# relgukxilef/GAN-Class-Transfer2

Measured on AMD Instinct MI355X. Metric: images/sec (train step) 3x128x128 bs=64/GPU, higher is better.
Workload: dtype bf16; 1 GPU; BASELINE config 3: Trainer step, 3x128x128, bs 64/GPU, octaves 6, pixel_size 128, max_size 512, bf16 operands / fp32 accumulate, Keras Adam + WarmUp; global_batch=64, parallelism=dp1

## Files before the change

gan-class-transfer2_amd/_lib.py:

```python
from __future__ import annotations

import ctypes as C
import os
import struct

F32, BF16, F16 = 0, 1, 2
F32_MATH_DIRECT, F32_MATH_MFMA = 0, 1
DTYPE_NAMES = {F32: "f32", BF16: "bf16", F16: "f16"}
ABI_VERSION = 17
DENSE2_FAST_PIXELS = 64
DENSE2_PLAIN_MAX = 256
SAMPLE_X, SAMPLE_EPS, SAMPLE_SCALED_EPS, SAMPLE_ODE = 0, 1, 2, 3
BUILD_STAMP = 1
CLIP_NONE, CLIP_VALUE, CLIP_NORM, CLIP_GLOBAL_NORM = 0, 1, 2, 3
SUMSQ_CHUNK, SUMSQ_MAX_SEGMENTS = 32768, 1024
OPT_ADAM, OPT_SGD, OPT_RMSPROP = 0, 1, 2
SCHEDULE_WARMUP, SCHEDULE_INVERSE_TIME_DECAY = 0, 1
GRAD_NONE, GRAD_SIGN = 0, 1
LOSS_MSE, LOSS_L1, LOSS_MSE_POOLED, LOSS_DCT = 0, 1, 2, 3

_HERE = os.path.dirname(os.path.abspath(__file__))
LIB_PATH = os.path.join(_HERE, "csrc", "libgct2.so")


class Gct2Error(RuntimeError):
    """non-zero status from libgct2 (mirrors TensorFlow raising on bad shapes, SURVEY.md §8b)."""


class LossScaleState(C.Structure):
    _fields_ = [("scale", C.c_float), ("inv_scale", C.c_float), ("good_steps", C.c_int32), ("found_inf", C.c_int32),
                ("applied_steps", C.c_int32), ("alpha", C.c_float), ("reserved", C.c_int32 * 2)]


class AdamArgs(C.Structure):
    _fields_ = [("p", C.c_void_p), ("m", C.c_void_p), ("v", C.c_void_p), ("shadow", C.c_void_p), ("shadow_dtype", C.c_int),
                ("n", C.c_size_t), ("alpha", C.c_float), ("beta1", C.c_float), ("beta2", C.c_float), ("eps", C.c_float),
                ("grad_mul", C.c_float), ("defer", C.c_int), ("slab_base", C.c_void_p), ("nslab", C.c_int), ("slab_stride", C.c_size_t)]


_vp, _i, _f, _d, _u64, _sz = C.c_void_p, C.c_int, C.c_float, C.c_double, C.c_uint64, C.c_size_t

SIGNATURES = {
    "gct2_abi_version": [],
    "gct2_build_flags": [],
    "gct2_device_check": [],
    "gct2_stream_occupy": [_vp, _i, _d],
    "gct2_ctx_create": [C.POINTER(C.c_void_p)],
    "gct2_ctx_destroy": [_vp],
    "gct2_ctx_set_workspace": [_vp, _vp, _sz],
    "gct2_ctx_set_wgrad_workspace": [_vp, _vp, _sz],
    "gct2_ctx_set_bias_queue": [_vp, _vp, _sz],
    "gct2_bias_queue_flush": [_vp, _vp],
    "gct2_ctx_set_tuning": [_vp, _i],
    "gct2_ctx_force_direct": [_vp, _i],
    "gct2_ctx_set_f32_math": [_vp, _i],
    "gct2_ctx_set_stamp_buffer": [_vp, _vp, _sz],
    "gct2_ctx_set_relu_bits": [_vp, _vp, _i],
    "gct2_ctx_log_launches": [_vp, _i],
    "gct2_ctx_read_launch_log": [_vp, _vp, _sz, C.POINTER(C.c_size_t)],
    "gct2_diffusion_mix": [_i, _vp, _vp, _f, _vp, _vp, _i, _vp, _i, _sz, _i, _vp],
    "gct2_diffusion_update": [_i, _vp, _vp, _d, _d, _vp, _vp, _sz, _vp],
    "gct2_noise_edits": [_vp, _vp, _i, _vp, _i, _i, _i, _vp],
    "gct2_image_prepare": [_vp, _vp, _vp, _vp, _i, _i, _vp],
    "gct2_conv4s2_fwd": [_vp, _i, _vp, _i, _vp, _vp, _vp, _i, _i, _i, _i, _i, _i, _i, _vp],
    "gct2_conv4s2_dgrad": [_vp, _i, _vp, _i, _vp, _vp, _i, _vp, _i, _i, _i, _i, _i, _i, _i, _vp, _i, _vp, _i, _vp],
    "gct2_conv4s2_wgrad": [_vp, _i, _vp, _i, _vp, _i, _vp, _vp, _i, _i, _i, _i, _i, _i, _vp, _vp],
    "gct2_adam_apply": [_vp, _vp, _sz, _vp],
    "gct2_convT4s2_fwd": [_vp, _i, _vp, _i, _vp, _vp, _vp, _i, _i, _i, _i, _i, _i, _i, _vp],
    "gct2_convT4s2_fwd_head_train": [_vp, _i, _vp, _i, _vp, _vp, _vp, _vp, _vp, _vp, _vp, _i, _vp, _vp, _vp, _i, _i, _i, _i, _i, _i, _i,
                                     _vp, _vp, _vp, _i, _i, _vp],
    "gct2_convT4s2_dgrad": [_vp, _i, _vp, _i, _vp, _vp, _i, _vp, _i, _i, _i, _i, _i, _i, _i, _vp, _i, _vp, _i, _vp],
    "gct2_convT4s2_wgrad": [_vp, _i, _vp, _i, _vp, _i, _vp, _vp, _i, _i, _i, _i, _i, _i, _vp, _vp],
    "gct2_conv2d_s1_fwd": [_vp, _i, _vp, _i, _vp, _vp, _vp, _i, _i, _i, _i, _i, _i, _i, _i, _vp],
    "gct2_conv2d_s1_dgrad": [_vp, _i, _vp, _i, _vp, _vp, _i, _vp, _i, _i, _i, _i, _i, _i, _i, _i, _vp],
    "gct2_conv2d_s1_wgrad": [_vp, _i, _vp, _i, _vp, _i, _vp, _vp, _i, _i, _i, _i, _i, _i, _i, _vp],
    "gct2_relu_mask": [_i, _vp, _i, _vp, _i, _sz, _i, _vp],
    "gct2_add": [_i, _vp, _i, _vp, _i, _sz, _i, _vp],
    "gct2_mix_per_image": [_vp, _vp, _vp, _vp, _vp, _i, _sz, _vp],
    "gct2_dense_fwd": [_i, _vp, _i, _vp, _vp, _vp, _i, _i, _i, _vp],
    "gct2_dense_bwd": [_i, _vp, _i, _vp, _vp, _vp, _i, _vp, _vp, _i, _i, _i, _i, _i, _vp],
    "gct2_dense_head_train": [_vp, _i, _vp, _i, _vp, _vp, _vp, _vp, _vp, _i, _vp, _vp, _vp, _vp, _i, _i, _i, _i, _vp, _vp, _vp, _i, _i, _vp],
    "gct2_dense_steps_fwd": [_vp, _i, _vp, _i, _vp, _vp, _vp, _vp, _i, _i, _i, _i, _i, _vp],
    "gct2_dense_steps_scratch": [_i, _i, _i, _i, C.POINTER(C.c_size_t)],
    "gct2_dense_steps_bwd": [_vp, _i, _vp, _i, _vp, _vp, _vp, _vp, _i, _vp, _vp, _vp, _sz, _i, _i, _i, _i, _i, _i, _i, _vp],
    "gct2_dense2_fwd": [_vp, _i, _vp, _i, _vp, _vp, _vp, _vp, _vp, _i, _i, _i, _i, _vp],
    "gct2_dense2_scratch": [_i, _i, _i, _i, C.POINTER(C.c_size_t)],
    "gct2_dense2_bwd": [_vp, _i, _vp, _i, _vp, _vp, _vp, _vp, _vp, _i, _vp, _vp, _vp, _vp, _vp, _sz, _i, _i, _i, _i, _i, _i, _vp],
    "gct2_rng_uniform_int": [_u64, _u64, _u64, _vp, _sz, _i, _i, _vp],
    "gct2_rng_normal": [_u64, _u64, _u64, _vp, _sz, _vp],
    "gct2_noise_image": [_i, _vp, _vp, _vp, _vp, _i, _vp, _i, _i, _i, _i, _i, _vp],
    "gct2_noise_image_rng": [_i, _vp, _vp, _u64, _u64, _u64, _vp, _vp, _i, _vp, _i, _i, _i, _i, _i, _vp],
    "gct2_mse_fwd_bwd": [_vp, _vp, _vp, _vp, _vp, _sz, _vp, _vp],
    "gct2_loss_scratch": [_i, _i, _i, _i, _i, C.POINTER(C.c_size_t)],
    "gct2_loss_fwd_bwd": [_i, _vp, _vp, _vp, _vp, _vp, _sz, _i, _i, _i, _i, _vp, _vp, _vp],
    "gct2_adam_keras_multi": [_vp, _vp, _vp, _vp, _vp, _i, _sz, _f, _f, _f, _f, _f, _vp, _i, _vp],
    "gct2_ema_update": [_vp, _vp, _vp, _i, _sz, _f, _f, _vp, _vp],
    "gct2_sumsq_layout": [_vp, _vp, _i, _vp, C.POINTER(C.c_size_t)],
    "gct2_grad_sumsq": [_vp, _vp, _i, _sz, _f, _vp, _vp, _vp, _vp],
    "gct2_adam_keras_clipped": [_vp, _vp, _vp, _vp, _vp, _i, _sz, _f, _f, _f, _f, _f, _vp, _i, _f, _vp, _vp],
    "gct2_optimizer_apply": [_i, _vp, _vp, _vp, _vp, _vp, _i, _sz, _f, _f, _i, _f, _f, _f, _vp, _i, _f, _vp, _vp],
    "gct2_optimizer_apply_reg": [_i, _vp, _vp, _vp, _vp, _vp, _i, _sz, _f, _f, _i, _f, _f, _f, _vp, _i, _f, _vp, _f, _i, _vp],
    "gct2_grad_sumsq_l2": [_vp, _vp, _vp, _vp, _i, _sz, _f, _vp, _vp, _vp, _vp],
    "gct2_l2_penalty": [_vp, _vp, _f, _vp, _vp, _vp],
    "gct2_cast_from_f32": [_i, _vp, _vp, _sz, _vp],
    "gct2_loss_scale_init": [_vp, _f, _vp],
    "gct2_loss_scale_begin": [_vp, _f, _i, _f, _f, _vp],
    "gct2_loss_scale_begin_schedule": [_vp, _i, _f, _f, _f, _i, _i, _f, _f, _vp],
    "gct2_scale_check_finite": [_vp, _sz, _vp, _vp],
    "gct2_loss_scale_update": [_vp, _i, _vp],
    "gct2_plan_create": [C.POINTER(C.c_void_p)],
    "gct2_plan_destroy": [_vp],
    "gct2_plan_add_call": [_vp, C.c_char_p, C.POINTER(C.c_uint64), _i, C.POINTER(C.c_int)],
    "gct2_plan_add_record": [_vp, _vp, C.POINTER(C.c_int)],
    "gct2_plan_add_wait": [_vp, _vp, _i],
    "gct2_plan_add_record_kind": [_vp, _vp, _i, C.POINTER(C.c_int)],
    "gct2_plan_elapsed": [_vp, _i, _i, C.POINTER(C.c_float)],
    "gct2_plan_size": [_vp, C.POINTER(C.c_int)],
    "gct2_plan_set_arg": [_vp, _i, _i, _u64],
    "gct2_plan_run": [_vp, _i, _i, C.POINTER(C.c_int)],
}

_lib = None


def load() -> C.CDLL:
    global _lib
    if _lib is not None:
        return _lib
    path = LIB_PATH
    if os.environ.get("GCT2_ALLOW_DIAGNOSTIC_BUILD") == "1" and os.environ.get("GCT2_USE_STAMP_LIB") in ("1", "phases"):
        path = os.path.join(_HERE, "csrc", "libgct2_phases.so" if os.environ["GCT2_USE_STAMP_LIB"] == "phases" else "libgct2_stamp.so")
    if not os.path.exists(path):
        raise Gct2Error(
            f"{path} not found: build it with `python -c 'import __graft_entry__ as g; g.build()'` "
            "(or `make -C gan-class-transfer2_amd/csrc`). There is no CPU fallback.")
    lib = C.CDLL(path)
    for name, argtypes in SIGNATURES.items():
        fn = getattr(lib, name)
        fn.argtypes = argtypes
        fn.restype = _i
    lib.gct2_last_error.argtypes = []
    lib.gct2_last_error.restype = C.c_char_p
    if lib.gct2_abi_version() != ABI_VERSION:
        raise Gct2Error(f"{LIB_PATH} has ABI version {lib.gct2_abi_version()}, this binding is written for {ABI_VERSION}: rebuild it "
                        "(`make -C gan-class-transfer2_amd/csrc`)")
    flags = lib.gct2_build_flags()
    if flags != 0 and os.environ.get("GCT2_ALLOW_DIAGNOSTIC_BUILD") != "1":
        raise Gct2Error(f"{LIB_PATH} is a DIAGNOSTIC build (gct2_build_flags() = {flags}: in-kernel stamps): results and timings of "
                        "such a library are never product numbers.  Rebuild with `make -C gan-class-transfer2_amd/csrc clean all`, or "
                        "set GCT2_ALLOW_DIAGNOSTIC_BUILD=1 for the scripts/stamp_*.py diagnostics")
    _lib = lib
    return lib


def build_flags() -> int:
    return int(load().gct2_build_flags())


def check(rc: int, what: str = "") -> None:
    if rc != 0:
        msg = load().gct2_last_error().decode("utf-8", "replace")
        raise Gct2Error(f"{what or 'gct2'} failed (status {rc}): {msg}")


class Slot:
    __slots__ = ("key", "value")

    def __init__(self, key: str, value):
        self.key, self.value = key, value


def call(name: str, *args) -> None:
    if _recording is not None:
        _recording.add_call(name, args)
        if not _recording.execute or name not in PLANNABLE:
            return
    check(getattr(load(), name)(*[a.value if type(a) is Slot else a for a in args]), name)


PLANNABLE = frozenset(n for n, sig in SIGNATURES.items() if n == "gct2_ctx_set_relu_bits" or (
    not n.startswith(("gct2_ctx_", "gct2_plan_", "gct2_loss_scale_init")) and n not in ("gct2_abi_version", "gct2_build_flags", "gct2_device_check", "gct2_stream_occupy", "gct2_sumsq_layout", "gct2_loss_scratch", "gct2_dense_steps_scratch", "gct2_dense2_scratch")))
_recording = None
_FLOAT_STRUCT = struct.Struct("<f")
_DOUBLE_STRUCT = struct.Struct("<d")


def _slot_bits(ctype, v) -> int:
    if ctype is _f:
        return int.from_bytes(_FLOAT_STRUCT.pack(float(v)), "little")
    if ctype is _d:
        return int.from_bytes(_DOUBLE_STRUCT.pack(float(v)), "little")
    if v is None:
        return 0
    return int(v) & 0xFFFFFFFFFFFFFFFF


EVENT_DEVICE, EVENT_SYSTEM, EVENT_TIMED = 0, 1, 2


class Plan:

    def __init__(self):
        h = C.c_void_p()
        check(load().gct2_plan_create(C.byref(h)), "gct2_plan_create")
        self.handle = h.value
        self.execute = True
        self.slots = {}
        self.values = {}
        self.cuts = []
        self.keep = []
        self.n = 0

    def begin(self, execute: bool = True) -> None:
        global _recording
        if _recording is not None:
            raise Gct2Error("a plan is already recording")
        self.execute = execute
        _recording = self

    def end(self) -> None:
        global _recording
        _recording = None
        self.cuts.append((self.n, None))

    def add_call(self, name: str, args) -> None:
        if name not in PLANNABLE:
            check(getattr(load(), name)(*[a.value if type(a) is Slot else a for a in args]), name)
            return
        types = SIGNATURES[name]
        if len(types) != len(args):
            raise Gct2Error(f"{name}: {len(args)} arguments for {len(types)} parameters")
        arr = (C.c_uint64 * len(args))()
        for i, (t, a) in enumerate(zip(types, args)):
            if type(a) is Slot:
                self.slots.setdefault(a.key, []).append((self.n, i, t))
                self.values[a.key] = a.value
                a = a.value
            arr[i] = _slot_bits(t, a)
        idx = C.c_int(-1)
        check(load().gct2_plan_add_call(self.handle, name.encode(), arr, len(args), C.byref(idx)), "gct2_plan_add_call")
        self.n = idx.value + 1

    def record(self, stream: int, kind: int = EVENT_DEVICE) -> int:
        ev = C.c_int(-1)
        check(load().gct2_plan_add_record_kind(self.handle, stream, kind, C.byref(ev)), "gct2_plan_add_record_kind")
        self.n += 1
        return ev.value

    def elapsed_ms(self, start: int, end: int) -> float:
        ms = C.c_float(0.0)
        check(load().gct2_plan_elapsed(self.handle, start, end, C.byref(ms)), "gct2_plan_elapsed")
        return ms.value

    def wait(self, stream: int, event: int) -> None:
        check(load().gct2_plan_add_wait(self.handle, stream, event), "gct2_plan_add_wait")
        self.n += 1

    def cut(self, payload) -> None:
        self.cuts.append((self.n, payload))

    def set(self, key: str, value) -> None:
        if self.values.get(key) == value:
            return
        self.values[key] = value
        L = load()
        for rec, arg, t in self.slots.get(key, ()):
            check(L.gct2_plan_set_arg(self.handle, rec, arg, _slot_bits(t, value)), "gct2_plan_set_arg")

    def segments(self) -> int:
        return len(self.cuts)

    def run_segment(self, k: int):
        first = self.cuts[k - 1][0] if k else 0
        last, payload = self.cuts[k]
        if last > first:
            failed = C.c_int(-1)
            rc = load().gct2_plan_run(self.handle, first, last - first, C.byref(failed))
            if rc != 0:
                check(rc, f"gct2_plan_run (record {failed.value})")
        return payload

    def __del__(self):
        try:
            if getattr(self, "handle", None) and _lib is not None:
                _lib.gct2_plan_destroy(self.handle)
                self.handle = None
        except Exception:
            pass


class Context:

    def __init__(self):
        h = C.c_void_p()
        call("gct2_ctx_create", C.byref(h))
        self.handle = h.value
        self._keep = [None, None, None]
        self.version = 0
        self.tuning = 0
        self.direct = False
        self.f32_math = F32_MATH_DIRECT
        self.logging = False

    def set_relu_bits(self, ptr, ld_bytes: int) -> None:
        call("gct2_ctx_set_relu_bits", self.handle, ptr, int(ld_bytes) if ptr is not None else 0)

    def set_stamp_buffer(self, tensor) -> None:
        self._keep[2] = tensor
        self.version += 1
        call("gct2_ctx_set_stamp_buffer", self.handle, tensor.data_ptr() if tensor is not None else None,
             tensor.numel() * tensor.element_size() if tensor is not None else 0)

    def log_launches(self, on: bool = True) -> None:
        self.logging = bool(on)
        call("gct2_ctx_log_launches", self.handle, int(bool(on)))

    def read_launch_log(self) -> list:
        need = C.c_size_t(0)
        buf = C.create_string_buffer(1 << 12)
        rc = load().gct2_ctx_read_launch_log(self.handle, C.cast(buf, C.c_void_p), len(buf), C.byref(need))
        if rc != 0 and need.value > len(buf):
            buf = C.create_string_buffer(need.value)
            rc = load().gct2_ctx_read_launch_log(self.handle, C.cast(buf, C.c_void_p), len(buf), C.byref(need))
        check(rc, "gct2_ctx_read_launch_log")
        return [t for t in buf.value.decode().split(";") if t]

    def mirror(self, other: "Context") -> None:
        if self.tuning != other.tuning:
            self.set_tuning(other.tuning)
        if self.direct != other.direct:
            self.force_direct(other.direct)
        if self.f32_math != other.f32_math:
            self.set_f32_math(other.f32_math)
        if self.logging != other.logging:
            self.log_launches(other.logging)
        if self._keep[2] is not other._keep[2]:
            self.set_stamp_buffer(other._keep[2])

    def set_workspace(self, tensor) -> None:
        self._keep[0] = tensor
        self.version += 1
        call("gct2_ctx_set_workspace", self.handle, tensor.data_ptr() if tensor is not None else None,
             tensor.numel() * tensor.element_size() if tensor is not None else 0)

    def set_wgrad_workspace(self, tensor) -> None:
        self._keep[1] = tensor
        self.version += 1
        call("gct2_ctx_set_wgrad_workspace", self.handle, tensor.data_ptr() if tensor is not None else None,
             tensor.numel() * tensor.element_size() if tensor is not None else 0)

    def set_bias_queue(self, tensor) -> None:
        self._keep.append(tensor)
        self.version += 1
        call("gct2_ctx_set_bias_queue", self.handle, tensor.data_ptr() if tensor is not None else None,
             tensor.numel() * tensor.element_size() if tensor is not None else 0)

    def set_tuning(self, v: int) -> None:
        self.version += 1
        self.tuning = int(v)
        call("gct2_ctx_set_tuning", self.handle, int(v))

    def force_direct(self, on: bool) -> None:
        self.version += 1
        self.direct = bool(on)
        call("gct2_ctx_force_direct", self.handle, int(bool(on)))

    def set_f32_math(self, mode: int) -> None:
        call("gct2_ctx_set_f32_math", self.handle, int(mode))
        self.version += 1
        self.f32_math = int(mode)

    def __del__(self):
        try:
            if getattr(self, "handle", None) and _lib is not None:
                _lib.gct2_ctx_destroy(self.handle)
                self.handle = None
        except Exception:
            pass
```

gan-class-transfer2_amd/csrc/capi.hip:

```cpp
#include "gct2_common.h"
#include <cstdarg>
#include <cstdio>
#include <cstring>

static thread_local char g_err[512] = "";
static thread_local gct2_ctx g_null_ctx{};

int gct2_fail(int code, const char* fmt, ...) {
  va_list ap;
  va_start(ap, fmt);
  vsnprintf(g_err, sizeof(g_err), fmt, ap);
  va_end(ap);
  return code;
}
void gct2_log(gct2_ctx& c, const char* fmt, ...) {
  if (!c.log_on) return;
  char buf[160];
  va_list ap;
  va_start(ap, fmt);
  vsnprintf(buf, sizeof(buf), fmt, ap);
  va_end(ap);
  constexpr size_t LOG_CAP = (size_t)1 << 20;
  if (c.log.size() + sizeof(buf) + 16 > LOG_CAP) {
    if (!c.log_full) { c.log += "log:truncated;"; c.log_full = true; }
    return;
  }
  c.log += buf;
  c.log += ';';
}
int gct2_check_launch(const char* what) {
  const hipError_t e = hipGetLastError();
  if (e != hipSuccess) return gct2_fail(GCT2_ELAUNCH, "%s: %s", what, hipGetErrorString(e));
  return GCT2_OK;
}

namespace {
inline hipStream_t S(void* s) { return reinterpret_cast<hipStream_t>(s); }
inline bool dtype_ok(int d) { return d == GCT2_F32 || d == GCT2_BF16 || d == GCT2_F16; }
inline size_t esize(int d) { return d == GCT2_F32 ? 4 : 2; }

int check_conv_args(const char* fn, int dtype, const void* a, const void* b, const void* c, int B, int H, int W, int Cin, int Cout) {
  if (!dtype_ok(dtype)) return gct2_fail(GCT2_EINVAL, "%s: unknown dtype %d", fn, dtype);
  if (!a || !b || !c) return gct2_fail(GCT2_EINVAL, "%s: null pointer", fn);
  if (B <= 0 || H <= 0 || W <= 0 || Cin <= 0 || Cout <= 0) return gct2_fail(GCT2_EINVAL, "%s: non-positive dimension", fn);
  if ((size_t)B * H * W * 4 >= ((size_t)1 << 31)) return gct2_fail(GCT2_EINVAL, "%s: B*H*W too large for 32-bit pixel indices", fn);
  return GCT2_OK;
}
inline gct2_ctx& C(gct2_ctx* c) {
  if (c) return *c;
  g_null_ctx = gct2_ctx{};
  return g_null_ctx;
}
struct PlaneTaken {
  unsigned char* bits; int ld;
  explicit PlaneTaken(gct2_ctx& c) : bits(c.relu_bits), ld(c.relu_ldbits) { c.relu_bits = nullptr; c.relu_ldbits = 0; c.relu_bits_done = 0; }
  int none(const char* fn) const {
    return bits ? gct2_fail(GCT2_EINVAL, "%s: a ReLU bit plane was registered (gct2_ctx_set_relu_bits), but this call neither writes nor reads one", fn) : GCT2_OK;
  }
  int into(const char* fn, int channels, TapGemmParams& p) const {
    if (!bits) return GCT2_OK;
    if (channels % 8 || ld < channels / 8) return gct2_fail(GCT2_EINVAL, "%s: ReLU bit plane needs channels %% 8 == 0 and ld_bytes >= channels / 8 (got %d, %d)", fn, channels, ld);
    p.bits = bits; p.ldbits = ld;
    return GCT2_OK;
  }
};
int finish_relu_bits(gct2_ctx& c, int dtype, const TapGemmParams& p, size_t pixels, void* stream) {
  if (!p.bits || c.relu_bits_done) return GCT2_OK;
  gct2_log(c, "relu_bits:derived");
  return pw_relu_bits(dtype, p.y, p.ldy, pixels, p.N, p.bits, p.ldbits, S(stream));
}
inline bool f32_on_mfma(const gct2_ctx& c, int dtype) { return dtype == GCT2_F32 && c.f32_math == GCT2_F32_MATH_MFMA && !c.force_direct; }
int run_tapgemm(gct2_ctx& c, int dtype, int form, int epi, const TapGemmParams& p, void* stream) {
  const bool s1 = form == FORM_S1 || form == FORM_S1T;
  if (f32_on_mfma(c, dtype)) return f32_tapgemm(c, form, epi, p, S(stream));
  if (!c.force_direct && (!s1 || p.ks <= 5) && tapgemm_mfma_supported(dtype, p)) return tapgemm_mfma(c, dtype, form, epi, p, S(stream));
  if (s1)
    return conv_s1_direct(dtype, form == FORM_S1T, p.x, p.ldx, p.w, p.bias, p.act, p.ldact, p.y, p.ldy, p.B, p.Hs, p.Ws, p.K, p.N, p.ks, p.relu,
                          p.accumulate, S(stream));
  gct2_log(c, "direct:tap");
  return tapgemm_direct(dtype, form, epi, p, S(stream));
}
int run_dgrad(gct2_ctx& c, int dtype, int form, TapGemmParams p, size_t out_pixels, float* db, int split, float* db2, int db_acc,
              void* stream) {
  if (split < 0 || split > p.N) return gct2_fail(GCT2_EINVAL, "dgrad: db_split out of range");
  p.db = db; p.db_split = split; p.db2 = db2; p.db_acc = db_acc;
  if (!c.force_direct && tapgemm_mfma_supported(dtype, p)) return tapgemm_mfma(c, dtype, form, EPI_MASK, p, S(stream));
  const bool f32m = f32_on_mfma(c, dtype);
  if (!f32m) gct2_log(c, "direct:tap");
  if (int e = tapgemm_dbq_flush_for(c, db, split, db2, p.N - split, S(stream))) return e;
  zero_overwritten_db(p, S(stream));
  const size_t es = esize(dtype);
  auto sums = [&](float sign) -> int {
    if (db && split > 0) if (int e = pw_colsum(dtype, p.y, p.ldy, db, out_pixels, split, sign, S(stream))) return e;
    if (db2 && split < p.N)
      if (int e = pw_colsum(dtype, (const char*)p.y + (size_t)split * es, p.ldy, db2, out_pixels, p.N - split, sign, S(stream))) return e;
    return GCT2_OK;
  };
  if ((db || db2) && p.accumulate) if (int e = sums(-1.f)) return e;
  if (int e = f32m ? f32_tapgemm(c, form, EPI_MASK, p, S(stream)) : tapgemm_direct(dtype, form, EPI_MASK, p, S(stream))) return e;
  return (db || db2) ? sums(1.f) : GCT2_OK;
}
int run_wgrad(gct2_ctx& c, int dtype, const WgradParams& p, void* stream, WgradSlabs* defer) {
  if (f32_on_mfma(c, dtype)) return f32_wgrad(c, p, S(stream), defer);
  if (!c.force_direct && wgrad_mfma_supported(dtype, p)) return wgrad_mfma(c, dtype, p, S(stream), defer);
  if (defer) *defer = WgradSlabs{nullptr, 0, 0};
  if (p.ks)
    return conv_s1_wgrad_direct(dtype, p.big, p.ldbig, p.small, p.ldsmall, p.dw, p.B, p.Hs, p.Ws, p.Cb, p.Cs, p.ks, p.accumulate, S(stream));
  gct2_log(c, "direct:wgrad");
  return wgrad_direct(dtype, p, S(stream));
}
int wgrad_db(gct2_ctx& c, int dtype, const void* dz, int lddz, float* db, size_t pixels, int Cout, int accumulate, void* stream) {
  if (int e = tapgemm_dbq_flush_for(c, db, Cout, nullptr, 0, S(stream))) return e;
  if (!accumulate) (void)hipMemsetAsync(db, 0, (size_t)Cout * sizeof(float), S(stream));
  return pw_colsum(dtype, dz, lddz, db, pixels, Cout, 1.f, S(stream));
}
int check_adam_args(const gct2_adam_args* a, const float* dw, size_t nw) {
  if (!a->p || !a->m || !a->v) return gct2_fail(GCT2_EINVAL, "wgrad + adam: null arena pointers");
  if (a->n < nw || ((uintptr_t)a->p | (uintptr_t)a->m | (uintptr_t)a->v | (uintptr_t)dw) % 16)
    return gct2_fail(GCT2_EINVAL, "wgrad + adam: range shorter than the weight tensor or misaligned");
  return GCT2_OK;
}
int run_adam(const gct2_adam_args* a, float* dw, size_t nw, const WgradSlabs& sl, void* stream) {
  return pw_adam(a->p, a->m, a->v, dw, a->shadow, a->shadow_dtype, a->n, a->alpha, a->beta1, a->beta2, a->eps, a->grad_mul, nullptr, 0,
                 S(stream), sl.base, sl.nslab, sl.stride, sl.nslab ? nw : 0);
}
int adam_after_wgrad(gct2_adam_args* a, float* dw, size_t nw, const WgradSlabs& sl, void* stream) {
  if (a->defer) {
    a->slab_base = sl.base; a->nslab = sl.nslab; a->slab_stride = sl.stride;
    return GCT2_OK;
  }
  return run_adam(a, dw, nw, sl, stream);
}
int check_s1(const char* fn, int KS) {
  if (KS < 1 || KS > 7 || !(KS & 1)) return gct2_fail(GCT2_EINVAL, "%s: kernel size %d (odd, 1..7: 'same' padding is symmetric then)", fn, KS);
  return GCT2_OK;
}
enum WgradKind { WG_CONV, WG_CONVT, WG_S1 };
int wgrad_entry(gct2_ctx* ctx, const char* fn, WgradKind kind, int dtype, const void* x, int ldx, const void* dz, int lddz, float* dw, float* db,
                int B, int H, int W, int Cin, int Cout, int KS, int accumulate, gct2_adam_args* adam, void* stream) {
  gct2_ctx& c = C(ctx);
  if (int e = PlaneTaken(c).none(fn)) return e;
  const int up = kind == WG_CONVT ? 2 : 1;
  if (int e = check_conv_args(fn, dtype, x, dz, dw, B, up * H, up * W, Cin, Cout)) return e;
  if (kind == WG_S1) if (int e = check_s1(fn, KS)) return e;
  if (kind == WG_CONV && ((H & 1) || (W & 1))) return gct2_fail(GCT2_EINVAL, "%s: H=%d W=%d must be even", fn, H, W);
  if (ldx < Cin || lddz < Cout) return gct2_fail(GCT2_EINVAL, "%s: ld smaller than channel count", fn);
  if (adam && accumulate) return gct2_fail(GCT2_EINVAL, "%s: the fused optimizer step needs accumulate = 0", fn);
  WgradParams p = kind == WG_CONV    ? WgradParams{x, ldx, dz, lddz, dw, B, H / 2, W / 2, Cin, Cout, 1}
                  : kind == WG_CONVT ? WgradParams{dz, lddz, x, ldx, dw, B, H, W, Cout, Cin, 1}
                                     : WgradParams{x, ldx, dz, lddz, dw, B, H, W, Cin, Cout, 1};
  p.accumulate = accumulate ? 1 : 0;
  p.ks = kind == WG_S1 ? KS : 0;
  const size_t nw = (size_t)16 * Cin * Cout, dz_pixels = (size_t)B * p.Hs * p.Ws * (kind == WG_CONVT ? 4 : 1);
  WgradSlabs sl{nullptr, 0, 0};
  WgradSlabs* defer = adam ? &sl : nullptr;
  if (adam) if (int e = check_adam_args(adam, dw, nw)) return e;
  if (kind == WG_CONV && !c.force_direct && rgb_wgrad_supported(dtype, p)) {
    gct2_log(c, "rgb:wgrad");
    if (int e = rgb_wgrad(c, dtype, p, S(stream), defer)) return e;
  } else if (int e = run_wgrad(c, dtype, p, stream, defer)) return e;
  if (db) if (int e = wgrad_db(c, dtype, dz, lddz, db, dz_pixels, Cout, accumulate, stream)) return e;
  return adam ? adam_after_wgrad(adam, dw, nw, sl, stream) : GCT2_OK;
}
int check_scratch(const char* fn, const gct2_ctx* ctx, const void* buf) {
  if (!ctx) return gct2_fail(GCT2_EINVAL, "%s: null ctx", fn);
  if (buf && ((uintptr_t)buf % 16)) return gct2_fail(GCT2_EINVAL, "%s: pointer must be 16-byte aligned", fn);
  return GCT2_OK;
}
}

extern "C" {

int gct2_abi_version(void) { return 17; }
int gct2_build_flags(void) {
#ifdef GCT2_STAMP
  return GCT2_BUILD_STAMP;
#else
  return 0;
#endif
}
const char* gct2_last_error(void) { return g_err; }

int gct2_ctx_create(gct2_ctx** ctx) {
  if (!ctx) return gct2_fail(GCT2_EINVAL, "ctx_create: null output pointer");
  *ctx = new (std::nothrow) gct2_ctx();
  return *ctx ? GCT2_OK : gct2_fail(GCT2_EINVAL, "ctx_create: out of host memory");
}
int gct2_ctx_destroy(gct2_ctx* ctx) {
  delete ctx;
  return GCT2_OK;
}
int gct2_ctx_set_workspace(gct2_ctx* ctx, void* ws, size_t bytes) {
  if (int e = check_scratch("ctx_set_workspace", ctx, ws)) return e;
  ctx->ws = ws ? reinterpret_cast<float*>(ws) : nullptr;
  ctx->ws_bytes = ws ? bytes : 0;
  return GCT2_OK;
}
int gct2_ctx_set_wgrad_workspace(gct2_ctx* ctx, void* ws, size_t bytes) {
  if (int e = check_scratch("ctx_set_wgrad_workspace", ctx, ws)) return e;
  ctx->wws = ws ? reinterpret_cast<float*>(ws) : nullptr;
  ctx->wws_bytes = ws ? bytes : 0;
  return GCT2_OK;
}
int gct2_ctx_set_bias_queue(gct2_ctx* ctx, void* buf, size_t bytes) {
  if (int e = check_scratch("ctx_set_bias_queue", ctx, buf)) return e;
  ctx->dbq_jobs.clear();
  ctx->dbq_used = 0;
  ctx->dbq = buf ? reinterpret_cast<float*>(buf) : nullptr;
  ctx->dbq_floats = buf ? bytes / sizeof(float) : 0;
  return GCT2_OK;
}
int gct2_bias_queue_flush(gct2_ctx* ctx, void* stream) {
  if (!ctx) return gct2_fail(GCT2_EINVAL, "bias_queue_flush: null ctx");
  return tapgemm_dbq_flush(*ctx, S(stream));
}
int gct2_ctx_set_tuning(gct2_ctx* ctx, int v) {
  if (!ctx) return gct2_fail(GCT2_EINVAL, "ctx_set_tuning: null ctx");
  const int tap = v & 0xff, wg = (v >> 16) & 0xff, known = 0x1ff | (0xff << 16) | (0x7f << 24);
  if ((v & ~known) || (tap != 0 && tap != 2 && tap != 5) || (wg != 0 && wg != 2 && wg != 3 && wg != 4 && wg != 5 && wg != 6 && wg != 7) || ((v >> 24) & 3) == 3 || ((v >> 26) & 3) == 3)
    return gct2_fail(GCT2_EINVAL, "ctx_set_tuning: unknown tuning word 0x%x (include/gct2.h)", v);
  ctx->tap_variant = tap;
  ctx->wgrad_variant = wg;
  ctx->no_splitk = (v >> 8) & 1;
  ctx->halo_mode = (v >> 24) & 3;
  ctx->xcd_order = (v >> 26) & 3;
  ctx->wgrad_split = (v >> 28) & 7;
  return GCT2_OK;
}
int gct2_ctx_set_relu_bits(gct2_ctx* ctx, void* bits, int ld_bytes) {
  if (!ctx) return gct2_fail(GCT2_EINVAL, "ctx_set_relu_bits: null ctx");
  if (bits && ld_bytes <= 0) return gct2_fail(GCT2_EINVAL, "ctx_set_relu_bits: ld_bytes must be positive");
  ctx->relu_bits = reinterpret_cast<unsigned char*>(bits);
  ctx->relu_ldbits = bits ? ld_bytes : 0;
  return GCT2_OK;
}
int gct2_ctx_set_stamp_buffer(gct2_ctx* ctx, void* stamps, size_t bytes) {
  if (!ctx) return gct2_fail(GCT2_EINVAL, "ctx_set_stamp_buffer: null ctx");
#ifdef GCT2_STAMP
  if (stamps && ((uintptr_t)stamps % 8)) return gct2_fail(GCT2_EINVAL, "ctx_set_stamp_buffer: pointer must be 8-byte aligned");
  ctx->stamps = reinterpret_cast<unsigned long long*>(stamps);
  ctx->stamps_bytes = stamps ? bytes : 0;
  return GCT2_OK;
#else
  (void)stamps; (void)bytes;
  return gct2_fail(GCT2_EINVAL, "ctx_set_stamp_buffer: this is the product build (rebuild with make EXTRA=-DGCT2_STAMP for in-kernel stamps)");
#endif
}
int gct2_ctx_log_launches(gct2_ctx* ctx, int on) {
  if (!ctx) return gct2_fail(GCT2_EINVAL, "ctx_log_launches: null ctx");
  ctx->log_on = on != 0;
  ctx->log.clear();
  ctx->log_full = false;
  return GCT2_OK;
}
int gct2_ctx_read_launch_log(gct2_ctx* ctx, char* buf, size_t bytes, size_t* needed) {
  if (!ctx) return gct2_fail(GCT2_EINVAL, "ctx_read_launch_log: null ctx");
  const size_t need = ctx->log.size() + 1;
  if (needed) *needed = need;
  if (!buf || bytes < need)
    return gct2_fail(GCT2_EINVAL, "ctx_read_launch_log: the log holds %zu bytes, the buffer %zu", need, buf ? bytes : (size_t)0);
  memcpy(buf, ctx->log.data(), need - 1);
  buf[need - 1] = 0;
  ctx->log.clear();
  ctx->log_full = false;
  return GCT2_OK;
}
int gct2_ctx_force_direct(gct2_ctx* ctx, int on) {
  if (!ctx) return gct2_fail(GCT2_EINVAL, "ctx_force_direct: null ctx");
  ctx->force_direct = on ? 1 : 0;
  return GCT2_OK;
}
int gct2_ctx_set_f32_math(gct2_ctx* ctx, int mode) {
  if (!ctx) return gct2_fail(GCT2_EINVAL, "ctx_set_f32_math: null ctx");
  if (mode != GCT2_F32_MATH_DIRECT && mode != GCT2_F32_MATH_MFMA) return gct2_fail(GCT2_EINVAL, "ctx_set_f32_math: unknown mode %d", mode);
  ctx->f32_math = mode;
  return GCT2_OK;
}

int gct2_device_check(void) {
  int dev = 0;
  if (hipGetDevice(&dev) != hipSuccess) return gct2_fail(GCT2_ENODEV, "no HIP device");
  hipDeviceProp_t prop;
  if (hipGetDeviceProperties(&prop, dev) != hipSuccess) return gct2_fail(GCT2_ENODEV, "hipGetDeviceProperties failed");
  if (strncmp(prop.gcnArchName, "gfx950", 6) != 0) return gct2_fail(GCT2_ENODEV, "device is %s, this library is built for gfx950", prop.gcnArchName);
  return GCT2_OK;
}

int gct2_stream_occupy(void* stream, int workgroups, double microseconds) {
  if (workgroups < 1 || workgroups > 1024 || !(microseconds >= 0.0) || microseconds > 20000.0)
    return gct2_fail(GCT2_EINVAL, "stream_occupy: 1..1024 work-groups for 0..20000 us (got %d, %g)", workgroups, microseconds);
  return pw_occupy(workgroups, (unsigned long long)(microseconds * 100.0), S(stream));
}

int gct2_conv4s2_fwd(gct2_ctx* ctx, int dtype, const void* x, int ldx, const void* w, const float* bias, void* y, int ldy, int B, int H, int W,
                     int Cin, int Cout, int relu, void* stream) {
  gct2_ctx& c = C(ctx);
  const PlaneTaken plane(c);
  if (int e = check_conv_args("conv4s2_fwd", dtype, x, w, y, B, H, W, Cin, Cout)) return e;
  if ((H & 1) || (W & 1)) return gct2_fail(GCT2_EINVAL, "conv4s2_fwd: H=%d W=%d must be even (skip concat, train.py:114-119)", H, W);
  if (ldx < Cin || ldy < Cout) return gct2_fail(GCT2_EINVAL, "conv4s2_fwd: ld smaller than channel count");
  TapGemmParams p{x, ldx, w, bias, nullptr, 0, y, ldy, B, H / 2, W / 2, Cin, Cout, relu, 0};
  if (int e = plane.into("conv4s2_fwd", Cout, p)) return e;
  const size_t out_pixels = (size_t)B * (H / 2) * (W / 2);
  if (!c.force_direct && rgb_fwd_supported(dtype, p)) {
    gct2_log(c, "rgb:fwd");
    if (int e = rgb_fwd(dtype, p, S(stream))) return e;
    if (p.bits && rgb_fwd_writes_bits(p)) c.relu_bits_done = 1;
    return finish_relu_bits(c, dtype, p, out_pixels, stream);
  }
  if (int e = run_tapgemm(c, dtype, FORM_CONV, EPI_BIAS_ACT, p, stream)) return e;
  return finish_relu_bits(c, dtype, p, out_pixels, stream);
}

int gct2_conv4s2_dgrad(gct2_ctx* ctx, int dtype, const void* dz, int lddz, const void* w, const void* act, int ldact, void* dx, int lddx, int B,
                       int H, int W, int Cin, int Cout, int accumulate, float* db, int db_split, float* db2, int db_accumulate, void* stream) {
  gct2_ctx& c = C(ctx);
  const PlaneTaken plane(c);
  if (int e = check_conv_args("conv4s2_dgrad", dtype, dz, w, dx, B, H, W, Cin, Cout)) return e;
  if ((H & 1) || (W & 1)) return gct2_fail(GCT2_EINVAL, "conv4s2_dgrad: H=%d W=%d must be even", H, W);
  if (lddz < Cout || lddx < Cin || (act && ldact < Cin)) return gct2_fail(GCT2_EINVAL, "conv4s2_dgrad: ld smaller than channel count");
  TapGemmParams p{dz, lddz, w, nullptr, act, ldact, dx, lddx, B, H / 2, W / 2, Cout, Cin, 0, accumulate};
  if (int e = plane.into("conv4s2_dgrad", Cin, p)) return e;
  if (!act) p.bits = nullptr;
  return run_dgrad(c, dtype, FORM_CONVT, p, (size_t)B * H * W, db, db_split, db2, db_accumulate, stream);
}

int gct2_conv4s2_wgrad(gct2_ctx* ctx, int dtype, const void* x, int ldx, const void* dz, int lddz, float* dw, float* db, int B, int H, int W,
                       int Cin, int Cout, int accumulate, gct2_adam_args* adam, void* stream) {
  return wgrad_entry(ctx, "conv4s2_wgrad", WG_CONV, dtype, x, ldx, dz, lddz, dw, db, B, H, W, Cin, Cout, 0, accumulate, adam, stream);
}

int gct2_convT4s2_fwd(gct2_ctx* ctx, int dtype, const void* x, int ldx, const void* w, const float* bias, void* y, int ldy, int B, int H, int W,
                      int Cin, int Cout, int relu, void* stream) {
  gct2_ctx& c = C(ctx);
  const PlaneTaken plane(c);
  if (int e = check_conv_args("convT4s2_fwd", dtype, x, w, y, B, 2 * H, 2 * W, Cin, Cout)) return e;
  if (ldx < Cin || ldy < Cout) return gct2_fail(GCT2_EINVAL, "convT4s2_fwd: ld smaller than channel count");
  TapGemmParams p{x, ldx, w, bias, nullptr, 0, y, ldy, B, H, W, Cin, Cout, relu, 0};
  if (int e = plane.into("convT4s2_fwd", Cout, p)) return e;
  if (int e = run_tapgemm(c, dtype, FORM_CONVT, EPI_BIAS_ACT, p, stream)) return e;
  return finish_relu_bits(c, dtype, p, (size_t)B * 4 * H * W, stream);
}

int gct2_convT4s2_fwd_head_train(gct2_ctx* ctx, int dtype, const void* x, int ldx, const void* w, const float* bias, const float* head_w,
                                 const float* head_b, const float* target, float* pred, void* dy, int lddy, float* head_dw, float* head_db,
                                 float* loss, int B, int H, int W, int Cin, int Cout, int head_Cin, int head_Cout,
                                 const float* loss_scale_ptr, float* db, const void* x2, int ldx2, int accumulate, void* stream) {
  gct2_ctx& c = C(ctx);
  if (int e = PlaneTaken(c).none("convT4s2_fwd_head_train")) return e;
  if (int e = check_conv_args("convT4s2_fwd_head_train", dtype, x, w, dy, B, 2 * H, 2 * W, Cin, Cout)) return e;
  if (!head_w || !target || !head_dw || !loss) return gct2_fail(GCT2_EINVAL, "convT4s2_fwd_head_train: null pointer");
  if (ldx < Cin || lddy < Cout) return gct2_fail(GCT2_EINVAL, "convT4s2_fwd_head_train: ld smaller than channel count");
  const int nimg = head_Cin - Cout;
  if (head_Cout < 1 || head_Cout > 3 || nimg < 0 || nimg > 3 || (nimg > 0 && (!x2 || ldx2 < 4 || ldx2 % 4 || (uintptr_t)x2 % 8)))
    return gct2_fail(GCT2_EINVAL, "convT4s2_fwd_head_train: head needs <= 3 outputs and <= 3 image channels in a packed x2 (8-byte rows)");
  TapGemmParams p{x, ldx, w, bias, nullptr, 0, dy, lddy, B, H, W, Cin, Cout, 1, 0};
  p.head = HeadFuse{head_w, head_b, target, pred, x2, ldx2, nullptr, loss_scale_ptr, head_Cin, head_Cout,
                    (float)((double)B * 2 * H * 2 * W * head_Cout)};
  if (c.force_direct || !halo_head_supported(c, dtype, p))
    return gct2_fail(GCT2_EINVAL, "convT4s2_fwd_head_train: needs a 16-bit dtype, Cout = 64, H and W multiples of 16, 16-byte aligned views "
                                  "and a ctx workspace of B*(H/16)*(W/16)*288 floats");
  return halo_head(c, dtype, p, head_dw, head_db, loss, db, accumulate, S(stream));
}

int gct2_convT4s2_dgrad(gct2_ctx* ctx, int dtype, const void* dz, int lddz, const void* w, const void* act, int ldact, void* dx, int lddx, int B,
                        int H, int W, int Cin, int Cout, int accumulate, float* db, int db_split, float* db2, int db_accumulate, void* stream) {
  gct2_ctx& c = C(ctx);
  const PlaneTaken plane(c);
  if (int e = check_conv_args("convT4s2_dgrad", dtype, dz, w, dx, B, 2 * H, 2 * W, Cin, Cout)) return e;
  if (lddz < Cout || lddx < Cin || (act && ldact < Cin)) return gct2_fail(GCT2_EINVAL, "convT4s2_dgrad: ld smaller than channel count");
  TapGemmParams p{dz, lddz, w, nullptr, act, ldact, dx, lddx, B, H, W, Cout, Cin, 0, accumulate};
  if (int e = plane.into("convT4s2_dgrad", Cin, p)) return e;
  if (!act) p.bits = nullptr;
  return run_dgrad(c, dtype, FORM_CONV, p, (size_t)B * H * W, db, db_split, db2, db_accumulate, stream);
}

int gct2_convT4s2_wgrad(gct2_ctx* ctx, int dtype, const void* x, int ldx, const void* dz, int lddz, float* dw, float* db, int B, int H, int W,
                        int Cin, int Cout, int accumulate, gct2_adam_args* adam, void* stream) {
  return wgrad_entry(ctx, "convT4s2_wgrad", WG_CONVT, dtype, x, ldx, dz, lddz, dw, db, B, H, W, Cin, Cout, 0, accumulate, adam, stream);
}

int gct2_conv2d_s1_fwd(gct2_ctx* ctx, int dtype, const void* x, int ldx, const void* w, const float* bias, void* y, int ldy, int B, int H, int W,
                       int Cin, int Cout, int KS, int relu, void* stream) {
  gct2_ctx& c = C(ctx);
  if (int e = PlaneTaken(c).none("conv2d_s1_fwd")) return e;
  if (int e = check_conv_args("conv2d_s1_fwd", dtype, x, w, y, B, H, W, Cin, Cout)) return e;
  if (int e = check_s1("conv2d_s1_fwd", KS)) return e;
  if (ldx < Cin || ldy < Cout) return gct2_fail(GCT2_EINVAL, "conv2d_s1_fwd: ld smaller than channel count");
  TapGemmParams p{x, ldx, w, bias, nullptr, 0, y, ldy, B, H, W, Cin, Cout, relu, 0};
  p.ks = KS;
  return run_tapgemm(c, dtype, FORM_S1, EPI_BIAS_ACT, p, stream);
}
int gct2_conv2d_s1_dgrad(gct2_ctx* ctx, int dtype, const void* dz, int lddz, const void* w, const void* act, int ldact, void* dx, int lddx, int B,
                         int H, int W, int Cin, int Cout, int KS, int accumulate, void* stream) {
  gct2_ctx& c = C(ctx);
  if (int e = PlaneTaken(c).none("conv2d_s1_dgrad")) return e;
  if (int e = check_conv_args("conv2d_s1_dgrad", dtype, dz, w, dx, B, H, W, Cin, Cout)) return e;
  if (int e = check_s1("conv2d_s1_dgrad", KS)) return e;
  if (lddz < Cout || lddx < Cin || (act && ldact < Cin)) return gct2_fail(GCT2_EINVAL, "conv2d_s1_dgrad: ld smaller than channel count");
  TapGemmParams p{dz, lddz, w, nullptr, act, ldact, dx, lddx, B, H, W, Cout, Cin, 0, accumulate};
  p.ks = KS;
  return run_tapgemm(c, dtype, FORM_S1T, EPI_MASK, p, stream);
}
int gct2_conv2d_s1_wgrad(gct2_ctx* ctx, int dtype, const void* x, int ldx, const void* dz, int lddz, float* dw, float* db, int B, int H, int W,
                         int Cin, int Cout, int KS, int accumulate, void* stream) {
  return wgrad_entry(ctx, "conv2d_s1_wgrad", WG_S1, dtype, x, ldx, dz, lddz, dw, db, B, H, W, Cin, Cout, KS, accumulate, nullptr, stream);
}
int gct2_relu_mask(int dtype, const void* act, int ldact, void* d, int ldd, size_t npix, int C, void* stream) {
  if (!dtype_ok(dtype) || !act || !d || C <= 0 || ldact < C || ldd < C) return gct2_fail(GCT2_EINVAL, "relu_mask: bad dtype, null pointer or ld < C");
  if (npix == 0) return GCT2_OK;
  return pw_relu_mask(dtype, act, ldact, d, ldd, npix, C, S(stream));
}
int gct2_add(int dtype, void* dst, int lddst, const void* src, int ldsrc, size_t npix, int C, void* stream) {
  if (!dtype_ok(dtype) || !dst || !src || C <= 0 || lddst < C || ldsrc < C) return gct2_fail(GCT2_EINVAL, "add: bad dtype, null pointer or ld < C");
  if (npix == 0) return GCT2_OK;
  return pw_add(dtype, dst, lddst, src, ldsrc, npix, C, S(stream));
}
int gct2_mix_per_image(const float* x, const float* eps, const float* a, const float* c, float* out, int B, size_t per_image, void* stream) {
  if (!x || !a || !out || (eps && !c) || B <= 0 || per_image == 0) return gct2_fail(GCT2_EINVAL, "mix_per_image: null pointer or empty batch");
  return pw_mix_per_image(x, eps, a, c, out, B, per_image, S(stream));
}

int gct2_dense_fwd(int dtype, const void* x, int ldx, const float* w, const float* b, float* y, int M, int Cin, int Cout, void* stream) {
  if (!dtype_ok(dtype) || !x || !w || !y) return gct2_fail(GCT2_EINVAL, "dense_fwd: bad dtype or null pointer");
  if (M <= 0 || Cin <= 0 || Cout <= 0 || Cout > 4 || ldx < Cin) return gct2_fail(GCT2_EINVAL, "dense_fwd: bad shape (Cout must be 1..4)");
  return pw_dense_fwd(dtype, x, ldx, w, b, y, M, Cin, Cout, S(stream));
}

int gct2_dense_bwd(int dtype, const void* x, int ldx, const float* w, const float* dy, void* dx, int lddx, float* dw, float* db, int M,
                   int Cin, int Cout, int Cmask, int accumulate, void* stream) {
  if (!dtype_ok(dtype) || !x || !w || !dy || !dx || !dw) return gct2_fail(GCT2_EINVAL, "dense_bwd: bad dtype or null pointer");
  if (M <= 0 || Cin <= 0 || Cout <= 0 || Cout > 4 || ldx < Cin || Cmask < 0 || Cmask > Cin || lddx < Cmask)
    return gct2_fail(GCT2_EINVAL, "dense_bwd: bad shape");
  if ((Cin + 1) * Cout > 2048) return gct2_fail(GCT2_EINVAL, "dense_bwd: (Cin+1)*Cout = %d exceeds 2048", (Cin + 1) * Cout);
  if ((size_t)Cin * 16 + 128 * 16 + (size_t)128 * Cin * esize(dtype) > 160 * 1024)
    return gct2_fail(GCT2_EINVAL, "dense_bwd: Cin=%d too large for the LDS tile", Cin);
  return pw_dense_bwd(dtype, x, ldx, w, dy, dx, lddx, dw, db, M, Cin, Cout, Cmask, accumulate, S(stream));
}

static int check_steps_shape(const char* fn, int B, int HW, int Cin, int Cout, int steps) {
  if (B <= 0 || HW <= 0 || Cin <= 0 || steps <= 0) return gct2_fail(GCT2_EINVAL, "%s: non-positive dimension (B=%d HW=%d Cin=%d steps=%d)", fn, B, HW, Cin, steps);
  if (Cout < 1 || Cout > 4) return gct2_fail(GCT2_EINVAL, "%s: Cout=%d outside 1..4", fn, Cout);
  if (B > 65535 || steps > 65535) return gct2_fail(GCT2_EINVAL, "%s: B=%d / steps=%d beyond 65535 (one grid row per image / per slice)", fn, B, steps);
  if ((size_t)B * HW >= ((size_t)1 << 31)) return gct2_fail(GCT2_EINVAL, "%s: B*HW too large for 32-bit pixel indices", fn);
  if ((size_t)Cin * steps * Cout >= ((size_t)1 << 31)) return gct2_fail(GCT2_EINVAL, "%s: Cin*steps*Cout too large for 32-bit weight indices", fn);
  return GCT2_OK;
}
int gct2_dense_steps_fwd(gct2_ctx* ctx, int dtype, const void* x, int ldx, const float* w, const float* b, const int32_t* t_int, float* y,
                         int B, int HW, int Cin, int Cout, int steps, void* stream) {
  if (!dtype_ok(dtype)) return gct2_fail(GCT2_EINVAL, "dense_steps_fwd: unknown dtype %d", dtype);
  if (!x || !w || !t_int || !y) return gct2_fail(GCT2_EINVAL, "dense_steps_fwd: null pointer (x, w, t_int, y)");
  if (int e = check_steps_shape("dense_steps_fwd", B, HW, Cin, Cout, steps)) return e;
  if (ldx < Cin) return gct2_fail(GCT2_EINVAL, "dense_steps_fwd: ldx=%d smaller than Cin=%d", ldx, Cin);
  if ((size_t)Cin * 16 > 64 * 1024) return gct2_fail(GCT2_EINVAL, "dense_steps_fwd: Cin=%d too large for the LDS weight image", Cin);
  if (ctx) gct2_log(*ctx, "dense_steps:fwd");
  return pw_dense_steps_fwd(dtype, x, ldx, w, b, t_int, y, B, HW, Cin, Cout, steps, S(stream));
}
int gct2_dense_steps_scratch(int B, int HW, int Cin, int Cout, size_t* floats) {
  if (!floats) return gct2_fail(GCT2_EINVAL, "dense_steps_scratch: null output pointer");
  if (int e = check_steps_shape("dense_steps_scratch", B, HW, Cin, Cout, 1)) return e;
  if ((Cin + 1) * Cout > 2048) return gct2_fail(GCT2_EINVAL, "dense_steps_scratch: (Cin+1)*Cout = %d exceeds 2048", (Cin + 1) * Cout);
  *floats = dense_steps_scratch_floats(B, HW, Cin, Cout);
  return GCT2_OK;
}
int gct2_dense_steps_bwd(gct2_ctx* ctx, int dtype, const void* x, int ldx, const float* w, const int32_t* t_int, const float* dy, void* dx,
                         int lddx, float* dw, float* db, float* scratch, size_t scratch_floats, int B, int HW, int Cin, int Cout, int steps,
                         int Cmask, int accumulate, void* stream) {
  if (!dtype_ok(dtype)) return gct2_fail(GCT2_EINVAL, "dense_steps_bwd: unknown dtype %d", dtype);
  if (!x || !w || !t_int || !dy || !dw || !scratch) return gct2_fail(GCT2_EINVAL, "dense_steps_bwd: null pointer (x, w, t_int, dy, dw, scratch)");
  if (int e = check_steps_shape("dense_steps_bwd", B, HW, Cin, Cout, steps)) return e;
  if (ldx < Cin) return gct2_fail(GCT2_EINVAL, "dense_steps_bwd: ldx=%d smaller than Cin=%d", ldx, Cin);
  if (Cmask < 0 || Cmask > Cin || (dx && lddx < Cmask)) return gct2_fail(GCT2_EINVAL, "dense_steps_bwd: Cmask=%d outside 0..Cin or lddx=%d smaller than it", Cmask, lddx);
  if ((Cin + 1) * Cout > 2048) return gct2_fail(GCT2_EINVAL, "dense_steps_bwd: (Cin+1)*Cout = %d exceeds 2048", (Cin + 1) * Cout);
  if ((size_t)Cin * 16 + 128 * 16 + (size_t)128 * Cin * esize(dtype) > 160 * 1024)
    return gct2_fail(GCT2_EINVAL, "dense_steps_bwd: Cin=%d too large for the LDS tile", Cin);
  if ((uintptr_t)scratch % 16) return gct2_fail(GCT2_EINVAL, "dense_steps_bwd: scratch must be 16-byte aligned");
  const size_t need = dense_steps_scratch_floats(B, HW, Cin, Cout);
  if (scratch_floats < need)
    return gct2_fail(GCT2_EINVAL, "dense_steps_bwd: %zu floats of scratch, this shape needs %zu (gct2_dense_steps_scratch)", scratch_floats, need);
  if (ctx) gct2_log(*ctx, "dense_steps:bwd");
  return pw_dense_steps_bwd(dtype, x, ldx, w, t_int, dy, dx, lddx, dw, db, scratch, B, HW, Cin, Cout, steps, Cmask, accumulate, S(stream));
}
// ... 360 lines not shown
```

gan-class-transfer2_amd/csrc/gct2_common.h:

```cpp
#pragma once
#include <hip/hip_runtime.h>
#include <stdint.h>
#include <stddef.h>
#include <string>
#include <vector>
#include "../../include/gct2.h"

typedef __attribute__((ext_vector_type(8))) __bf16 bf16x8_t;
typedef __attribute__((ext_vector_type(8))) _Float16 f16x8_t;
typedef __attribute__((ext_vector_type(4))) short s16x4_t;
typedef __attribute__((ext_vector_type(4))) float f32x4_t;
typedef __attribute__((ext_vector_type(4))) uint32_t u32x4_t;
typedef __attribute__((ext_vector_type(2))) uint32_t u32x2_t;
typedef __attribute__((address_space(3))) s16x4_t lds_s16x4_t;

struct gct2_ctx {
  float* ws = nullptr; size_t ws_bytes = 0;
  float* wws = nullptr; size_t wws_bytes = 0;
  int tap_variant = 0;
  int wgrad_variant = 0;
  int halo_mode = 0;
  int xcd_order = 0;
  int wgrad_split = 0;
  int no_splitk = 0;
  int force_direct = 0;
  int f32_math = GCT2_F32_MATH_DIRECT;
  unsigned long long* stamps = nullptr; size_t stamps_bytes = 0;
  unsigned char* relu_bits = nullptr; int relu_ldbits = 0; int relu_bits_done = 0;
  bool log_on = false, log_full = false; std::string log;
  struct DbJob { const float* part; int rows, N; float* db; int db_split; float* db2; int db_acc; };
  float* dbq = nullptr; size_t dbq_floats = 0, dbq_used = 0;
  std::vector<DbJob> dbq_jobs;
  float* dbq_alloc(size_t floats) {
    floats = (floats + 3) / 4 * 4;
    if (!dbq || dbq_jobs.size() >= 16 || dbq_used + floats > dbq_floats) return nullptr;
    float* q = dbq + dbq_used;
    dbq_used += floats;
    return q;
  }
  float* wgrad_scratch(size_t* bytes) const {
    if (wws) { *bytes = wws_bytes; return wws; }
    *bytes = ws_bytes; return ws;
  }
};

#ifdef GCT2_STAMP
constexpr size_t GCT2_CLOCK_OFF = (size_t)1 << 19, GCT2_CLOCK_ENTRIES = (size_t)1 << 16, GCT2_CLOCK_BYTES = (GCT2_CLOCK_OFF + 8 * GCT2_CLOCK_ENTRIES) * 8;
struct ClockStamp { unsigned long long t0 = 0, r0 = 0, t1 = 0, r1 = 0, rin = 0; };
__device__ __forceinline__ void clock_now(unsigned long long& t, unsigned long long& r) {
  __builtin_amdgcn_sched_barrier(0);
  asm volatile("s_memtime %0\n\ts_memrealtime %1\n\ts_waitcnt lgkmcnt(0)" : "=s"(t), "=s"(r)::"memory");
  __builtin_amdgcn_sched_barrier(0);
}
__device__ __forceinline__ unsigned long long realtime_now() {
  unsigned long long r;
  __builtin_amdgcn_sched_barrier(0);
  asm volatile("s_memrealtime %0\n\ts_waitcnt lgkmcnt(0)" : "=s"(r)::"memory");
  __builtin_amdgcn_sched_barrier(0);
  return r;
}
__device__ __forceinline__ void clock_store(unsigned long long* stamps, const ClockStamp& c, int waves_per_group, int wave, int lane) {
  const size_t e = (size_t)blockIdx.x * waves_per_group + wave;
  if (stamps && lane == 0 && e < GCT2_CLOCK_ENTRIES) {
    unsigned long long* o = stamps + GCT2_CLOCK_OFF + e * 8;
    o[0] = c.t0; o[1] = c.r0; o[2] = c.t1; o[3] = c.r1; o[4] = c.rin;
  }
}
__device__ __forceinline__ void clock_exit(unsigned long long* stamps, int waves_per_group, int wave, int lane) {
  const size_t e = (size_t)blockIdx.x * waves_per_group + wave;
  asm volatile("s_waitcnt vmcnt(0)" ::: "memory");
  const unsigned long long r = realtime_now();
  if (stamps && lane == 0 && e < GCT2_CLOCK_ENTRIES) stamps[GCT2_CLOCK_OFF + e * 8 + 5] = r;
}
#define GCT2_CLOCK_DECL ClockStamp clk_; clk_.rin = realtime_now()
#define GCT2_CLOCK_BEGIN clock_now(clk_.t0, clk_.r0)
#define GCT2_CLOCK_END(stamps, nwaves, wave, lane) do { clock_now(clk_.t1, clk_.r1); clock_store(stamps, clk_, nwaves, wave, lane); } while (0)
#define GCT2_CLOCK_EXIT(stamps, nwaves, wave, lane) clock_exit(stamps, nwaves, wave, lane)
#else
#define GCT2_CLOCK_DECL
#define GCT2_CLOCK_BEGIN
#define GCT2_CLOCK_END(stamps, nwaves, wave, lane)
#define GCT2_CLOCK_EXIT(stamps, nwaves, wave, lane)
#endif

template <typename T> struct is16 { static constexpr bool value = sizeof(T) == 2; };

template <typename T> __device__ __forceinline__ float to_f32(T v) { return (float)v; }
template <typename T> __device__ __forceinline__ T from_f32(float v) { return (T)v; }

template <typename T> __device__ __forceinline__ f32x4_t mfma16(u32x4_t a, u32x4_t b, f32x4_t c);
template <> __device__ __forceinline__ f32x4_t mfma16<__bf16>(u32x4_t a, u32x4_t b, f32x4_t c) {
  return __builtin_amdgcn_mfma_f32_16x16x32_bf16(__builtin_bit_cast(bf16x8_t, a),
                                                 __builtin_bit_cast(bf16x8_t, b), c, 0, 0, 0);
}
template <> __device__ __forceinline__ f32x4_t mfma16<_Float16>(u32x4_t a, u32x4_t b, f32x4_t c) {
  return __builtin_amdgcn_mfma_f32_16x16x32_f16(__builtin_bit_cast(f16x8_t, a),
                                                __builtin_bit_cast(f16x8_t, b), c, 0, 0, 0);
}

__device__ __forceinline__ int nimg_off(int row, int chunk) {
  return row * 128 + ((chunk ^ ((row >> 1) & 7)) << 4);
}
__device__ __forceinline__ int timg_swz(int k) { return (k & 3) | (((k >> 3) & 1) << 2); }
__device__ __forceinline__ int timg_off(int k, int chunk16) {
  return k * 256 + ((((chunk16 >> 1) ^ timg_swz(k))) << 5) + ((chunk16 & 1) << 4);
}

__device__ __forceinline__ u32x4_t lds_read128(const char* lds, int off) {
  return *reinterpret_cast<const u32x4_t*>(lds + off);
}
__device__ __forceinline__ void lds_write128(char* lds, int off, u32x4_t v) {
  *reinterpret_cast<u32x4_t*>(lds + off) = v;
}
__device__ __forceinline__ u32x4_t nimg_frag(const char* img, int rowbase, int kk, int lane) {
  return lds_read128(img, nimg_off(rowbase + (lane & 15), 4 * kk + (lane >> 4)));
}
__device__ __forceinline__ u32x4_t timg_frag(const char* img, int colbase, int kk, int lane) {
  const int g = lane >> 4, q = (lane >> 2) & 3, p = lane & 3;
  const int k0 = kk * 32 + 8 * g + q;
  const int c32 = colbase >> 4;
  const int o0 = k0 * 256 + ((c32 ^ timg_swz(k0)) << 5) + p * 8;
  const int o1 = (k0 + 4) * 256 + ((c32 ^ timg_swz(k0 + 4)) << 5) + p * 8;
  s16x4_t lo = __builtin_amdgcn_ds_read_tr16_b64_v4i16((lds_s16x4_t*)(img + o0));
  s16x4_t hi = __builtin_amdgcn_ds_read_tr16_b64_v4i16((lds_s16x4_t*)(img + o1));
  u32x2_t l2 = __builtin_bit_cast(u32x2_t, lo), h2 = __builtin_bit_cast(u32x2_t, hi);
  u32x4_t r = {l2[0], l2[1], h2[0], h2[1]};
  return r;
}

template <int CTRL> __device__ __forceinline__ float dpp_f32(float v) {
  return __builtin_bit_cast(float, __builtin_amdgcn_update_dpp(0, __builtin_bit_cast(int, v), CTRL, 0xf, 0xf, true));
}
__device__ __forceinline__ float row16_sum(float t) {
  t += dpp_f32<0xB1>(t);
  t += dpp_f32<0x4E>(t);
  t += dpp_f32<0x141>(t);
  t += dpp_f32<0x140>(t);
  return t;
}
__device__ __forceinline__ float rows4_sum(float t) {
  float a = t, b = t;
  asm volatile("" : "+v"(b));
  asm volatile("v_permlane16_swap_b32 %0, %1" : "+v"(a), "+v"(b));
  t = a + b;
  a = t; b = t;
  asm volatile("" : "+v"(b));
  asm volatile("v_permlane32_swap_b32 %0, %1" : "+v"(a), "+v"(b));
  return a + b;
}

__device__ __forceinline__ unsigned rows4_or(unsigned t) {
  unsigned a = t, b = t;
  asm volatile("" : "+v"(b));
  asm volatile("v_permlane16_swap_b32 %0, %1" : "+v"(a), "+v"(b));
  t = a | b;
  a = t; b = t;
  asm volatile("" : "+v"(b));
  asm volatile("v_permlane32_swap_b32 %0, %1" : "+v"(a), "+v"(b));
  return a | b;
}

__device__ __forceinline__ u32x4_t gload128(const void* p) {
  return *reinterpret_cast<const u32x4_t*>(p);
}

typedef __attribute__((ext_vector_type(2))) float f32x2_t;
template <typename T> __device__ __forceinline__ uint32_t pack2(float a, float b) {
  typedef __attribute__((ext_vector_type(2))) T t2_t;
  static_assert(sizeof(T) == 2, "pack2 packs 16-bit storage types");
  const f32x2_t v = {a, b};
  return __builtin_bit_cast(uint32_t, __builtin_convertvector(v, t2_t));
}
template <typename T> __device__ __forceinline__ float unpack_lo(uint32_t u) {
  return to_f32<T>(__builtin_bit_cast(T, (uint16_t)(u & 0xffffu)));
}
template <typename T> __device__ __forceinline__ float unpack_hi(uint32_t u) {
  return to_f32<T>(__builtin_bit_cast(T, (uint16_t)(u >> 16)));
}

template <typename T> __device__ __forceinline__ unsigned relu_bits8(u32x4_t o) {
  unsigned m = 0;
#pragma unroll
  for (int k = 0; k < 4; k++) {
    m |= (unpack_lo<T>(o[k]) > 0.f ? 1u : 0u) << (2 * k);
    m |= (unpack_hi<T>(o[k]) > 0.f ? 1u : 0u) << (2 * k + 1);
  }
  return m;
}
__device__ __forceinline__ void apply_relu_bits8(unsigned m, f32x4_t& a, f32x4_t& c) {
#pragma unroll
  for (int r = 0; r < 4; r++) {
    if (!((m >> r) & 1u)) a[r] = 0.f;
    if (!((m >> (4 + r)) & 1u)) c[r] = 0.f;
  }
}

enum { FORM_CONV = 0, FORM_CONVT = 1, FORM_S1 = 2, FORM_S1T = 3 };
enum { EPI_BIAS_ACT = 0, EPI_MASK = 1, EPI_HEAD = 2 };

template <typename T> __device__ __forceinline__ float keras_f16_point(float v) {
  if constexpr (sizeof(T) == 2 && !__is_same(T, __bf16)) return (float)(_Float16)v;
  else return v;
}

constexpr int HEAD_ROW = 288;
struct HeadFuse {
  const float* w; const float* b;
  const float* target;
  float* pred;
  const void* x2; int ldx2;
  float* part;
  const float* loss_scale;
  int Cin, Cout;
  float count;
};

struct TapGemmParams {
  const void* x; int ldx;
  const void* w;
  const float* bias;
  const void* act; int ldact;
  void* y; int ldy;
  int B, Hs, Ws;
  int K, N;
  int relu, accumulate;
  float* ws; int ksplit;
  int m_tiles, n_tiles, xcd_chunk;
  int wstat;
  int wide;
  float* db; int db_split; float* db2;
  int db_acc;
  float* dbws;
  HeadFuse head;
  int ks = 0;
  int bits_words = 0;
  unsigned char* bits = nullptr; int ldbits = 0;
  int ws_shift = -1, hs_shift = -1;
#ifdef GCT2_STAMP
  unsigned long long* stamps = nullptr;
  int clock = 0;
#endif
};
inline int pow2_shift(int v) { return (v > 0 && !(v & (v - 1))) ? __builtin_ctz((unsigned)v) : -1; }
__device__ __forceinline__ void decode_pixel(int m, int Hs, int Ws, int hs_shift, int ws_shift, int& sw, int& sh, int& b) {
  if (ws_shift >= 0 && hs_shift >= 0) {
    sw = m & (Ws - 1);
    const int t = m >> ws_shift;
    sh = t & (Hs - 1);
    b = t >> hs_shift;
  } else {
    sw = m % Ws;
    const int t = m / Ws;
    sh = t % Hs;
    b = t / Hs;
  }
}

__device__ __forceinline__ bool xcd_tile(int id, int m_tiles, int inner, int chunk, int& m_tile, int& in) {
  const int xcd = id & 7, j = id >> 3;
  in = j % inner;
  m_tile = xcd * chunk + j / inner;
  return (j / inner) < chunk && m_tile < m_tiles;
}

inline void zero_overwritten_db(const TapGemmParams& p, hipStream_t s) {
  if (p.db && !(p.db_acc & 1) && p.db_split > 0) (void)hipMemsetAsync(p.db, 0, (size_t)p.db_split * sizeof(float), s);
  if (p.db2 && !(p.db_acc & 2) && p.N > p.db_split) (void)hipMemsetAsync(p.db2, 0, (size_t)(p.N - p.db_split) * sizeof(float), s);
}

__device__ __forceinline__ void adam_keras_update(float& p, float& m, float& v, float g, float alpha, float b1, float ob1, float b2,
                                                  float ob2, float eps) {
#pragma clang fp contract(off)
  const float m1 = b1 * m, m2 = ob1 * g;
  m = m1 + m2;
  const float v1 = b2 * v, v2 = (ob2 * g) * g;
  v = v1 + v2;
  const float num = alpha * m, den = sqrtf(v) + eps;
  p = p - num / den;
}
struct WgradParams {
  const void* big; int ldbig;
  const void* small; int ldsmall;
  float* dw;
  int B, Hs, Ws, Cb, Cs;
  int rsplit;
  float* ws;
  int accumulate;
  int ks = 0;
#ifdef GCT2_STAMP
  unsigned long long* stamps = nullptr;
  int clock = 0;
#endif
};
struct WgradSlabs { const float* base; int nslab; size_t stride; };

template <typename T> struct DTypeTag { using type = T; };
template <typename F> inline auto with_dtype16(int dtype, F&& f) {
  if (dtype == GCT2_BF16) return f(DTypeTag<__bf16>{});
  return f(DTypeTag<_Float16>{});
}
template <typename F> inline auto with_dtype(int dtype, F&& f) {
  if (dtype == GCT2_F32) return f(DTypeTag<float>{});
  return with_dtype16(dtype, f);
}

int gct2_fail(int code, const char* fmt, ...);
void gct2_log(gct2_ctx& c, const char* fmt, ...);
int gct2_check_launch(const char* what);

bool tapgemm_mfma_supported(int dtype, const TapGemmParams& p);
int tapgemm_mfma(gct2_ctx& c, int dtype, int form, int epi, const TapGemmParams& p, hipStream_t s);
int tapgemm_dbpart_reduce(const float* part, int rows, const TapGemmParams& p, hipStream_t s);
int tapgemm_dbq_push(gct2_ctx& c, const float* part, int rows, const TapGemmParams& p, hipStream_t s);
int tapgemm_dbq_flush(gct2_ctx& c, hipStream_t s);
int tapgemm_dbq_flush_for(gct2_ctx& c, const float* db, int n0, const float* db2, int n1, hipStream_t s);

bool halo_convT_wanted(const gct2_ctx& c, int epi, const TapGemmParams& p);
int halo_convT(gct2_ctx& c, int dtype, int epi, TapGemmParams p, hipStream_t s);
bool halo_head_supported(const gct2_ctx& c, int dtype, const TapGemmParams& p);
int halo_head(gct2_ctx& c, int dtype, TapGemmParams p, float* dw, float* db, float* loss, float* db_up, int accumulate, hipStream_t s);

bool wgrad_mfma_supported(int dtype, const WgradParams& p);
int wgrad_mfma(gct2_ctx& c, int dtype, WgradParams p, hipStream_t s, WgradSlabs* defer);
int wgrad_reduce(const float* ws, float* dw, size_t n, int nsplit, int accumulate, hipStream_t s);

bool rgb_fwd_supported(int dtype, const TapGemmParams& p);
bool rgb_fwd_writes_bits(const TapGemmParams& p);
int rgb_fwd(int dtype, const TapGemmParams& p, hipStream_t s);
bool rgb_wgrad_supported(int dtype, const WgradParams& p);
int rgb_wgrad(const gct2_ctx& c, int dtype, WgradParams p, hipStream_t s, WgradSlabs* defer);

int f32_tapgemm(gct2_ctx& c, int form, int epi, TapGemmParams p, hipStream_t s);
int f32_wgrad(gct2_ctx& c, WgradParams p, hipStream_t s, WgradSlabs* defer);

int loss_scratch_floats(int kind, int B, int H, int W, int C, size_t* partial_floats, size_t* floats);
int loss_l1(const float* pred, const float* target, float* dpred, float* loss, float* scratch, size_t n, const float* ls, hipStream_t s);
int loss_pooled(const float* pred, const float* target, float* dpred, float* loss, float* scratch, int B, int H, int W, int C, const float* ls,
                hipStream_t s);
int loss_dct(const float* pred, const float* target, float* dpred, float* loss, float* scratch, int B, int S, int C, const float* basis,
             const float* ls, hipStream_t s);

int tapgemm_direct(int dtype, int form, int epi, const TapGemmParams& p, hipStream_t s);
int wgrad_direct(int dtype, WgradParams p, hipStream_t s);
int conv_s1_direct(int dtype, bool dgrad, const void* x, int ldx, const void* w, const float* bias, const void* act, int ldact, void* y, int ldy,
                   int B, int H, int W, int K, int N, int KS, int relu, int accumulate, hipStream_t s);
int conv_s1_wgrad_direct(int dtype, const void* x, int ldx, const void* dz, int lddz, float* dw, int B, int H, int W, int Cin, int Cout, int KS,
                         int accumulate, hipStream_t s);

int pw_occupy(int workgroups, unsigned long long ticks, hipStream_t s);
int pw_rng_uniform_int(uint64_t seed, uint64_t stream_id, uint64_t offset, int32_t* out, size_t n, int lo, int hi, hipStream_t s);
int pw_rng_normal(uint64_t seed, uint64_t stream_id, uint64_t offset, float* out, size_t n, hipStream_t s);
int pw_noise(int dtype, const float* x, const int32_t* t, const float* eps, void* out, int ldout, void* out2, int ldout2, int B, int HW,
             int C, int steps, hipStream_t s);
int pw_noise_rng(int dtype, const float* x, const int32_t* t, uint64_t seed, uint64_t stream_id, uint64_t offset, float* eps_out, void* out,
                 int ldout, void* out2, int ldout2, int B, int HW, int C, int steps, hipStream_t s);
int pw_dense_fwd(int dtype, const void* x, int ldx, const float* w, const float* b, float* y, int M, int Cin, int Cout, hipStream_t s);
int pw_dense_bwd(int dtype, const void* x, int ldx, const float* w, const float* dy, void* dx, int lddx, float* dw, float* db, int M,
                 int Cin, int Cout, int Cmask, int accumulate, hipStream_t s);
size_t dense_steps_scratch_floats(int B, int HW, int Cin, int Cout);
int pw_dense_steps_fwd(int dtype, const void* x, int ldx, const float* w, const float* b, const int32_t* t_int, float* y, int B, int HW,
                       int Cin, int Cout, int steps, hipStream_t s);
int pw_dense_steps_bwd(int dtype, const void* x, int ldx, const float* w, const int32_t* t_int, const float* dy, void* dx, int lddx,
                       float* dw, float* db, float* scratch, int B, int HW, int Cin, int Cout, int steps, int Cmask, int accumulate,
                       hipStream_t s);
size_t dense2_scratch_floats(int M, int Cin, int Chid, int Cout);
int dense2_fwd(gct2_ctx& c, int dtype, const void* x, int ldx, const void* w1, const float* b1, const float* w2, const float* b2, float* y,
               int M, int Cin, int Chid, int Cout, hipStream_t s);
int dense2_bwd(gct2_ctx& c, int dtype, const void* x, int ldx, const void* w1, const float* b1, const float* w2, const float* dy, void* dx,
               int lddx, float* dw1, float* db1, float* dw2, float* db2, float* scratch, int M, int Cin, int Chid, int Cout, int Cmask,
               int accumulate, hipStream_t s);
int pw_head_finish(const float* part, int rows, float* dw, float* db, float* loss, float* db_dx, int ndw, int Cout, float inv_n,
                   int accumulate, hipStream_t s);
int pw_dense_head_train(const gct2_ctx& c, int dtype, const void* x, int ld, const float* w, const float* b, const float* target, float* pred,
                        void* dx, int lddx, float* dw, float* db, float* loss, float* partials, int M, int Cin, int Cout, int Cmask,
                        const float* ls, float* db_dx, const void* x2, int ldx2, int accumulate, hipStream_t s);
int pw_diffusion_mix(int dtype, const float* x, const float* e, float a, float* fake, void* out, int ldout, void* out2, int ldout2,
                     size_t npix, int C, hipStream_t s);
int pw_diffusion_update(int mode, const float* pred, const float* fake, double a, double a1, float* x, float* e, size_t n, hipStream_t s);
int pw_noise_edits(const float* eps, const float* dict, int K, float* out, int H, int W, int C, hipStream_t s);
int pw_image_prepare(const uint8_t* src, const int64_t* offsets, const int32_t* dims, float* dst, int B, int size, hipStream_t s);
int pw_mse(const float* pred, const float* target, float* dpred, float* loss, float* partials, size_t n, const float* ls, hipStream_t s);
int pw_relu_mask(int dtype, const void* act, int ldact, void* d, int ldd, size_t npix, int C, hipStream_t s);
int pw_add(int dtype, void* dst, int lddst, const void* src, int ldsrc, size_t npix, int C, hipStream_t s);
int pw_mix_per_image(const float* x, const float* eps, const float* a, const float* c, float* out, int B, size_t per_image, hipStream_t s);
int pw_colsum(int dtype, const void* dz, int ld, float* db, size_t M, int C, float sign, hipStream_t s);
int pw_adam(float* p, float* m, float* v, float* g, void* shadow, int shadow_dtype, size_t n, float alpha, float b1, float b2, float eps,
            float grad_mul, const gct2_loss_scale_state* ls, int zero_grad, hipStream_t s, const float* slabs = nullptr, int nslab = 0,
            size_t slab_stride = 0, size_t n_slab = 0);
int pw_ema(float* ema, const float* p, void* shadow, int shadow_dtype, size_t n, float momentum, float one_minus,
           const gct2_loss_scale_state* ls, hipStream_t s);
int pw_grad_sumsq(const float* g, const gct2_sumsq_seg* segs, int nseg, size_t npartials, float grad_mul, gct2_loss_scale_state* ls,
                  double* partials, double* sumsq, hipStream_t s);
int pw_adam_clipped(float* p, float* m, float* v, const float* g, void* shadow, int shadow_dtype, size_t n, float alpha, float b1, float b2,
                    float eps, float grad_mul, const gct2_loss_scale_state* ls, int mode, float clip, const double* sumsq, hipStream_t s);
int pw_optimizer(int kind, float* p, float* m, float* v, const float* g, void* shadow, int shadow_dtype, size_t n, float lr, float momentum,
                 int nesterov, float rho, float eps, float grad_mul, const gct2_loss_scale_state* ls, int mode, float clip, const double* sumsq,
                 hipStream_t s);
int pw_optimizer_reg(int kind, float* p, float* m, float* v, const float* g, void* shadow, int shadow_dtype, size_t n, float lr, float momentum,
                     int nesterov, float rho, float eps, float grad_mul, const gct2_loss_scale_state* ls, int mode, float clip, const double* sumsq,
                     float l2c, int transform, hipStream_t s);
int pw_grad_sumsq_l2(const float* g, const float* p, const gct2_sumsq_seg* segs, const float* seg_coeff, int nseg, size_t npartials,
                     float grad_mul, gct2_loss_scale_state* ls, double* partials, double* sumsq, hipStream_t s);
int pw_l2_penalty(const float* loss, const double* S, float l2, float* penalty, float* total, hipStream_t s);
int pw_cast(int dtype, const float* src, void* dst, size_t n, hipStream_t s);
int pw_ls_init(gct2_loss_scale_state* st, float scale, hipStream_t s);
int pw_ls_begin(gct2_loss_scale_state* st, float base_lr, int warmup_steps, float b1, float b2, hipStream_t s);
int pw_ls_begin_schedule(gct2_loss_scale_state* st, int schedule, float initial, float steps, float decay_rate, int staircase, int bias_correction,
                         float b1, float b2, hipStream_t s);
int pw_ls_check(const float* g, size_t n, gct2_loss_scale_state* st, hipStream_t s);
int pw_ls_update(gct2_loss_scale_state* st, int growth_interval, hipStream_t s);
int pw_relu_bits(int dtype, const void* y, int ldy, size_t pixels, int channels, unsigned char* bits, int ldbits, hipStream_t s);
```

gan-class-transfer2_amd/csrc/plan.hip:

```cpp
#include "gct2_common.h"
#include <cstdlib>
#include <cstring>
#include <type_traits>
#include <utility>
#include <vector>

namespace {

constexpr int MAX_ARGS = 28;

template <class T> T slot_as(uint64_t v) {
  if constexpr (std::is_pointer<T>::value) return reinterpret_cast<T>(static_cast<uintptr_t>(v));
  else if constexpr (std::is_same<T, float>::value) { const uint32_t u = (uint32_t)v; float f; memcpy(&f, &u, 4); return f; }
  else if constexpr (std::is_same<T, double>::value) { double d; memcpy(&d, &v, 8); return d; }
  else return static_cast<T>(v);
}
template <class... A, size_t... I> int invoke(int (*fn)(A...), const uint64_t* a, std::index_sequence<I...>) { return fn(slot_as<A>(a[I])...); }
template <class... A> int thunk(int (*fn)(A...), const uint64_t* a) { return invoke(fn, a, std::index_sequence_for<A...>{}); }
template <class... A> constexpr int arity(int (*)(A...)) { return (int)sizeof...(A); }

struct Entry { const char* name; int (*call)(const uint64_t*); int nargs; };
#define GCT2_ENTRY(f) {#f, [](const uint64_t* a) -> int { return thunk(&f, a); }, arity(&f)}
const Entry ENTRIES[] = {
    GCT2_ENTRY(gct2_ctx_set_relu_bits), GCT2_ENTRY(gct2_bias_queue_flush),
    GCT2_ENTRY(gct2_conv4s2_fwd), GCT2_ENTRY(gct2_conv4s2_dgrad), GCT2_ENTRY(gct2_conv4s2_wgrad),
    GCT2_ENTRY(gct2_convT4s2_fwd), GCT2_ENTRY(gct2_convT4s2_fwd_head_train), GCT2_ENTRY(gct2_convT4s2_dgrad), GCT2_ENTRY(gct2_convT4s2_wgrad),
    GCT2_ENTRY(gct2_adam_apply), GCT2_ENTRY(gct2_adam_keras_multi), GCT2_ENTRY(gct2_ema_update),
    GCT2_ENTRY(gct2_grad_sumsq), GCT2_ENTRY(gct2_adam_keras_clipped), GCT2_ENTRY(gct2_optimizer_apply), GCT2_ENTRY(gct2_loss_scale_begin_schedule),
    GCT2_ENTRY(gct2_optimizer_apply_reg), GCT2_ENTRY(gct2_grad_sumsq_l2), GCT2_ENTRY(gct2_l2_penalty),
    GCT2_ENTRY(gct2_conv2d_s1_fwd), GCT2_ENTRY(gct2_conv2d_s1_dgrad), GCT2_ENTRY(gct2_conv2d_s1_wgrad),
    GCT2_ENTRY(gct2_relu_mask), GCT2_ENTRY(gct2_add), GCT2_ENTRY(gct2_mix_per_image),
    GCT2_ENTRY(gct2_dense_fwd), GCT2_ENTRY(gct2_dense_bwd), GCT2_ENTRY(gct2_dense_head_train),
    GCT2_ENTRY(gct2_dense_steps_fwd), GCT2_ENTRY(gct2_dense_steps_bwd), GCT2_ENTRY(gct2_dense2_fwd), GCT2_ENTRY(gct2_dense2_bwd),
    GCT2_ENTRY(gct2_rng_uniform_int), GCT2_ENTRY(gct2_rng_normal), GCT2_ENTRY(gct2_noise_image), GCT2_ENTRY(gct2_noise_image_rng),
    GCT2_ENTRY(gct2_mse_fwd_bwd), GCT2_ENTRY(gct2_loss_fwd_bwd), GCT2_ENTRY(gct2_cast_from_f32),
    GCT2_ENTRY(gct2_loss_scale_begin), GCT2_ENTRY(gct2_scale_check_finite), GCT2_ENTRY(gct2_loss_scale_update),
    GCT2_ENTRY(gct2_diffusion_mix), GCT2_ENTRY(gct2_diffusion_update), GCT2_ENTRY(gct2_noise_edits), GCT2_ENTRY(gct2_image_prepare),
};
#undef GCT2_ENTRY

enum { OP_CALL = 0, OP_RECORD = 1, OP_WAIT = 2 };
struct Op {
  int kind, entry, nargs, event;
  hipStream_t stream;
  uint64_t a[MAX_ARGS];
};

}

struct gct2_plan {
  std::vector<Op> ops;
  std::vector<hipEvent_t> events;
  std::vector<char> timed;
};

extern "C" {

int gct2_plan_create(gct2_plan** plan) {
  if (!plan) return gct2_fail(GCT2_EINVAL, "plan_create: null output pointer");
  *plan = new (std::nothrow) gct2_plan();
  return *plan ? GCT2_OK : gct2_fail(GCT2_EINVAL, "plan_create: out of host memory");
}

int gct2_plan_destroy(gct2_plan* plan) {
  if (!plan) return GCT2_OK;
  for (hipEvent_t e : plan->events) (void)hipEventDestroy(e);
  delete plan;
  return GCT2_OK;
}

int gct2_plan_add_call(gct2_plan* plan, const char* name, const uint64_t* args, int nargs, int* index) {
  if (!plan || !name || (nargs > 0 && !args)) return gct2_fail(GCT2_EINVAL, "plan_add_call: null pointer");
  for (int e = 0; e < (int)(sizeof(ENTRIES) / sizeof(ENTRIES[0])); e++) {
    if (strcmp(ENTRIES[e].name, name)) continue;
    if (nargs != ENTRIES[e].nargs) return gct2_fail(GCT2_EINVAL, "plan_add_call: %s takes %d arguments, got %d", name, ENTRIES[e].nargs, nargs);
    static_assert(MAX_ARGS >= 28, "gct2_convT4s2_fwd_head_train has 28 arguments");
    if (nargs > MAX_ARGS) return gct2_fail(GCT2_EINVAL, "plan_add_call: too many arguments");
    Op op{};
    op.kind = OP_CALL; op.entry = e; op.nargs = nargs; op.event = -1; op.stream = nullptr;
    for (int i = 0; i < nargs; i++) op.a[i] = args[i];
    plan->ops.push_back(op);
    if (index) *index = (int)plan->ops.size() - 1;
    return GCT2_OK;
  }
  return gct2_fail(GCT2_EINVAL, "plan_add_call: %s is not an entry point a plan can hold", name);
}

int gct2_plan_add_record_kind(gct2_plan* plan, void* stream, int kind, int* event) {
  if (!plan || !event) return gct2_fail(GCT2_EINVAL, "plan_add_record: null pointer");
  if (kind < GCT2_EVENT_DEVICE || kind > GCT2_EVENT_TIMED) return gct2_fail(GCT2_EINVAL, "plan_add_record: unknown event kind %d", kind);
  hipEvent_t ev;
  unsigned flags = kind == GCT2_EVENT_DEVICE ? (hipEventDisableTiming | hipEventReleaseToDevice) : kind == GCT2_EVENT_SYSTEM ? hipEventDisableTiming : hipEventDefault;
  if (kind == GCT2_EVENT_DEVICE)
    if (const char* e = getenv("GCT2_PLAN_EVENT_FLAGS")) flags = (unsigned)strtoul(e, nullptr, 0);
  if (hipEventCreateWithFlags(&ev, flags) != hipSuccess) {
    (void)hipGetLastError();
    return gct2_fail(GCT2_ELAUNCH, "plan_add_record: hipEventCreateWithFlags failed");
  }
  plan->events.push_back(ev);
  plan->timed.push_back(kind == GCT2_EVENT_TIMED);
  Op op{};
  op.kind = OP_RECORD; op.entry = -1; op.nargs = 0; op.event = (int)plan->events.size() - 1; op.stream = reinterpret_cast<hipStream_t>(stream);
  plan->ops.push_back(op);
  *event = op.event;
  return GCT2_OK;
}

int gct2_plan_add_record(gct2_plan* plan, void* stream, int* event) { return gct2_plan_add_record_kind(plan, stream, GCT2_EVENT_DEVICE, event); }

int gct2_plan_elapsed(gct2_plan* plan, int start, int end, float* ms) {
  if (!plan || !ms) return gct2_fail(GCT2_EINVAL, "plan_elapsed: null pointer");
  const int n = (int)plan->events.size();
  if (start < 0 || start >= n || end < 0 || end >= n || !plan->timed[start] || !plan->timed[end])
    return gct2_fail(GCT2_EINVAL, "plan_elapsed: events %d / %d are not timed records of this plan", start, end);
  if (hipEventElapsedTime(ms, plan->events[start], plan->events[end]) != hipSuccess) {
    (void)hipGetLastError();
    return gct2_fail(GCT2_ELAUNCH, "plan_elapsed: hipEventElapsedTime failed (events not recorded yet, or still pending)");
  }
  return GCT2_OK;
}

int gct2_plan_add_wait(gct2_plan* plan, void* stream, int event) {
  if (!plan || event < 0 || event >= (int)plan->events.size()) return gct2_fail(GCT2_EINVAL, "plan_add_wait: null plan or unknown event %d", event);
  Op op{};
  op.kind = OP_WAIT; op.entry = -1; op.nargs = 0; op.event = event; op.stream = reinterpret_cast<hipStream_t>(stream);
  plan->ops.push_back(op);
  return GCT2_OK;
}

int gct2_plan_size(const gct2_plan* plan, int* ops) {
  if (!plan || !ops) return gct2_fail(GCT2_EINVAL, "plan_size: null pointer");
  *ops = (int)plan->ops.size();
  return GCT2_OK;
}

int gct2_plan_set_arg(gct2_plan* plan, int index, int arg, uint64_t value) {
  if (!plan || index < 0 || index >= (int)plan->ops.size()) return gct2_fail(GCT2_EINVAL, "plan_set_arg: no record %d", index);
  Op& op = plan->ops[index];
  if (op.kind != OP_CALL || arg < 0 || arg >= op.nargs) return gct2_fail(GCT2_EINVAL, "plan_set_arg: record %d has no argument %d", index, arg);
  op.a[arg] = value;
  return GCT2_OK;
}

int gct2_plan_run(gct2_plan* plan, int first, int count, int* failed) {
  if (failed) *failed = -1;
  if (!plan || first < 0 || count < 0 || (size_t)first + (size_t)count > plan->ops.size())
    return gct2_fail(GCT2_EINVAL, "plan_run: records [%d, %d) outside the plan", first, first + count);
  for (int k = first; k < first + count; k++) {
    const Op& op = plan->ops[k];
    int rc = GCT2_OK;
    if (op.kind == OP_CALL) rc = ENTRIES[op.entry].call(op.a);
    else if (op.kind == OP_RECORD) {
      if (hipEventRecord(plan->events[op.event], op.stream) != hipSuccess) { (void)hipGetLastError(); rc = gct2_fail(GCT2_ELAUNCH, "plan_run: hipEventRecord failed"); }
    } else {
      if (hipStreamWaitEvent(op.stream, plan->events[op.event], 0) != hipSuccess) { (void)hipGetLastError(); rc = gct2_fail(GCT2_ELAUNCH, "plan_run: hipStreamWaitEvent failed"); }
    }
    if (rc != GCT2_OK) {
      if (failed) *failed = k;
      return rc;
    }
  }
  return GCT2_OK;
}

}
```

gan-class-transfer2_amd/csrc/wgrad_mfma.hip:

```cpp
#include "gct2_common.h"
#include <type_traits>
#include <algorithm>

namespace {

constexpr unsigned OOB = 0x80000000u;
typedef __attribute__((address_space(3))) void lds_void_t;

__device__ __forceinline__ __amdgpu_buffer_rsrc_t make_rsrc(const void* base) {
  return __builtin_amdgcn_make_buffer_rsrc(const_cast<void*>(base), 0, (int)OOB, 0x00020000);
}
__device__ __forceinline__ void dma16(__amdgpu_buffer_rsrc_t rsrc, char* lds_piece, unsigned voff) {
  __builtin_amdgcn_raw_ptr_buffer_load_lds(rsrc, (lds_void_t*)lds_piece, 16, (int)voff, 0, 0, 0);
}

template <typename T, bool S1 = false, bool IMGAL = false>
__global__ __launch_bounds__(256, 2) void wgrad_kernel(WgradParams p) {
  static_assert(!(S1 && IMGAL), "the image-aligned form exists for the 4x4 / stride-2 layers");
  constexpr int IMG = 64 * 256;
  const int KS = S1 ? p.ks : 4, STRIDE = S1 ? 1 : 2, PAD = S1 ? (p.ks - 1) / 2 : 1;
  __shared__ __attribute__((aligned(16))) char lds0[2 * IMG];
  __shared__ __attribute__((aligned(16))) char lds1[2 * IMG];

  GCT2_CLOCK_DECL;
// ... 38 lines not shown
  int rb[4], rh[4], rw[4];
#pragma unroll
  for (int i = 0; i < 4; i++) {
    const int r = step_lo * 64 + row0 + 16 * i;
    rw[i] = r % Ws; const int t = r / Ws; rh[i] = t % Hs; rb[i] = t / Hs;
  }

  unsigned cB[4], cS[4];
  bool vB[4];
  int rr4[4];
  const unsigned stepB = IMGAL ? (unsigned)((64 / (Hs * Ws)) * Hb * Wb * ldb2) : 0u, stepS = (unsigned)(64 * lds2);
  if constexpr (IMGAL) {
    const int hw = Hs * Ws;
#pragma unroll
    for (int i = 0; i < 4; i++) {
      const int rr = row0 + 16 * i, img = rr / hw, pos = rr - img * hw, sh = pos / Ws, sw = pos - sh * Ws;
      const int h = 2 * sh + kh - 1, w = 2 * sw + kw - 1;
      rr4[i] = rr;
      vB[i] = gc_ok && (unsigned)h < (unsigned)Hb && (unsigned)w < (unsigned)Wb;
      cB[i] = (unsigned)(((img * Hb + h) * Wb + w) * ldb2 + cb * 2) + (unsigned)step_lo * stepB;
      cS[i] = (unsigned)(rr * lds2 + (cs0 + lc * 8) * 2) + (unsigned)step_lo * stepS;
    }
  }
  auto issue_al = [&](int step, char* base) {
    const int rem = R - step * 64;
#pragma unroll
    for (int i = 0; i < 4; i++) {
      const bool in = rr4[i] < rem;
      dma16(rs_b, base + (wave + 4 * i) * 1024, (vB[i] && in) ? cB[i] : OOB);
      dma16(rs_s, base + IMG + (wave + 4 * i) * 1024, (cs_ok && in) ? cS[i] : OOB);
      cB[i] += stepB; cS[i] += stepS;
    }
  };
  auto issue_gen = [&](int step, char* base) {
#pragma unroll
    for (int i = 0; i < 4; i++) {
      const int r = step * 64 + row0 + 16 * i;
      const int h = STRIDE * rh[i] + kh - PAD, w = STRIDE * rw[i] + kw - PAD;
      const bool okb = gc_ok && r < R && (unsigned)h < (unsigned)Hb && (unsigned)w < (unsigned)Wb;
      const unsigned offb = (unsigned)(((rb[i] * Hb + h) * Wb + w) * ldb2 + cb * 2);
      dma16(rs_b, base + (wave + 4 * i) * 1024, okb ? offb : OOB);
      const unsigned offs = (unsigned)(r * lds2 + (cs0 + lc * 8) * 2);
      dma16(rs_s, base + IMG + (wave + 4 * i) * 1024, (cs_ok && r < R) ? offs : OOB);
      rw[i] += adv_w; rh[i] += adv_h; rb[i] += adv_b;
      if (rw[i] >= Ws) { rw[i] -= Ws; rh[i]++; }
      if (rh[i] >= Hs) { rh[i] -= Hs; rb[i]++; }
    }
  };
  auto issue = [&](int step, char* base) {
    if constexpr (IMGAL) issue_al(step, base);
    else issue_gen(step, base);
  };

  f32x4_t acc[4][4];
#pragma unroll
  for (int i = 0; i < 4; i++)
#pragma unroll
    for (int j = 0; j < 4; j++) acc[i][j] = f32x4_t{0.f, 0.f, 0.f, 0.f};

  int bfo[2][4], sfo[2][4];
  if constexpr (IMGAL) {
    const int g4 = lane >> 4, q = (lane >> 2) & 3, pq = lane & 3;
#pragma unroll
    for (int kk = 0; kk < 2; kk++) {
      const int k0 = kk * 32 + 8 * g4 + q, swz = timg_swz(k0);
#pragma unroll
      for (int i = 0; i < 4; i++) {
        bfo[kk][i] = k0 * 256 + ((((wm * 64 + i * 16) >> 4) ^ swz) << 5) + pq * 8;
        sfo[kk][i] = IMG + k0 * 256 + ((((wn * 64 + i * 16) >> 4) ^ swz) << 5) + pq * 8;
      }
    }
  }
  auto frag_at = [&](const char* base, int off) -> u32x4_t {
    const s16x4_t lo = __builtin_amdgcn_ds_read_tr16_b64_v4i16((lds_s16x4_t*)(base + off));
    const s16x4_t hi = __builtin_amdgcn_ds_read_tr16_b64_v4i16((lds_s16x4_t*)(base + off + 4 * 256));
    const u32x2_t l2 = __builtin_bit_cast(u32x2_t, lo), h2 = __builtin_bit_cast(u32x2_t, hi);
    return u32x4_t{l2[0], l2[1], h2[0], h2[1]};
  };
  auto compute = [&](const char* base) {
#pragma unroll
    for (int kk = 0; kk < 2; kk++) {
      u32x4_t bf[4], sf[4];
#pragma unroll
      for (int i = 0; i < 4; i++) {
        if constexpr (IMGAL) {
          bf[i] = frag_at(base, bfo[kk][i]);
          sf[i] = frag_at(base, sfo[kk][i]);
        } else {
          bf[i] = timg_frag(base, wm * 64 + i * 16, kk, lane);
          sf[i] = timg_frag(base + IMG, wn * 64 + i * 16, kk, lane);
        }
      }
#pragma unroll
      for (int i = 0; i < 4; i++)
#pragma unroll
        for (int j = 0; j < 4; j++) acc[i][j] = mfma16<T>(sf[j], bf[i], acc[i][j]);
    }
  };

  GCT2_CLOCK_BEGIN;
  {
    issue(step_lo, lds0);
    asm volatile("s_waitcnt vmcnt(0)" ::: "memory");
    __syncthreads();
    for (int step = step_lo; step < step_hi; step += 2) {
      if (step + 1 < step_hi) issue(step + 1, lds1);
      compute(lds0);
      asm volatile("s_waitcnt vmcnt(0)" ::: "memory");
      __syncthreads();
      if (step + 1 >= step_hi) break;
      if (step + 2 < step_hi) issue(step + 2, lds0);
      compute(lds1);
      asm volatile("s_waitcnt vmcnt(0)" ::: "memory");
      __syncthreads();
    }
  }

#ifdef GCT2_STAMP
  GCT2_CLOCK_END(p.clock ? p.stamps : nullptr, 4, wave, lane);
#endif
  float* __restrict__ out = p.ws ? p.ws + (size_t)split * GC * Cs : p.dw;
  const int mode = p.ws ? 2 : (p.rsplit == 1 ? 1 : 0);
  int elane = lane;
  asm volatile("" : "+v"(elane));
#pragma unroll
  for (int i = 0; i < 4; i++) {
    const int row = gc0 + wm * 64 + i * 16 + (elane & 15);
    if (row >= GC) continue;
#pragma unroll
    for (int j = 0; j < 4; j++) {
      const int col = cs0 + wn * 64 + j * 16 + 4 * (elane >> 4);
      if (col >= Cs) continue;
      float* q = out + (size_t)row * Cs + col;
      if (mode == 2) *reinterpret_cast<f32x4_t*>(q) = acc[i][j];
      else if (mode == 1) { if (p.accumulate) *reinterpret_cast<f32x4_t*>(q) += acc[i][j]; else *reinterpret_cast<f32x4_t*>(q) = acc[i][j]; }
      else {
#pragma unroll
        for (int r = 0; r < 4; r++) atomicAdd(q + r, acc[i][j][r]);
      }
    }
  }
#ifdef GCT2_STAMP
  GCT2_CLOCK_EXIT(p.clock ? p.stamps : nullptr, 4, wave, lane);
#endif
}

#define GCT2_VMCNT_ONLY(n) ((((n) & 0xF) | 0x70 | 0xF00 | ((((n) >> 4) & 3) << 14)))
__device__ __forceinline__ void dma16_hidden(__amdgpu_buffer_rsrc_t rsrc, char* lds_piece, unsigned voff) {
  const unsigned lds_addr = (unsigned)(uintptr_t)(lds_void_t*)lds_piece;
  asm volatile("s_mov_b32 m0, %0\n\ts_nop 0\n\tbuffer_load_dwordx4 %1, %2, 0 offen lds" ::"s"(lds_addr), "v"(voff), "s"(rsrc)
               : "memory", "m0");
}

template <typename T, bool TURNS, bool ALIGNED, bool PIPE = false>
__global__ __launch_bounds__(512, 2) void wgrad256q_kernel(WgradParams p) {
  static_assert(!PIPE || (TURNS && ALIGNED), "the pipelined order exists for the aligned, turn-taking stage only");
  constexpr int NST = 5;
  constexpr int IMG = 32 * 256;
  constexpr int STAGE = 4 * IMG;
  constexpr int NDMA = 4;
  __shared__ __attribute__((aligned(16))) char lds[NST * STAGE];

  GCT2_CLOCK_DECL;
  const int tid = threadIdx.x, lane = tid & 63;
  const int wave = __builtin_amdgcn_readfirstlane(tid >> 6);
  const int wn = wave & 3, wm = wave >> 2;
  const int Hs = p.Hs, Ws = p.Ws, Cb = p.Cb, Cs = p.Cs;
  const int Hb = 2 * Hs, Wb = 2 * Ws;
  const int R = p.B * Hs * Ws;
  const int GC = 16 * Cb;
  const int tiles_n = (Cs + 255) / 256;
  const int tiles = ((GC + 255) / 256) * tiles_n;
  int tile, split;
  if (p.rsplit >= 8) {
    const int xcd = blockIdx.x & 7, j = blockIdx.x >> 3;
    tile = j % tiles;
    split = (j / tiles) * 8 + xcd;
    if (split >= p.rsplit) return;
  } else {
    tile = blockIdx.x % tiles;
    split = blockIdx.x / tiles;
  }
  const int gc0 = (tile / tiles_n) * 256, cs0 = (tile % tiles_n) * 256;
  const int steps_total = (R + 63) / 64;
  const int steps_per = (steps_total + p.rsplit - 1) / p.rsplit;
  const int step_lo = split * steps_per;
  const int step_hi = min(steps_total, step_lo + steps_per);
  if (step_lo >= step_hi) return;
  const int st_lo = 2 * step_lo, st_hi = 2 * step_hi;

  const __amdgpu_buffer_rsrc_t rs_b = make_rsrc(p.big), rs_s = make_rsrc(p.small);
  const int row0 = 4 * wave + (lane >> 4);
  const int lc = ((((lane & 15) >> 1) ^ timg_swz(row0)) << 1) | (lane & 1);
  const int ldb2 = p.ldbig * 2, lds2b = p.ldsmall * 2;
  int dg[2];
  unsigned edge[2];
  unsigned s_bad[2];
#pragma unroll
  for (int g = 0; g < 2; g++) {
    const int gc = gc0 + 128 * g + lc * 8;
    const bool ok = gc < GC;
    const int tap = ok ? gc / Cb : 0;
    const int cb = ok ? gc - tap * Cb : 0;
    const int kh = tap >> 2, kw = tap & 3;
    dg[g] = ((kh - 1) * Wb + (kw - 1)) * ldb2 + cb * 2;
    edge[g] = (kh == 0 ? 1u : 0u) | (kh == 3 ? 2u : 0u) | (kw == 0 ? 4u : 0u) | (kw == 3 ? 8u : 0u) | (ok ? 0u : 16u);
    s_bad[g] = (cs0 + 128 * g + lc * 8) < Cs ? 0u : 16u;
  }
  const int adv_w = 32 % Ws, q1 = 32 / Ws, adv_h = q1 % Hs, adv_b = q1 / Hs;
  const int pixA = adv_w * 2 * ldb2, pixB = Wb * ldb2, pixCD = (adv_h * 2 * Wb + adv_b * Hb * Wb) * ldb2;
  int r = st_lo * 32 + row0;
  int rw = r % Ws, rh, rb;
  { const int t = r / Ws; rh = t % Hs; rb = t / Hs; }
  unsigned pix = (unsigned)(((rb * Hb + 2 * rh) * Wb + 2 * rw) * ldb2);
  unsigned soff = (unsigned)(r * lds2b + (cs0 + lc * 8) * 2);
  auto issue = [&](char* base) {
    const unsigned pos = (rh == 0 ? 1u : 0u) | (rh == Hs - 1 ? 2u : 0u) | (rw == 0 ? 4u : 0u) | (rw == Ws - 1 ? 8u : 0u) | (r < R ? 0u : 16u);
    char* piece = base + wave * 1024;
#pragma unroll
    for (int g = 0; g < 2; g++) {
      const unsigned badb = (edge[g] & pos & 15u) | ((edge[g] | pos) & 16u);
      const unsigned bads = (s_bad[g] | pos) & 16u;
      dma16_hidden(rs_b, piece + g * IMG, badb ? OOB : pix + (unsigned)dg[g]);
      dma16_hidden(rs_s, piece + (2 + g) * IMG, bads ? OOB : soff + (unsigned)(g * 256));
    }
    r += 32; soff += (unsigned)(32 * lds2b);
    rw += adv_w; pix += (unsigned)pixA;
    const bool cw = rw >= Ws;
    rw -= cw ? Ws : 0; rh += cw ? 1 : 0; pix += cw ? (unsigned)pixB : 0u;
    rh += adv_h; rb += adv_b; pix += (unsigned)pixCD;
    const bool ch = rh >= Hs;
    rh -= ch ? Hs : 0; rb += ch ? 1 : 0;
  };

  const int span_w = min(32, Ws), span_h = max(1, 32 / Ws);
  const int l_rw = row0 % span_w, l_dh = row0 / span_w;
  unsigned cbig[2], csml[2], eflag[2];
  unsigned long long ms_never[2];
#pragma unroll
  for (int g = 0; g < 2; g++) {
    cbig[g] = (unsigned)((2 * l_dh * Wb + 2 * l_rw) * ldb2 + dg[g]);
    csml[g] = (unsigned)(row0 * lds2b + (cs0 + lc * 8) * 2 + g * 256);
    eflag[g] = ((edge[g] & 1u) && l_dh == 0 ? 1u : 0u) | ((edge[g] & 2u) && l_dh == span_h - 1 ? 2u : 0u) | ((edge[g] & 4u) && l_rw == 0 ? 4u : 0u) |
               ((edge[g] & 8u) && l_rw == span_w - 1 ? 8u : 0u) | (edge[g] & 16u) | 32u;
    ms_never[g] = __builtin_amdgcn_ballot_w64(s_bad[g] != 0);
  }
  int u_rs = st_lo * 32;
  int u_w = u_rs % Ws, u_h, u_b;
  { const int t = u_rs / Ws; u_h = t % Hs; u_b = t / Hs; }
  unsigned u_pix = (unsigned)(((u_b * Hb + 2 * u_h) * Wb + 2 * u_w) * ldb2), u_soff = (unsigned)(u_rs * lds2b);
  auto issue_aligned = [&](char* base) {
    const bool beyond = u_rs >= R;
    const unsigned s_pos = (u_h == 0 ? 1u : 0u) | (u_h + span_h == Hs ? 2u : 0u) | (u_w == 0 ? 4u : 0u) | (u_w + span_w == Ws ? 8u : 0u) | 16u | (beyond ? 32u : 0u);
    const unsigned long long all = beyond ? ~0ull : 0ull;
    char* piece = base + wave * 1024;
#pragma unroll
    for (int g = 0; g < 2; g++) {
      const bool badb = (eflag[g] & s_pos) != 0u;
      const bool bads = __builtin_amdgcn_inverse_ballot_w64(all | ms_never[g]);
      dma16_hidden(rs_b, piece + g * IMG, badb ? OOB : u_pix + cbig[g]);
      dma16_hidden(rs_s, piece + (2 + g) * IMG, bads ? OOB : u_soff + csml[g]);
    }
    u_rs += 32; u_soff += (unsigned)(32 * lds2b);
    u_w += adv_w; u_pix += (unsigned)pixA;
    if (u_w >= Ws) { u_w -= Ws; u_h++; u_pix += (unsigned)pixB; }
    u_h += adv_h; u_b += adv_b; u_pix += (unsigned)pixCD;
    if (u_h >= Hs) { u_h -= Hs; u_b++; }
  };
  auto issue_x = [&](char* base) {
    if constexpr (ALIGNED) issue_aligned(base);
    else issue(base);
  };

  f32x4_t acc[8][4];
#pragma unroll
  for (int i = 0; i < 8; i++)
#pragma unroll
    for (int j = 0; j < 4; j++) acc[i][j] = f32x4_t{0.f, 0.f, 0.f, 0.f};

  int sf_off[4], bf_off[8];
  {
    const int g4 = lane >> 4, q = (lane >> 2) & 3, pq = lane & 3;
    const int k0 = 8 * g4 + q;
    const int swz = timg_swz(k0);
#pragma unroll
    for (int j = 0; j < 4; j++) sf_off[j] = (2 + (wn >> 1)) * IMG + k0 * 256 + (((((wn & 1) * 64 + j * 16) >> 4) ^ swz) << 5) + pq * 8;
#pragma unroll
    for (int i = 0; i < 8; i++) bf_off[i] = wm * IMG + k0 * 256 + ((i ^ swz) << 5) + pq * 8;
  }
  auto frag = [&](const char* base, int off) -> u32x4_t {
    const s16x4_t lo = __builtin_amdgcn_ds_read_tr16_b64_v4i16((lds_s16x4_t*)(base + off));
    const s16x4_t hi = __builtin_amdgcn_ds_read_tr16_b64_v4i16((lds_s16x4_t*)(base + off + 4 * 256));
    const u32x2_t l2 = __builtin_bit_cast(u32x2_t, lo), h2 = __builtin_bit_cast(u32x2_t, hi);
    return u32x4_t{l2[0], l2[1], h2[0], h2[1]};
  };
  auto compute = [&](const char* base) {
    u32x4_t sf[4];
#pragma unroll
    for (int j = 0; j < 4; j++) sf[j] = frag(base, sf_off[j]);
#pragma unroll
    for (int i = 0; i < 8; i++) {
      const u32x4_t bf = frag(base, bf_off[i]);
#pragma unroll
      for (int j = 0; j < 4; j++) acc[i][j] = mfma16<T>(sf[j], bf, acc[i][j]);
    }
  };

  const bool live = p.rsplit > 0;
  auto wait_tail = [&](int ahead) {
    if (ahead >= 3) __builtin_amdgcn_s_waitcnt(GCT2_VMCNT_ONLY(3 * NDMA));
    else if (ahead == 2) __builtin_amdgcn_s_waitcnt(GCT2_VMCNT_ONLY(2 * NDMA));
    else if (ahead == 1) __builtin_amdgcn_s_waitcnt(GCT2_VMCNT_ONLY(NDMA));
    else __builtin_amdgcn_s_waitcnt(GCT2_VMCNT_ONLY(0));
  };
  auto stage = [&](int st, const char* cur, char* tgt) {
    const bool more = st + NST - 1 < st_hi;
    if (more) issue_x(tgt);
    if (live) compute(cur);
    if (more) __builtin_amdgcn_s_waitcnt(GCT2_VMCNT_ONLY(3 * NDMA));
    else wait_tail(st_hi - 1 - (st + 1));
    __builtin_amdgcn_s_barrier();
  };
#if defined(GCT2_STAMP) && defined(GCT2_PHASES)
  unsigned long long ph[6] = {0, 0, 0, 0, 0, 0}, nstages = 0;
  auto now = [&]() -> unsigned long long {
    unsigned long long t;
    __builtin_amdgcn_sched_barrier(0);
// ... 29 lines not shown
        for (int j = 0; j < 4; j++) acc[i][j] = mfma16<T>(sf[j], bf[i], acc[i][j]);
        __builtin_amdgcn_sched_barrier(0);
        if (has_next) {
          bf[i] = frag(nxt, bf_off[i]);
          if (i < 4) sn[i] = frag(nxt, sf_off[i]);
        }
        __builtin_amdgcn_sched_barrier(0);
      }
      if (has_next) {
#pragma unroll
        for (int j = 0; j < 4; j++) sf[j] = sn[j];
      }
    };
    auto pstage_fast = [&](const char* nxt, char* tgt) {
      GCT2_PH(const unsigned long long t0 = now();)
      if (front) issue_aligned(tgt);
      GCT2_PH(const unsigned long long t1 = now();)
      __builtin_amdgcn_sched_barrier(0);
      if (live) rows(nxt, true);
      __builtin_amdgcn_sched_barrier(0);
      GCT2_PH(const unsigned long long t3 = now();)
      if (!front) issue_aligned(tgt);
      GCT2_PH(const unsigned long long t4 = now();)
      __builtin_amdgcn_s_waitcnt(GCT2_VMCNT_ONLY(2 * NDMA));
      GCT2_PH(const unsigned long long t5 = now();)
      __builtin_amdgcn_s_barrier();
      GCT2_PH(const unsigned long long t6 = now();
              ph[0] += t1 - t0; ph[2] += t3 - t1; ph[3] += t4 - t3; ph[4] += t5 - t4; ph[5] += t6 - t5; nstages++;)
    };
    auto pstage = [&](int s, const char* nxt, char* tgt) {
      const bool more = s + NST - 1 < st_hi, has_next = s + 1 < st_hi;
      if (more && front) issue_aligned(tgt);
      __builtin_amdgcn_sched_barrier(0);
      if (live) rows(nxt, has_next);
      __builtin_amdgcn_sched_barrier(0);
      if (more && !front) issue_aligned(tgt);
      const int ahead = st_hi - 1 - (s + 2);
      if (ahead >= 2) __builtin_amdgcn_s_waitcnt(GCT2_VMCNT_ONLY(2 * NDMA));
      else if (ahead == 1) __builtin_amdgcn_s_waitcnt(GCT2_VMCNT_ONLY(NDMA));
      else __builtin_amdgcn_s_waitcnt(GCT2_VMCNT_ONLY(0));
      __builtin_amdgcn_s_barrier();
    };
    int s = st_lo;
    for (; s + 8 < st_hi; s += 5) {
      pstage_fast(lds + STAGE, lds + 4 * STAGE);
      pstage_fast(lds + 2 * STAGE, lds);
      pstage_fast(lds + 3 * STAGE, lds + STAGE);
      pstage_fast(lds + 4 * STAGE, lds + 2 * STAGE);
      pstage_fast(lds, lds + 3 * STAGE);
    }
    for (; s < st_hi; s += 5) {
      pstage(s, lds + STAGE, lds + 4 * STAGE);
      if (s + 1 >= st_hi) break;
      pstage(s + 1, lds + 2 * STAGE, lds);
      if (s + 2 >= st_hi) break;
      pstage(s + 2, lds + 3 * STAGE, lds + STAGE);
      if (s + 3 >= st_hi) break;
      pstage(s + 3, lds + 4 * STAGE, lds + 2 * STAGE);
      if (s + 4 >= st_hi) break;
      pstage(s + 4, lds, lds + 3 * STAGE);
    }
  } else {
  wait_tail(min(st_lo + 3, st_hi - 1) - st_lo);
  __builtin_amdgcn_s_barrier();
  auto stage_fast = [&](const char* cur, char* tgt) {
    const bool front = TURNS ? wm != 0 : true;
    GCT2_PH(const unsigned long long t0 = now(); unsigned long long t2 = 0;)
    if (front) issue_x(tgt);
    GCT2_PH(const unsigned long long t1 = now();)
    __builtin_amdgcn_sched_barrier(0);
    if (live) {
      if constexpr (TURNS) {
        u32x4_t sf[4], bf[8];
#pragma unroll
        for (int j = 0; j < 4; j++) sf[j] = frag(cur, sf_off[j]);
#pragma unroll
        for (int i = 0; i < 8; i++) bf[i] = frag(cur, bf_off[i]);
        __builtin_amdgcn_sched_barrier(0);
        GCT2_PH(t2 = now();)
#pragma unroll
        for (int i = 0; i < 8; i++)
#pragma unroll
          for (int j = 0; j < 4; j++) acc[i][j] = mfma16<T>(sf[j], bf[i], acc[i][j]);
      } else {
        GCT2_PH(t2 = t1;)
        compute(cur);
      }
    }
    __builtin_amdgcn_sched_barrier(0);
    GCT2_PH(const unsigned long long t3 = now();)
    if (!front) issue_x(tgt);
    GCT2_PH(const unsigned long long t4 = now();)
    __builtin_amdgcn_s_waitcnt(GCT2_VMCNT_ONLY(3 * NDMA));
    GCT2_PH(const unsigned long long t5 = now();)
    __builtin_amdgcn_s_barrier();
    GCT2_PH(const unsigned long long t6 = now();
            ph[0] += t1 - t0; ph[1] += t2 - t1; ph[2] += t3 - t2; ph[3] += t4 - t3; ph[4] += t5 - t4; ph[5] += t6 - t5; nstages++;)
  };
  int st = st_lo;
  for (; st + 8 < st_hi; st += 5) {
    stage_fast(lds, lds + 4 * STAGE);
    stage_fast(lds + STAGE, lds);
    stage_fast(lds + 2 * STAGE, lds + STAGE);
    stage_fast(lds + 3 * STAGE, lds + 2 * STAGE);
    stage_fast(lds + 4 * STAGE, lds + 3 * STAGE);
  }
  for (; st < st_hi; st += 5) {
    stage(st, lds, lds + 4 * STAGE);
    if (st + 1 >= st_hi) break;
    stage(st + 1, lds + STAGE, lds);
    if (st + 2 >= st_hi) break;
    stage(st + 2, lds + 2 * STAGE, lds + STAGE);
    if (st + 3 >= st_hi) break;
    stage(st + 3, lds + 3 * STAGE, lds + 2 * STAGE);
    if (st + 4 >= st_hi) break;
    stage(st + 4, lds + 4 * STAGE, lds + 3 * STAGE);
  }
  }
#ifdef GCT2_STAMP
  GCT2_CLOCK_END(p.clock ? p.stamps : nullptr, 8, wave, lane);
#ifdef GCT2_PHASES
  if (p.clock && lane == 0 && (size_t)blockIdx.x * 8 + wave < ((size_t)1 << 15)) {
    unsigned long long* o = p.stamps + ((size_t)1 << 18) + ((size_t)blockIdx.x * 8 + wave) * 8;
    for (int k = 0; k < 6; k++) o[k] = ph[k];
    o[6] = 0; o[7] = nstages;
  }
#endif
#endif
  float* __restrict__ out = p.ws ? p.ws + (size_t)split * GC * Cs : p.dw;
  const int mode = p.ws ? 2 : (p.rsplit == 1 ? 1 : 0);
  int elane = lane;
  asm volatile("" : "+v"(elane));
#pragma unroll
  for (int i = 0; i < 8; i++) {
    const int row = gc0 + wm * 128 + i * 16 + (elane & 15);
    if (row >= GC) continue;
#pragma unroll
    for (int j = 0; j < 4; j++) {
      const int col = cs0 + wn * 64 + j * 16 + 4 * (elane >> 4);
      if (col >= Cs) continue;
      float* q = out + (size_t)row * Cs + col;
      if (mode == 2) *reinterpret_cast<f32x4_t*>(q) = acc[i][j];
      else if (mode == 1) { if (p.accumulate) *reinterpret_cast<f32x4_t*>(q) += acc[i][j]; else *reinterpret_cast<f32x4_t*>(q) = acc[i][j]; }
      else {
#pragma unroll
        for (int rr = 0; rr < 4; rr++) atomicAdd(q + rr, acc[i][j][rr]);
      }
    }
  }
#ifdef GCT2_STAMP
  GCT2_CLOCK_EXIT(p.clock ? p.stamps : nullptr, 8, wave, lane);
#endif
}

__global__ __launch_bounds__(256) void wgrad_reduce_kernel(const float* __restrict__ ws, float* __restrict__ dw, size_t n4, int nsplit,
                                                            int accumulate) {
  const size_t i = (size_t)blockIdx.x * blockDim.x + threadIdx.x;
  if (i >= n4) return;
  const f32x4_t* src = reinterpret_cast<const f32x4_t*>(ws) + i;
  f32x4_t a = src[0];
  int s = 1;
  for (; s + 8 <= nsplit; s += 8) {
    f32x4_t t[8];
#pragma unroll
    for (int u = 0; u < 8; u++) t[u] = src[(size_t)(s + u) * n4];
#pragma unroll
    for (int u = 0; u < 8; u++) a += t[u];
  }
  for (; s < nsplit; s++) a += src[(size_t)s * n4];
  if (accumulate) a += reinterpret_cast<const f32x4_t*>(dw)[i];
  reinterpret_cast<f32x4_t*>(dw)[i] = a;
}

__global__ __launch_bounds__(256) void wgrad_reduce_wide_kernel(const float* __restrict__ ws, float* __restrict__ dw, size_t n4, int nsplit,
                                                                 int accumulate) {
  const int col = threadIdx.x & 15, grp = threadIdx.x >> 4;
  const size_t i = (size_t)blockIdx.x * 16 + col;
  const int per = (nsplit + 15) / 16;
  const int s_lo = grp * per, s_hi = min(nsplit, s_lo + per);
  f32x4_t a = {0.f, 0.f, 0.f, 0.f};
  if (i < n4) {
    const f32x4_t* src = reinterpret_cast<const f32x4_t*>(ws) + i;
    int s = s_lo;
    for (; s + 8 <= s_hi; s += 8) {
      f32x4_t t[8];
#pragma unroll
      for (int u = 0; u < 8; u++) t[u] = __builtin_nontemporal_load(src + (size_t)(s + u) * n4);
#pragma unroll
      for (int u = 0; u < 8; u++) a += t[u];
    }
    for (; s < s_hi; s++) a += __builtin_nontemporal_load(src + (size_t)s * n4);
  }
  __shared__ f32x4_t red[16][16];
  red[grp][col] = a;
  __syncthreads();
  if (grp == 0 && i < n4) {
    f32x4_t t = red[0][col];
#pragma unroll
    for (int g = 1; g < 16; g++) t += red[g][col];
    if (accumulate) t += reinterpret_cast<const f32x4_t*>(dw)[i];
    reinterpret_cast<f32x4_t*>(dw)[i] = t;
  }
}

}

bool wgrad_mfma_supported(int dtype, const WgradParams& p) {
  if (dtype != GCT2_BF16 && dtype != GCT2_F16) return false;
  if (p.Cb % 8 || p.Cs % 8 || p.ldbig % 8 || p.ldsmall % 8) return false;
  if ((uintptr_t)p.big % 16 || (uintptr_t)p.small % 16 || (uintptr_t)p.dw % 16) return false;
  if (p.ks && (p.ks < 1 || p.ks > 7 || !(p.ks & 1))) return false;
  const size_t big_bytes = (size_t)p.B * p.Hs * p.Ws * (p.ks ? 1 : 4) * p.ldbig * 2, small_bytes = (size_t)p.B * p.Hs * p.Ws * p.ldsmall * 2;
  if (big_bytes >= 0x7ff00000u || small_bytes >= 0x7ff00000u) return false;
  return true;
}

int wgrad_mfma(gct2_ctx& c, int dtype, WgradParams p, hipStream_t s, WgradSlabs* defer) {
  if (defer) *defer = WgradSlabs{nullptr, 0, 0};
  const int variant = c.wgrad_variant;
  const int R = p.B * p.Hs * p.Ws;
  const int taps = p.ks ? p.ks * p.ks : 16;
  const int steps_total = (R + 63) / 64;
  const int tiles128 = ((taps * p.Cb + 127) / 128) * ((p.Cs + 127) / 128);
  const int tiles256 = ((taps * p.Cb + 255) / 256) * ((p.Cs + 255) / 256);
  const int minsteps = tiles128 < 256 ? 4 : 8;
  const int blocks256 = tiles256 * std::max(1, std::min((256 + tiles256 - 1) / tiles256, steps_total / minsteps));
  const bool big_tile = !p.ks && (variant == 2 || variant == 4 || variant == 5 || (variant == 0 && tiles128 < 512 && blocks256 >= 192));
  const int tiles = big_tile ? tiles256 : tiles128;
  int rsplit = big_tile ? (256 + tiles - 1) / tiles : (tiles >= 512 ? 1 : (768 + tiles - 1) / tiles);
  if (!big_tile && tiles >= 256 && tiles < 512) rsplit = steps_total >= 32 ? 2 : 1;
  if (!big_tile && c.wgrad_split) rsplit = 1 << (c.wgrad_split - 1);
  rsplit = max(1, min(rsplit, steps_total / 4));
  const int per = (steps_total + rsplit - 1) / rsplit;
  rsplit = (steps_total + per - 1) / per;
  p.rsplit = rsplit;
  p.ws = nullptr;
#ifdef GCT2_STAMP
  p.stamps = c.stamps;
  p.clock = c.stamps_bytes >= GCT2_CLOCK_BYTES ? 1 : 0;
#endif
  const size_t n = (size_t)taps * p.Cb * p.Cs;
  size_t ws_bytes = 0;
  float* ws = c.wgrad_scratch(&ws_bytes);
  if (rsplit > 1 && rsplit <= 128 && ws && n % 4 == 0 && (uintptr_t)p.dw % 16 == 0 && n * sizeof(float) * rsplit <= ws_bytes && variant != 7)
    p.ws = ws;
  dim3 grid(rsplit >= 8 ? tiles * 8 * ((rsplit + 7) / 8) : tiles * rsplit);
  if (!p.ws && rsplit > 1 && !p.accumulate) {
    (void)hipMemsetAsync(p.dw, 0, n * sizeof(float), s);
  }
  gct2_log(c, "wgrad:%s:rsplit=%d:%s", p.ks ? "s1" : (big_tile ? (variant == 4 ? "256q-r03" : (variant == 5 ? "256q-r04" : "256q")) : "128"), rsplit, p.ws ? "slabs" : (rsplit == 1 ? "owner" : "atomics"));
  const bool aligned = (p.Ws % 32 == 0 || (32 % p.Ws == 0 && p.Hs % (32 / p.Ws) == 0)) && variant != 4;
  const bool pipe = aligned && variant != 5;
  const bool imgal = 64 % (p.Hs * p.Ws) == 0 && variant != 6;
  with_dtype16(dtype, [&](auto tag) {
    using T = typename decltype(tag)::type;
    if (p.ks) hipLaunchKernelGGL((wgrad_kernel<T, true>), grid, dim3(256), 0, s, p);
    else if (big_tile && pipe) hipLaunchKernelGGL((wgrad256q_kernel<T, true, true, true>), grid, dim3(512), 0, s, p);
    else if (big_tile && aligned) hipLaunchKernelGGL((wgrad256q_kernel<T, true, true>), grid, dim3(512), 0, s, p);
    else if (big_tile) hipLaunchKernelGGL((wgrad256q_kernel<T, false, false>), grid, dim3(512), 0, s, p);
    else if (imgal) hipLaunchKernelGGL((wgrad_kernel<T, false, true>), grid, dim3(256), 0, s, p);
    else hipLaunchKernelGGL((wgrad_kernel<T>), grid, dim3(256), 0, s, p);
  });
  if (p.ws && defer && !p.accumulate) *defer = WgradSlabs{p.ws, rsplit, n};
  else if (p.ws) hipLaunchKernelGGL(wgrad_reduce_kernel, dim3((unsigned)((n / 4 + 255) / 256)), dim3(256), 0, s, p.ws, p.dw, n / 4, rsplit, p.accumulate);
  return gct2_check_launch("wgrad_mfma");
}

int wgrad_reduce(const float* ws, float* dw, size_t n, int nsplit, int accumulate, hipStream_t s) {
  if (n / 4 <= 16384 && nsplit >= 64) {
    hipLaunchKernelGGL(wgrad_reduce_wide_kernel, dim3((unsigned)((n / 4 + 15) / 16)), dim3(256), 0, s, ws, dw, n / 4, nsplit, accumulate);
    return gct2_check_launch("wgrad_reduce");
  }
  hipLaunchKernelGGL(wgrad_reduce_kernel, dim3((unsigned)((n / 4 + 255) / 256)), dim3(256), 0, s, ws, dw, n / 4, nsplit, accumulate);
  return gct2_check_launch("wgrad_reduce");
}
```

gan-class-transfer2_amd/engine.py:

```python
from __future__ import annotations

import ctypes
import os
import threading
from collections import OrderedDict
from dataclasses import dataclass
from typing import Callable, Dict, List, Optional, Tuple

import numpy as np
import torch

from . import _lib
from ._lib import BF16, F16, F32, Slot, call
from .trainer_math import TrainerState, glorot_limit
from .trainer_math import ema_coefficients as TM_ema_coefficients
from .trainer_math import check_timesteps as TM_check_timesteps
from .trainer_math import check_head_options as TM_check_head_options
from .trainer_math import check_hidden_marker as TM_check_hidden_marker
from .trainer_math import OPTIMIZER_KINDS as _OPTIMIZER_CODES

TORCH_DTYPE = {F32: torch.float32, BF16: torch.bfloat16, F16: torch.float16}


def _round_up(a: int, b: int) -> int:
# ... 115 lines not shown
            for suffix in (".w", ".b"):
                offs[layer + suffix] = off
                off = _round_up(off + int(np.prod(shapes[layer + suffix])), ParamArena.ALIGN)
        return offs, _round_up(off, 64 * ParamArena.ALIGN)

    def ready_order(self) -> List[str]:
        return [l for l in self.topo.layer_order() if l != "dense"] + ["fp32"]

    def numel(self, name: str) -> int:
        return int(np.prod(self.shapes[name]))

    def _view(self, arena: torch.Tensor, name: str) -> torch.Tensor:
        o = self.offsets[name]
        return arena[o:o + self.numel(name)].view(self.shapes[name])

    def param(self, name): return self._view(self.p, name)
    def grad(self, name): return self._view(self.g, name)
    def slot_m(self, name): return self._view(self.m, name)
    def slot_v(self, name): return self._view(self.v, name)

    def wptr(self, name: str) -> int:
        o = self.offsets[name]
        p, shadow = (self._ema, self._ema_shadow) if self._read_ema else (self._p, self._shadow)
        if shadow is None:
            return p.data_ptr() + 4 * o
        return shadow.data_ptr() + 2 * o

    def pptr(self, name: str) -> int:
        return (self._ema if self._read_ema else self._p).data_ptr() + 4 * self.offsets[name]

    def gptr(self, name: str) -> int:
        return self.g.data_ptr() + 4 * self.offsets[name]

    def refresh_shadow(self, stream: int) -> None:
        if self.shadow is not None:
            call("gct2_cast_from_f32", self.dtype, self._p.data_ptr(), self._shadow.data_ptr(), self.total, stream)

    def glorot_init(self, seed: int = 1234, head_initializer: str = "glorot_uniform") -> None:
        gen = torch.Generator(device="cpu").manual_seed(seed)
        for name in sorted(self.shapes):
            shp = self.shapes[name]
            if name.endswith(".b"):
                self.param(name).zero_()
                continue
            w = (torch.rand(shp, generator=gen, dtype=torch.float32) * 2 - 1) * glorot_limit(shp)
            if name == "dense.w" and head_initializer == "zeros":
                w.zero_()
            self.param(name).copy_(w.to(self.device))


class _Buffers:
    pass


class _StepPlan:

    def __init__(self, b: _Buffers):
        self.plan = _lib.Plan()
        self.b = b
        self.loss = None
        self.after: dict = {}
        self.d_off_t = self.d_off_eps = self.d_its = 0
        self.adam_inputs: dict = {}
        self.x_ref = None


_STREAMS: Dict[tuple, "torch.cuda.Stream"] = {}
_STREAMS_LOCK = threading.Lock()
_STREAM_LOG: list = []


def _marker_delay_us(busy: "torch.cuda.Stream", cand: "torch.cuda.Stream", device: torch.device, occupy_us: float = 300.0) -> float:
    e0, e1 = torch.cuda.Event(enable_timing=True), torch.cuda.Event(enable_timing=True)
    torch.cuda.synchronize(device)
    e0.record(busy)
    call("gct2_stream_occupy", busy.cuda_stream, 1, float(occupy_us))
    call("gct2_stream_occupy", cand.cuda_stream, 1, 1.0)
    e1.record(cand)
    cand.synchronize()
    busy.synchronize()
    return e0.elapsed_time(e1) * 1e3


def distinct_stream(device: torch.device, role: str, caller: "torch.cuda.Stream", priority: int = 0, tries: int = 8) -> "torch.cuda.Stream":
    key = (device.index, caller.cuda_stream, role)
    st = _STREAMS.get(key)
    if st is not None:
        return st
    with _STREAMS_LOCK:
        return _pick_stream(key, device, role, caller, priority, tries)


def _pick_stream(key: tuple, device: torch.device, role: str, caller: "torch.cuda.Stream", priority: int, tries: int) -> "torch.cuda.Stream":
    st = _STREAMS.get(key)
    if st is not None:
        return st
    avoid = [caller] + [v for (d, c, _), v in _STREAMS.items() if d == device.index and c == caller.cuda_stream]
    probe = os.environ.get("GCT2_STREAM_PROBE", "1") != "0"
    best, best_wait = None, None
    for k in range(tries if probe else 1):
        cand = torch.cuda.Stream(device=device, priority=priority)
        if any(cand.cuda_stream == a.cuda_stream for a in avoid):
            continue
        waits = [_marker_delay_us(a, cand, device) for a in avoid] if probe else []
        _STREAM_LOG.append((role, k, [round(w, 1) for w in waits]))
        worst = max(waits) if waits else 0.0
        if best is None or worst < best_wait:
            best, best_wait = cand, worst
        if worst < 150.0:
            break
    if best is None:
        best = torch.cuda.Stream(device=device, priority=priority)
    _STREAMS[key] = best
    return best


_ADAM_INPUT_FIELDS = ("p", "m", "v", "shadow", "shadow_dtype", "n", "beta1", "beta2", "eps", "grad_mul", "defer")


class UNetEngine(TrainerState):

    def __init__(self, topo: Topology, dtype: int = BF16, device: Optional[torch.device] = None, steps: int = 200,
                 base_lr: float = 2e-5, warm_up: int = 2000, beta_1: float = 0.9, beta_2: float = 0.999,
                 epsilon: float = 1e-7, loss_scaling: bool = False, seed: int = 1234, rng_seed: int = 0,
                 workspace_mb: int = 64, predict_x: bool = True, predict_scaled_epsilon: bool = False,
                 prediction_weighting: bool = False, ordinary_differential_equation: bool = False, f32_matrix: bool = False,
                 use_ema: bool = False, ema_momentum: float = 0.99, timestep_heads: bool = False,
                 hidden_dense: bool = False, head_initializer: str = "glorot_uniform"):
        TM_check_head_options(type(self).__name__, hidden_dense, timestep_heads, head_initializer)
        super().__init__(dtype, device, steps, base_lr, warm_up, beta_1, beta_2, epsilon, loss_scaling, rng_seed, predict_x,
                         predict_scaled_epsilon, prediction_weighting, ordinary_differential_equation, f32_matrix)
        self.topo = topo
        self.hidden_dense = bool(hidden_dense)
        self.head_initializer = head_initializer
        self.timestep_heads = bool(timestep_heads)
        self.use_fused_head = True
        self.fuse_u0_head = True
        self.keep_pred = False
        self.relu_bits = True
        self.relu_bits_min_bytes = 32 << 20
        self.arena = ParamArena(topo, dtype, self.device, self.head_shapes(topo.fu(0) + 3)[1][0], self.hidden_dense)
        self.arena.glorot_init(seed, head_initializer)
        self.arena.refresh_shadow(self._stream())
        self._bufs: "OrderedDict[Tuple[int, int, int], _Buffers]" = OrderedDict()
        self.max_buffer_sets = 4
        self.ctx = self._new_ctx()
        self.workspace = torch.empty(workspace_mb << 18, dtype=torch.float32, device=self.device) if workspace_mb else None
        self.overlap = True
        self.fuse_adam = True
        self._caller0 = torch.cuda.current_stream(self.device)
        self._side = distinct_stream(self.device, "side", self._caller0)
        self.chain_priority = False
        self._chain_stream = None
        self.wgrad_workspace = torch.empty(workspace_mb << 18, dtype=torch.float32, device=self.device) if workspace_mb else None
        self.ctx.set_workspace(self.workspace)
        self.ctx.set_wgrad_workspace(self.wgrad_workspace)
        self.tail_on_chain = True
        self.ctx_tail = self._new_ctx()
        self.ctx_tail.set_workspace(self.workspace)
        self.defer_adam = True
        self.defer_layers = ("U0", "U1", "U2")
        self.defer_window_at = 3
        self.defer_rowsums = True
        self._bias_queue = None
        self._bias_queue_on = False
        self._pending: list = []
        self._pending_event = None
        self._flush_event = None
        self._pending_names: set = set()
        self._pending_ema: Optional[tuple] = None
        self._defer_ctxs: Dict[str, "_lib.Context"] = {}
        self._defer_ws: Dict[str, torch.Tensor] = {}
        self.arena.before_read = self.flush_deferred
        self._adam_args: Dict[str, "_lib.AdamArgs"] = {}
        self.use_plan = True
        self._plans: Dict[tuple, "_StepPlan"] = {}
        self._plan_seen: Dict[tuple, int] = {}
        self.plan_after = 2
        self.grad_ready_hook: Optional[Callable[[str], None]] = None
        self.hook_plan_aware = False
        self.post_backward: Optional[Callable[[], None]] = None
        self.post_backward_ran = False
        self.post_replay: Optional[Callable[[], None]] = None
        self._grads_in_arena = True
        if use_ema:
            self.enable_ema(ema_momentum)

    def stream_for(self, role: str) -> "torch.cuda.Stream":
        return distinct_stream(self.device, role, self._caller0)

    def _mark(self, stream: "torch.cuda.Stream", system_scope: bool = False):
        P = _lib._recording
        if P is not None:
            return P.record(stream.cuda_stream, _lib.EVENT_SYSTEM if system_scope else _lib.EVENT_DEVICE)
        ev = torch.cuda.Event()
        ev.record(stream)
        return ev

    def _wait(self, stream: "torch.cuda.Stream", token) -> None:
        P = _lib._recording
        if P is not None:
            P.wait(stream.cuda_stream, token)
        else:
            stream.wait_event(token)

    def _wait_stream(self, waiter: "torch.cuda.Stream", other: "torch.cuda.Stream", system_scope: bool = False) -> None:
        self._wait(waiter, self._mark(other, system_scope))

    def _defer_ctx(self, layer: str) -> "_lib.Context":
        c = self._defer_ctxs.get(layer)
        if c is None:
            c = self._defer_ctxs[layer] = self._new_ctx()
            self._defer_ws[layer] = torch.empty_like(self.wgrad_workspace)
            c.set_wgrad_workspace(self._defer_ws[layer])
        c.mirror(self.ctx)
        return c

    def read_launch_log(self) -> list:
        out = self.ctx.read_launch_log() + self.ctx_tail.read_launch_log()
        for c in self._defer_ctxs.values():
            out += c.read_launch_log()
        return out

    def _launch_pending(self, stream: int) -> None:
        A = self.arena
        for _, layer, args in self._pending:
            call("gct2_adam_apply", ctypes.addressof(args), A.gptr(layer + ".w"), A.numel(layer + ".w"), stream)
        self._pending = []
        if self._pending_ema is not None:
            ranges, m, c = self._pending_ema
            self._pending_ema = None
            if self.use_ema:
                for lo, hi in ranges:
                    self._ema_launch(lo, hi, m, c, None, stream)

    def _ema_source(self) -> Tuple[torch.Tensor, Optional[torch.Tensor]]:
        return self.arena._p, self.arena._shadow

    def _ema_tensors(self) -> Tuple[Optional[torch.Tensor], Optional[torch.Tensor]]:
        return self.arena._ema, self.arena._ema_shadow

    def _ema_attach(self, ema: Optional[torch.Tensor], ema_shadow: Optional[torch.Tensor]) -> None:
        self.arena._ema, self.arena._ema_shadow = ema, ema_shadow
        self._plans.clear()
        self._plan_seen.clear()
        graphs = getattr(self, "_forward_graphs", None)
        if graphs:
            for gk in [k for k in graphs if k[2]]:
                del graphs[gk]

    def _ema_select(self, on: bool) -> None:
        self.arena._read_ema = bool(on)

    def _ema_selected(self) -> bool:
        return self.arena._read_ema

    def _ema_partition(self) -> Tuple[List[Tuple[int, int]], List[Tuple[int, int]]]:
        A = self.arena
        held: List[Tuple[int, int]] = []
        for lo, hi in sorted(A.layer_ranges[layer] for _, layer, _ in self._pending):
            if held and held[-1][1] == lo:
                held[-1] = (held[-1][0], hi)
            else:
                held.append((lo, hi))
        now, at = [], 0
        for lo, hi in held:
            if lo > at:
                now.append((at, lo))
            at = hi
        if at < A.total:
            now.append((at, A.total))
        return now, held

    def _ema_step_update(self) -> None:
        m, c = TM_ema_coefficients(self.ema_momentum)
        now, held = self._ema_partition()
        self._pending_ema = (tuple(held), m, c) if held else None
        for lo, hi in now:
            self._ema_launch(lo, hi, m, c, self._ls_ptr(), self._stream())

    def flush_deferred(self) -> None:
        cur = torch.cuda.current_stream(self.device)
        if self._pending:
            self._launch_pending(cur.cuda_stream)
            if _lib._recording is None:
                self._flush_event = torch.cuda.Event()
                self._flush_event.record(cur)
        if self._pending_event is not None:
            self._wait(cur, self._pending_event)
            self._pending_event = None
        self._pending_names = set()

    def _after_flush(self, stream: "torch.cuda.Stream") -> None:
        if self._flush_event is not None and _lib._recording is None:
            stream.wait_event(self._flush_event)

    def check_input_shape(self, H: int, W: int) -> None:
        n = self.topo.octaves
        if H % (2 ** n) or W % (2 ** n):
            raise ValueError(
                f"spatial size {H}x{W} is not divisible by 2**octaves = {2 ** n}: the channel concat of "
                "train.py:114-119 would see mismatched shapes (TensorFlow raises InvalidArgumentError here)")

    def buffers(self, B: int, H: int, W: int) -> _Buffers:
        key = (B, H, W)
        if key in self._bufs:
            self._bufs.move_to_end(key)
            return self._bufs[key]
        self.check_input_shape(H, W)
        while len(self._bufs) >= max(1, self.max_buffer_sets):
            _, old = self._bufs.popitem(last=False)
            graphs = getattr(self, "_forward_graphs", None)
            if graphs:
                for gk in [k for k in graphs if k[0] == id(old)]:
                    del graphs[gk]
        t, n, dt = self.topo, self.topo.octaves, TORCH_DTYPE[self.dtype]
        b = _Buffers()
        b.B, b.H, b.W = B, H, W
        b.hw = [(H >> i, W >> i) for i in range(n + 1)]
        b.ld = [_round_up(t.fu(i) + t.cx(i), 8) for i in range(n)]
        z = lambda *shape, dtype=dt: torch.zeros(*shape, dtype=dtype, device=self.device)
        b.R = [z(B, b.hw[i][0], b.hw[i][1], b.ld[i]) for i in range(n)]
        b.ldd = [_round_up(t.fu(0), 8) if i == 0 else b.ld[i] for i in range(n)]
        b.dR = [z(B, b.hw[i][0], b.hw[i][1], b.ldd[i]) for i in range(n)]
        b.img = z(B, H, W, 4)
        b.bits = [None] * n
        b.bits_valid = False
        for i in range(1, n):
            px = B * b.hw[i][0] * b.hw[i][1]
            if self.dtype != F32 and px * b.ld[i] * 2 >= self.relu_bits_min_bytes and b.ld[i] % 8 == 0 and t.fu(i) % 8 == 0:
                b.bits[i] = torch.zeros(px, b.ld[i] // 8, dtype=torch.uint8, device=self.device)
        b.Dlast = z(B, b.hw[n][0], b.hw[n][1], t.fd(n - 1))
        b.dDlast = z(B, b.hw[n][0], b.hw[n][1], t.fd(n - 1))
        b.pred = z(B, H, W, 3, dtype=torch.float32)
        b.dpred = z(B, H, W, 3, dtype=torch.float32)
        b.eps = z(B, H, W, 3, dtype=torch.float32)
        b.target = None
        b.t_int = z(B, dtype=torch.int32)
        b.loss = z(1, dtype=torch.float32)
        b.partials = z(1024, dtype=torch.float32)
        b.loss_store = {}
        self._bufs[key] = b
        return b

    def _esize(self) -> int:
        return 4 if self.dtype == F32 else 2

    def _slice_ptr(self, buf: torch.Tensor, ch: int) -> int:
        return buf.data_ptr() + ch * self._esize()

    def set_params(self, params: Dict[str, "np.ndarray | torch.Tensor"]) -> None:
        for name, val in params.items():
            tv = torch.as_tensor(np.asarray(val, dtype=np.float32) if not torch.is_tensor(val) else val)
            self.arena.param(name).copy_(tv.to(self.device, torch.float32))
        self.arena.refresh_shadow(self._stream())

    def get_params(self) -> Dict[str, np.ndarray]:
        return {k: self.arena.param(k).detach().cpu().numpy().copy() for k in self.arena.shapes}

    def get_grads(self) -> Dict[str, np.ndarray]:
        if not self._grads_in_arena:
            raise _lib.Gct2Error("the last step applied its weight gradients straight from the kernels' partial sums: the "
                                 "gradient arena does not hold them (use train_step(..., apply=False) or fuse_adam = False)")
        return {k: self.arena.grad(k).detach().cpu().numpy().copy() for k in self.arena.shapes}

    def sample_noise(self, b: _Buffers) -> None:
# ... 113 lines not shown
        n = b.H * b.W * 3
        call("gct2_mix_per_image", b.pred.data_ptr(), None, w.data_ptr(), None, b.pred.data_ptr(), b.B, n, self._stream())
        loss = self.loss_and_dpred(b, target, grad=grad)
        if not grad and self.training_loss != "mse":
            return loss
        call("gct2_mix_per_image", b.dpred.data_ptr(), None, w.data_ptr(), None, b.dpred.data_ptr(), b.B, n, self._stream())
        return loss

    def fused_head_ok(self) -> bool:
        return (self.use_fused_head and self.dtype != F32 and self.topo.fu(0) == 64 and self.workspace is not None
                and not self.objective_weighted() and self.training_loss == "mse" and not self.timestep_heads and not self.hidden_dense)

    def head_train(self, b: _Buffers, target: torch.Tensor, target_is_x: bool = False) -> torch.Tensor:
        t, A = self.topo, self.arena
        ls_ptr = self._ls_ptr()
        call("gct2_dense_head_train", self.ctx.handle, self.dtype, b.R[0].data_ptr(), b.ld[0], A.pptr("dense.w"), A.pptr("dense.b"),
             Slot("x", target.data_ptr()) if target_is_x else target.data_ptr(), b.pred.data_ptr() if self.keep_pred else None, b.dR[0].data_ptr(), b.ldd[0], A.gptr("dense.w"), A.gptr("dense.b"),
             b.loss.data_ptr(), b.partials.data_ptr(), b.B * b.H * b.W, t.fu(0) + 3, 3, t.fu(0), ls_ptr, A.gptr("U0.b"),
             b.img.data_ptr(), 4, 0, self._stream())
        return b.loss

    def fused_u0_head_ok(self, b: _Buffers) -> bool:
        if not (self.fuse_u0_head and self.fused_head_ok() and self.topo.octaves >= 1):
            return False
        Hs, Ws = b.hw[1]
        return Hs % 16 == 0 and Ws % 16 == 0 and self.workspace.numel() >= b.B * (Hs // 16) * (Ws // 16) * 288

    def u0_head_train(self, b: _Buffers, target: torch.Tensor, target_is_x: bool = False) -> torch.Tensor:
        t, A, n = self.topo, self.arena, self.topo.octaves
        Hi, Wi = b.hw[1]
        x, ldx = (b.R[1].data_ptr(), b.ld[1]) if n > 1 else (b.Dlast.data_ptr(), t.fd(0))
        ls_ptr = self._ls_ptr()
        call("gct2_convT4s2_fwd_head_train", self.ctx.handle, self.dtype, x, ldx, A.wptr("U0.w"), A.pptr("U0.b"),
             A.pptr("dense.w"), A.pptr("dense.b"), Slot("x", target.data_ptr()) if target_is_x else target.data_ptr(),
             b.pred.data_ptr() if self.keep_pred else None, b.dR[0].data_ptr(), b.ldd[0],
             A.gptr("dense.w"), A.gptr("dense.b"), b.loss.data_ptr(), b.B, Hi, Wi, t.up_in(0), t.fu(0), t.fu(0) + 3, 3, ls_ptr,
             A.gptr("U0.b"), b.img.data_ptr(), 4, 0, self._stream())
        return b.loss

    def host_call(self, fn: Callable[[], None]) -> None:
        P = _lib._recording
        if P is not None:
            P.cut(("__call__", fn))
        else:
            fn()

    def _ready(self, layer: str, stream: Optional["torch.cuda.Stream"] = None) -> None:
        if self.grad_ready_hook is None:
            return
        P = _lib._recording
        if P is not None and not self.hook_plan_aware:
            P.cut((layer, stream))
        elif stream is None:
            self.grad_ready_hook(layer)
        else:
            with torch.cuda.stream(stream):
                self.grad_ready_hook(layer)

    def backward(self, b: _Buffers, head_done: bool = False, adam_inline: bool = False) -> None:
        t, n, dt, A, cx = self.topo, self.topo.octaves, self.dtype, self.arena, self.ctx.handle
        want_queue = bool(self.defer_rowsums) and self.workspace is not None
        if want_queue != self._bias_queue_on:
            if want_queue and self._bias_queue is None:
                self._bias_queue = torch.empty(4 << 20, dtype=torch.float32, device=self.device)
            self.ctx.set_bias_queue(self._bias_queue if want_queue else None)
            self._bias_queue_on = want_queue
        caller = torch.cuda.current_stream(self.device)
        if self.overlap and self.chain_priority and self._chain_stream is None:
            self._chain_stream = distinct_stream(self.device, "chain", self._caller0, priority=-1)
        main = self._chain_stream if (self.overlap and self.chain_priority) else caller
        if main is not caller:
            self._wait_stream(main, caller)
        self._after_flush(main)
        side = self._side if self.overlap else main
        s, sw = main.cuda_stream, side.cuda_stream
        M = b.B * b.H * b.W
        if not head_done and self.hidden_dense:
            scratch = self._dense2_scratch(b.loss_store, M, t.fu(0) + 3, t.pixel_size)
            call("gct2_dense2_bwd", cx, dt, b.R[0].data_ptr(), b.ld[0], A.wptr("dense_hidden.w"), A.pptr("dense_hidden.b"), A.pptr("dense.w"),
                 b.dpred.data_ptr(), b.dR[0].data_ptr(), b.ldd[0], A.gptr("dense_hidden.w"), A.gptr("dense_hidden.b"), A.gptr("dense.w"),
                 A.gptr("dense.b"), scratch.data_ptr(), scratch.numel(), M, t.fu(0) + 3, t.pixel_size, 3, t.fu(0), 0, s)
        elif not head_done and self.timestep_heads:
            scratch = self._steps_scratch(b.loss_store, b.B, b.H * b.W, t.fu(0) + 3)
            call("gct2_dense_steps_bwd", cx, dt, b.R[0].data_ptr(), b.ld[0], A.pptr("dense.w"), b.t_int.data_ptr(), b.dpred.data_ptr(),
                 b.dR[0].data_ptr(), b.ldd[0], A.gptr("dense.w"), A.gptr("dense.b"), scratch.data_ptr(), scratch.numel(), b.B, b.H * b.W,
                 t.fu(0) + 3, 3, self.steps, t.fu(0), 0, s)
        elif not head_done:
            call("gct2_dense_bwd", dt, b.R[0].data_ptr(), b.ld[0], A.pptr("dense.w"), b.dpred.data_ptr(), b.dR[0].data_ptr(),
                 b.ldd[0], A.gptr("dense.w"), A.gptr("dense.b"), M, t.fu(0) + 3, 3, t.fu(0), 0, s)
        self._ready("dense", main)

        def side_waits_main() -> None:
            if side is not main:
                self._wait_stream(side, main)

        deferred = set(self.defer_layers) if (adam_inline and self.defer_adam and side is not main and self.wgrad_workspace is not None) else set()
        if self._pending:
            self.flush_deferred()

        alpha = self.adam_alpha() if adam_inline else 0.0

        def fused(layer: str):
            if not adam_inline:
                return None
            lo, hi = A.layer_ranges[layer]
            args = self._adam_args.get(layer)
            if args is None:
                args = self._adam_args[layer] = _lib.AdamArgs()
            args.p, args.m, args.v = A._p.data_ptr() + 4 * lo, A._m.data_ptr() + 4 * lo, A._v.data_ptr() + 4 * lo
            args.shadow = (A._shadow.data_ptr() + 2 * lo) if A._shadow is not None else None
            args.shadow_dtype, args.n = self.dtype, hi - lo
            args.alpha, args.beta1, args.beta2, args.eps, args.grad_mul = alpha, self.beta_1, self.beta_2, self.epsilon, 1.0
            args.defer = 1 if layer in deferred else 0
            if layer in deferred:
                self._pending.append(("layer", layer, args))
                self._pending_names.add(layer)
            used.append(layer)
            return ctypes.addressof(args)

        def wctx(layer: str) -> int:
            if layer not in deferred:
                return cx
            return self._defer_ctx(layer).handle

        used: list = []
        self._fused_layers = used
        for i in range(n):
            Hi, Wi = b.hw[i + 1]
            if i < n - 1:
                x, ldx, dx, lddx = b.R[i + 1].data_ptr(), b.ld[i + 1], b.dR[i + 1].data_ptr(), b.ld[i + 1]
            else:
                x, ldx, dx, lddx = b.Dlast.data_ptr(), t.fd(i), b.dDlast.data_ptr(), t.fd(i)
            dz, lddz = b.dR[i].data_ptr(), b.ldd[i]
            db_u = A.gptr(f"U{i}.b") if (i == 0 and not head_done) else None
            if i < n - 1:
                db, split, db2 = A.gptr(f"U{i + 1}.b"), t.fu(i + 1), A.gptr(f"D{i}.b")
            else:
                db, split, db2 = A.gptr(f"D{i}.b"), t.fd(i), None

            def dgrad_u():
                if i < n - 1 and b.bits_valid and b.bits[i + 1] is not None:
                    self.ctx.set_relu_bits(b.bits[i + 1].data_ptr(), b.ld[i + 1] // 8)
                call("gct2_convT4s2_dgrad", cx, dt, dz, lddz, A.wptr(f"U{i}.w"), x, ldx, dx, lddx, b.B, Hi, Wi, t.up_in(i),
                     t.fu(i), 0, db, split, db2, 0, s)

            if adam_inline:
                dgrad_u()
            side_waits_main()
            call("gct2_convT4s2_wgrad", wctx(f"U{i}"), dt, x, ldx, dz, lddz, A.gptr(f"U{i}.w"), db_u, b.B, Hi, Wi, t.up_in(i), t.fu(i), 0,
                 fused(f"U{i}"), sw)
            self._ready(f"U{i}", side)
            if not adam_inline:
                dgrad_u()
        for i in reversed(range(n)):
            H, W = b.hw[i]
            if i < n - 1:
                dz, lddz = self._slice_ptr(b.dR[i + 1], t.fu(i + 1)), b.ld[i + 1]
            else:
                dz, lddz = b.dDlast.data_ptr(), t.fd(i)
            x, ldx = self._slice_ptr(b.R[i], t.fu(i)), b.ld[i]
            xw, ldxw = (b.img.data_ptr(), 4) if i == 0 else (x, ldx)

            def dgrad_d():
                if i > 0:
                    if b.bits_valid and b.bits[i] is not None:
                        self.ctx.set_relu_bits(b.bits[i].data_ptr() + t.fu(i) // 8, b.ld[i] // 8)
                    call("gct2_conv4s2_dgrad", cx, dt, dz, lddz, A.wptr(f"D{i}.w"), x, ldx, self._slice_ptr(b.dR[i], t.fu(i)),
                         b.ld[i], b.B, H, W, t.cx(i), t.fd(i), 1, A.gptr(f"D{i - 1}.b"), t.cx(i), None, 1, s)

            if adam_inline:
                dgrad_d()
            if i == 0 and self._bias_queue_on:
                call("gct2_bias_queue_flush", cx, s)
            if i == 0:
                if adam_inline:
                    if not head_done and side is not main:
                        self._wait_stream(main, side)
                    self._apply_adam(*A.layer_ranges["fp32"], stream=s)
            if i == 0 and adam_inline and side is not main and self.tail_on_chain and self.workspace is not None:
                call("gct2_conv4s2_wgrad", self.ctx_tail.handle, dt, xw, ldxw, dz, lddz, A.gptr("D0.w"), None, b.B, H, W, t.cx(0),
                     t.fd(0), 0, fused("D0"), s)
                self._ready("D0", main)
                continue
            side_waits_main()
            call("gct2_conv4s2_wgrad", cx, dt, xw, ldxw, dz, lddz, A.gptr(f"D{i}.w"), None, b.B, H, W, t.cx(i), t.fd(i), 0,
                 fused(f"D{i}"), sw)
            self._ready(f"D{i}", side)
            if not adam_inline:
                dgrad_d()
        if side is not main:
            self._wait_stream(main, side)
        self._ready("fp32", main)
        if main is not caller:
            self._wait_stream(caller, main)

    def apply_adam(self, lo: int = 0, hi: Optional[int] = None, grad_div: float = 1.0, stream: Optional[int] = None) -> None:
        self.flush_deferred()
        self._apply_adam(lo, hi, grad_div, stream)

    def _apply_adam(self, lo: int = 0, hi: Optional[int] = None, grad_div: float = 1.0, stream: Optional[int] = None) -> None:
        A, s = self.arena, (self._stream() if stream is None else stream)
        hi = A.total if hi is None else hi
        if self.clip_mode != _lib.CLIP_NONE or self.optimizer_kind != "adam" or self._regularized():
            if self._clip_by_norm() and (lo, hi) != (0, A.total):
                raise ValueError(f"apply_adam({lo}, {hi}) with clipnorm / global_clipnorm: a norm needs every gradient of the arena "
                                 f"[0, {A.total}) reduced before the first update; clipping under a bucketed exchange is not built")
            launches = self._adam_clipped if self.optimizer_kind == "adam" else self._optimizer_launches
            if self._regularized():
                launches = self._reg_launches
            launches(A._p, A._m, A._v, A.g, A._shadow, lo, hi, 1.0 / grad_div, s)
            return
        ls_ptr = self._ls_ptr()
        alpha = 0.0 if self.ls_state is not None else self.adam_alpha()
        shadow = None if A._shadow is None else A._shadow.data_ptr() + 2 * lo
        call("gct2_adam_keras_multi", A._p.data_ptr() + 4 * lo, A._m.data_ptr() + 4 * lo, A._v.data_ptr() + 4 * lo,
             A.g.data_ptr() + 4 * lo, shadow, self.dtype, hi - lo, Slot("alpha", alpha), self.beta_1, self.beta_2,
             self.epsilon, 1.0 / grad_div, ls_ptr, 0, s)

    def _clip_segments(self) -> List[Tuple[int, int]]:
        A = self.arena
        return sorted((o, A.numel(name)) for name, o in A.offsets.items())

    def _clip_device(self) -> torch.device:
        return self.arena.g.device

    def check_finite(self, lo: int = 0, hi: Optional[int] = None, stream: Optional[int] = None) -> None:
        hi = self.arena.total if hi is None else hi
        self._check_finite(self.arena.g.data_ptr() + 4 * lo, hi - lo, stream)

    def train_step(self, x: torch.Tensor, t_int: Optional[torch.Tensor] = None, eps: Optional[torch.Tensor] = None,
                   apply: bool = True) -> torch.Tensor:
        if x.dim() != 4 or x.shape[-1] != 3:
            raise ValueError(f"expected an NHWC batch [B,H,W,3], got {tuple(x.shape)}")
        self._refuse_training_on_averages()
        if x.dtype != torch.float32 or not x.is_contiguous() or x.device != self.device:
            x = x.to(self.device, torch.float32).contiguous()
        B, H, W, _ = x.shape
        b = self.buffers(B, H, W)
        inline = (apply and self.fuse_adam and self.ls_state is None and self.clip_mode == _lib.CLIP_NONE and self.optimizer_kind == "adam"
                  and not self._regularized())
        self.post_backward_ran = self.post_backward is not None and not apply
        cur = torch.cuda.current_stream(self.device)
        if self._flush_event is not None:
            cur.wait_event(self._flush_event)
            self._flush_event = None
        if self.use_plan and t_int is None and eps is None and self.default_objective() and _lib._recording is None:
            return self._planned_step(b, x, apply, inline, cur)
        return self._step_body(b, x, t_int, eps, apply, inline)

    def _step_body(self, b: _Buffers, x: torch.Tensor, t_int, eps, apply: bool, inline: bool) -> torch.Tensor:
        if not inline:
            self.flush_deferred()
        self.begin_step()
        if self.l2 > 0.0:
            self._penalty_begin(self._stream())
        default_obj = self.default_objective()
        if t_int is None and eps is None:
            self.sample_and_noise_into_r0(b, x, keep_eps=not default_obj)
        else:
            if t_int is None or eps is None:
                self.sample_noise(b)
            if t_int is not None:
                b.t_int.copy_(t_int.to(self.device, torch.int32))
            if eps is not None:
                b.eps.copy_(eps.to(self.device, torch.float32))
            self.noise_into_r0(b, x)
        target, w = (x, None) if default_obj else self.make_target(b, x)
        weighted = self.objective_weighted()
        fused = self.fused_head_ok()
        if fused and self.fused_u0_head_ok(b):
            self.forward(b, head=False, stop_before_u0=True, planes=True, in_step=True)
            loss = self.u0_head_train(b, target, default_obj)
        else:
            self.forward(b, head=not fused, planes=True, in_step=True)
            if weighted:
                loss = self.weighted_loss_and_dpred(b, target, w)
            else:
                loss = self.head_train(b, target, default_obj) if fused else self.loss_and_dpred(b, target, default_obj)
        if self.l2 > 0.0:
            loss = self._penalty_finish(loss, self._stream())
        self.flush_deferred()
        if _lib._recording is not None:
            _lib._recording.cut(("__alpha__", None))
        self.backward(b, head_done=fused, adam_inline=inline)
        self._grads_in_arena = not inline
        if self.post_backward is not None and not apply:
            self.post_backward()
        if apply:
            if not inline:
                if not self._clip_by_norm():
                    self.check_finite()
                self.apply_adam()
            self.finish_step()
        return loss

    def _plan_key(self, b: _Buffers, apply: bool, inline: bool, cur: "torch.cuda.Stream") -> tuple:
        return (id(b), apply, inline, cur.cuda_stream, self.ctx.version, self.ctx_tail.version,
                tuple(sorted((k, c.version) for k, c in self._defer_ctxs.items())), tuple(l for _, l, _ in self._pending),
                id(self.grad_ready_hook), self.hook_plan_aware, id(self.post_backward), self.overlap, self.chain_priority, self.fuse_adam, self.defer_adam, tuple(self.defer_layers),
                self.defer_window_at, self.defer_rowsums, self.tail_on_chain, self.use_fused_head, self.fuse_u0_head, self.keep_pred, self.relu_bits,
                self.ls_state is not None, self.workspace is not None, self.wgrad_workspace is not None, self.steps, self.rng_seed,
                self.dtype, float(self.beta_1), float(self.beta_2), float(self.epsilon), float(self.base_lr), int(self.warm_up),
                id(self.post_replay), self._side.cuda_stream, self.use_ema, float(self.ema_momentum), self.clip_mode, float(self.clip),
                self.optimizer_kind, float(self.momentum), bool(self.nesterov), float(self.rho), self.lr_schedule, self.training_loss,
                float(self.l2), self.grad_transform, self.timestep_heads, self.hidden_dense,
                self._chain_stream.cuda_stream if self._chain_stream is not None else 0)

    def _planned_step(self, b: _Buffers, x: torch.Tensor, apply: bool, inline: bool, cur: "torch.cuda.Stream") -> torch.Tensor:
        key = self._plan_key(b, apply, inline, cur)
        sp = self._plans.get(key)
        if sp is None:
            seen = self._plan_seen[key] = self._plan_seen.get(key, 0) + 1
            if seen < self.plan_after:
                return self._step_body(b, x, None, None, apply, inline)
            if len(self._plans) >= 8:
                self._plans.pop(next(iter(self._plans)))
            off_t, off_eps, its = self.rng_offset_t, self.rng_offset_eps, self._iterations
            held = {l: bytes(a) for _, l, a in self._pending}
            before = dict(pending=list(self._pending), pending_names=set(self._pending_names), pending_event=self._pending_event,
                          pending_ema=self._pending_ema,
                          bits_valid=b.bits_valid, grads_in_arena=self._grads_in_arena, post_backward_ran=self.post_backward_ran,
                          structs={l: bytes(a) for l, a in self._adam_args.items()})
            sp = _StepPlan(b)
            sp.plan.begin(execute=False)
            try:
                sp.loss = self._step_body(b, x, None, None, apply, inline)
            except BaseException:
                sp.plan.end()
                self.rng_offset_t, self.rng_offset_eps, self._iterations = off_t, off_eps, its
                self._pending, self._pending_names = before["pending"], before["pending_names"]
                self._pending_event, b.bits_valid = before["pending_event"], before["bits_valid"]
                self._pending_ema = before["pending_ema"]
                self._grads_in_arena, self.post_backward_ran = before["grads_in_arena"], before["post_backward_ran"]
                for l, raw in before["structs"].items():
                    ctypes.memmove(ctypes.addressof(self._adam_args[l]), raw, len(raw))
                self._plan_seen[key] = self.plan_after - 1
                raise
            sp.plan.end()
            sp.after = dict(pending=list(self._pending), pending_names=set(self._pending_names), pending_ema=self._pending_ema, bits_valid=b.bits_valid,
                            grads_in_arena=self._grads_in_arena, fused_layers=list(getattr(self, "_fused_layers", [])))
# ... 178 lines not shown
```

include/gct2.h:

```cpp
#ifndef GCT2_H
#define GCT2_H

#include <stddef.h>
#include <stdint.h>

#ifdef __cplusplus
extern "C" {
#endif

enum { GCT2_F32 = 0, GCT2_BF16 = 1, GCT2_F16 = 2 };
enum {
  GCT2_OK = 0,
  GCT2_EINVAL = 1,
  GCT2_ELAUNCH = 2,
  GCT2_ENODEV = 3
};

int gct2_abi_version(void);
enum { GCT2_BUILD_STAMP = 1 };
int gct2_build_flags(void);
const char* gct2_last_error(void);
int gct2_device_check(void);
int gct2_stream_occupy(void* stream, int workgroups, double microseconds);
typedef struct gct2_ctx gct2_ctx;
int gct2_ctx_create(gct2_ctx** ctx);
int gct2_ctx_destroy(gct2_ctx* ctx);
int gct2_ctx_set_workspace(gct2_ctx* ctx, void* ws, size_t bytes);
int gct2_ctx_set_wgrad_workspace(gct2_ctx* ctx, void* ws, size_t bytes);
int gct2_ctx_set_bias_queue(gct2_ctx* ctx, void* buf, size_t bytes);
int gct2_bias_queue_flush(gct2_ctx* ctx, void* stream);
int gct2_ctx_set_tuning(gct2_ctx* ctx, int v);
int gct2_ctx_force_direct(gct2_ctx* ctx, int on);
enum { GCT2_F32_MATH_DIRECT = 0, GCT2_F32_MATH_MFMA = 1 };
int gct2_ctx_set_f32_math(gct2_ctx* ctx, int mode);
int gct2_ctx_set_relu_bits(gct2_ctx* ctx, void* bits, int ld_bytes);
int gct2_ctx_set_stamp_buffer(gct2_ctx* ctx, void* stamps, size_t bytes);

int gct2_ctx_log_launches(gct2_ctx* ctx, int on);
int gct2_ctx_read_launch_log(gct2_ctx* ctx, char* buf, size_t bytes, size_t* needed);

int gct2_conv4s2_fwd(gct2_ctx* ctx, int dtype, const void* x, int ldx, const void* w, const float* bias,
                     void* y, int ldy, int B, int H, int W, int Cin, int Cout, int relu,
                     void* stream);

int gct2_conv4s2_dgrad(gct2_ctx* ctx, int dtype, const void* dz, int lddz, const void* w, const void* act,
                       int ldact, void* dx, int lddx, int B, int H, int W, int Cin, int Cout,
                       int accumulate, float* db, int db_split, float* db2, int db_accumulate, void* stream);

typedef struct gct2_adam_args {
  float* p; float* m; float* v;
  void* shadow; int shadow_dtype;
  size_t n;
  float alpha, beta1, beta2, eps, grad_mul;
  int defer;
  const float* slab_base; int nslab; size_t slab_stride;
} gct2_adam_args;

int gct2_conv4s2_wgrad(gct2_ctx* ctx, int dtype, const void* x, int ldx, const void* dz, int lddz, float* dw,
                       float* db, int B, int H, int W, int Cin, int Cout, int accumulate,
                       gct2_adam_args* adam , void* stream);
int gct2_adam_apply(const gct2_adam_args* adam, float* dw, size_t nw, void* stream);

int gct2_convT4s2_fwd(gct2_ctx* ctx, int dtype, const void* x, int ldx, const void* w, const float* bias,
                      void* y, int ldy, int B, int H, int W, int Cin, int Cout, int relu,
                      void* stream);

int gct2_convT4s2_dgrad(gct2_ctx* ctx, int dtype, const void* dz, int lddz, const void* w, const void* act,
                        int ldact, void* dx, int lddx, int B, int H, int W, int Cin, int Cout,
                        int accumulate, float* db, int db_split, float* db2, int db_accumulate, void* stream);

int gct2_convT4s2_wgrad(gct2_ctx* ctx, int dtype, const void* x, int ldx, const void* dz, int lddz, float* dw,
                        float* db, int B, int H, int W, int Cin, int Cout, int accumulate,
                        gct2_adam_args* adam , void* stream);

int gct2_conv2d_s1_fwd(gct2_ctx* ctx, int dtype, const void* x, int ldx, const void* w, const float* bias, void* y, int ldy,
                       int B, int H, int W, int Cin, int Cout, int KS, int relu, void* stream);
int gct2_conv2d_s1_dgrad(gct2_ctx* ctx, int dtype, const void* dz, int lddz, const void* w, const void* act, int ldact,
                         void* dx, int lddx, int B, int H, int W, int Cin, int Cout, int KS, int accumulate, void* stream);
int gct2_conv2d_s1_wgrad(gct2_ctx* ctx, int dtype, const void* x, int ldx, const void* dz, int lddz, float* dw, float* db,
                         int B, int H, int W, int Cin, int Cout, int KS, int accumulate, void* stream);
int gct2_relu_mask(int dtype, const void* act, int ldact, void* d, int ldd, size_t npix, int C, void* stream);
int gct2_add(int dtype, void* dst, int lddst, const void* src, int ldsrc, size_t npix, int C, void* stream);
int gct2_mix_per_image(const float* x, const float* eps, const float* a, const float* c, float* out, int B, size_t per_image,
                       void* stream);

int gct2_dense_fwd(int dtype, const void* x, int ldx, const float* w, const float* b, float* y,
                   int M, int Cin, int Cout, void* stream);

int gct2_dense_bwd(int dtype, const void* x, int ldx, const float* w, const float* dy, void* dx,
                   int lddx, float* dw, float* db, int M, int Cin, int Cout, int Cmask,
                   int accumulate, void* stream);

int gct2_dense_head_train(gct2_ctx* ctx, int dtype, const void* x, int ldx, const float* w, const float* b,
                          const float* target, float* pred, void* dx, int lddx, float* dw, float* db,
                          float* loss, float* partials, int M, int Cin, int Cout, int Cmask,
                          const float* loss_scale_ptr, float* db_dx ,
                          const void* x2, int ldx2, int accumulate ,
                          void* stream);

int gct2_dense_steps_fwd(gct2_ctx* ctx, int dtype, const void* x, int ldx, const float* w, const float* b, const int32_t* t_int,
                         float* y, int B, int HW, int Cin, int Cout, int steps, void* stream);
int gct2_dense_steps_scratch(int B, int HW, int Cin, int Cout, size_t* floats);
int gct2_dense_steps_bwd(gct2_ctx* ctx, int dtype, const void* x, int ldx, const float* w, const int32_t* t_int, const float* dy,
                         void* dx, int lddx, float* dw, float* db, float* scratch, size_t scratch_floats, int B, int HW, int Cin,
                         int Cout, int steps, int Cmask, int accumulate, void* stream);

#define GCT2_DENSE2_FAST_PIXELS 64
#define GCT2_DENSE2_PLAIN_MAX 256
int gct2_dense2_fwd(gct2_ctx* ctx, int dtype, const void* x, int ldx, const void* w1, const float* b1, const float* w2, const float* b2,
                    float* y, int M, int Cin, int Chid, int Cout, void* stream);
int gct2_dense2_scratch(int M, int Cin, int Chid, int Cout, size_t* floats);
int gct2_dense2_bwd(gct2_ctx* ctx, int dtype, const void* x, int ldx, const void* w1, const float* b1, const float* w2, const float* dy,
                    void* dx, int lddx, float* dw1, float* db1, float* dw2, float* db2, float* scratch, size_t scratch_floats,
                    int M, int Cin, int Chid, int Cout, int Cmask, int accumulate, void* stream);

int gct2_convT4s2_fwd_head_train(gct2_ctx* ctx, int dtype, const void* x, int ldx, const void* w, const float* bias,
                                 const float* head_w, const float* head_b, const float* target, float* pred, void* dy,
                                 int lddy, float* head_dw, float* head_db, float* loss, int B, int H, int W, int Cin,
                                 int Cout, int head_Cin, int head_Cout, const float* loss_scale_ptr, float* db,
                                 const void* x2, int ldx2, int accumulate, void* stream);

int gct2_rng_uniform_int(uint64_t seed, uint64_t stream_id, uint64_t offset, int32_t* out, size_t n,
                         int lo, int hi_inclusive, void* stream);
int gct2_rng_normal(uint64_t seed, uint64_t stream_id, uint64_t offset, float* out, size_t n,
                    void* stream);

int gct2_noise_image(int dtype, const float* x, const int32_t* t_int, const float* eps, void* out,
                     int ldout, void* out2, int ldout2, int B, int HW, int C, int steps, void* stream);

int gct2_noise_image_rng(int dtype, const float* x, const int32_t* t_int, uint64_t seed, uint64_t stream_id,
                         uint64_t offset, float* eps_out, void* out, int ldout, void* out2, int ldout2, int B, int HW,
                         int C, int steps, void* stream);

int gct2_diffusion_mix(int dtype, const float* x_theta, const float* eps_theta, float alpha, float* fake,
                       void* out, int ldout, void* out2, int ldout2, size_t npix, int C, void* stream);
enum { GCT2_SAMPLE_X = 0, GCT2_SAMPLE_EPS = 1, GCT2_SAMPLE_SCALED_EPS = 2, GCT2_SAMPLE_ODE = 3 };
int gct2_diffusion_update(int mode, const float* pred, const float* fake, double alpha, double alpha_prev, float* x_theta,
                          float* eps_theta, size_t n, void* stream);
int gct2_noise_edits(const float* eps, const float* dictionary, int K, float* out, int H, int W, int C,
                     void* stream);

int gct2_image_prepare(const uint8_t* src, const int64_t* offsets, const int32_t* dims, float* dst, int B, int size,
                       void* stream);

int gct2_mse_fwd_bwd(const float* pred, const float* target, float* dpred, float* loss,
                     float* partials, size_t n, const float* loss_scale_ptr, void* stream);

#define GCT2_LOSS_MSE 0
#define GCT2_LOSS_L1 1
#define GCT2_LOSS_MSE_POOLED 2
#define GCT2_LOSS_DCT 3
int gct2_loss_scratch(int kind, int B, int H, int W, int C, size_t* floats);
int gct2_loss_fwd_bwd(int kind, const float* pred, const float* target, float* dpred, float* loss,
                      float* scratch, size_t scratch_floats, int B, int H, int W, int C,
                      const float* basis, const float* loss_scale_ptr, void* stream);

typedef struct {
  float scale; float inv_scale; int32_t good_steps; int32_t found_inf;
  int32_t applied_steps;
  float alpha;
  int32_t reserved[2];
} gct2_loss_scale_state;
int gct2_loss_scale_init(gct2_loss_scale_state* state, float initial_scale, void* stream);
int gct2_loss_scale_begin(gct2_loss_scale_state* state, float base_lr, int warmup_steps, float beta1, float beta2,
                          void* stream);
int gct2_scale_check_finite(const float* g, size_t n, gct2_loss_scale_state* state, void* stream);
int gct2_loss_scale_update(gct2_loss_scale_state* state, int growth_interval, void* stream);

int gct2_adam_keras_multi(float* p, float* m, float* v, float* g, void* shadow, int shadow_dtype,
                          size_t n, float alpha, float beta1, float beta2, float eps, float grad_mul,
                          const gct2_loss_scale_state* ls, int zero_grad, void* stream);

int gct2_ema_update(float* ema, const float* p, void* ema_shadow, int shadow_dtype, size_t n, float momentum, float one_minus,
                    const gct2_loss_scale_state* ls, void* stream);

#define GCT2_CLIP_NONE 0
#define GCT2_CLIP_VALUE 1
#define GCT2_CLIP_NORM 2
#define GCT2_CLIP_GLOBAL_NORM 3
#define GCT2_SUMSQ_CHUNK 32768
#define GCT2_SUMSQ_MAX_SEGMENTS 1024
typedef struct { uint64_t begin, count, first_partial; } gct2_sumsq_seg;

int gct2_sumsq_layout(const uint64_t* begin, const uint64_t* count, int nseg, gct2_sumsq_seg* out, size_t* npartials);

int gct2_grad_sumsq(const float* g, const gct2_sumsq_seg* segs, int nseg, size_t npartials, float grad_mul, gct2_loss_scale_state* ls,
                    double* partials, double* sumsq, void* stream);

int gct2_adam_keras_clipped(float* p, float* m, float* v, float* g, void* shadow, int shadow_dtype, size_t n,
                            float alpha, float beta1, float beta2, float eps, float grad_mul,
                            const gct2_loss_scale_state* ls, int clip_mode, float clip, const double* sumsq, void* stream);

#define GCT2_OPT_ADAM 0
#define GCT2_OPT_SGD 1
#define GCT2_OPT_RMSPROP 2
int gct2_optimizer_apply(int kind, float* p, float* m, float* v, float* g, void* shadow, int shadow_dtype, size_t n,
                         float lr, float momentum, int nesterov, float rho, float epsilon, float grad_mul,
                         const gct2_loss_scale_state* ls, int clip_mode, float clip, const double* sumsq, void* stream);

#define GCT2_GRAD_NONE 0
#define GCT2_GRAD_SIGN 1
int gct2_optimizer_apply_reg(int kind, float* p, float* m, float* v, float* g, void* shadow, int shadow_dtype, size_t n,
                             float lr, float momentum, int nesterov, float rho, float epsilon, float grad_mul,
                             const gct2_loss_scale_state* ls, int clip_mode, float clip, const double* sumsq,
                             float l2_coeff, int transform, void* stream);

int gct2_grad_sumsq_l2(const float* g, const float* p, const gct2_sumsq_seg* segs, const float* seg_coeff, int nseg, size_t npartials,
                       float grad_mul, gct2_loss_scale_state* ls, double* partials, double* sumsq, void* stream);

int gct2_l2_penalty(const float* loss, const double* S, float l2, float* penalty_out, float* total_out, void* stream);

#define GCT2_SCHEDULE_WARMUP 0
#define GCT2_SCHEDULE_INVERSE_TIME_DECAY 1
int gct2_loss_scale_begin_schedule(gct2_loss_scale_state* state, int schedule, float initial, float steps, float decay_rate,
                                   int staircase, int bias_correction, float beta1, float beta2, void* stream);
// ... 21 lines not shown
```

Measured before the change: 25880 images/sec.

## Group three discriminator wgrad convolutions into one grouped MFMA launch

Adds a grouped conv4s2 weight-gradient entry that packs up to four layers' wgrad work items into a single launch of the 256-tile MFMA kernel, with per-member split-K and XCD-aware item mapping. The engine now batches discriminator layers 3, 2 and 1 into one call instead of three separate launches, and triples the wgrad workspace so each member gets its own split slabs. The aim is to fill the GPU with small-layer wgrads concurrently and cut launch and tail overhead. The cost is a larger workspace and a fallback to per-layer calls whenever the shapes don't fit.

```diff
diff --git a/gan-class-transfer2_amd/_lib.py b/gan-class-transfer2_amd/_lib.py
--- a/gan-class-transfer2_amd/_lib.py
+++ b/gan-class-transfer2_amd/_lib.py
@@ -36,6 +36,22 @@
     _fields_ = [("p", C.c_void_p), ("m", C.c_void_p), ("v", C.c_void_p), ("shadow", C.c_void_p), ("shadow_dtype", C.c_int),
                 ("n", C.c_size_t), ("alpha", C.c_float), ("beta1", C.c_float), ("beta2", C.c_float), ("eps", C.c_float),
                 ("grad_mul", C.c_float), ("defer", C.c_int), ("slab_base", C.c_void_p), ("nslab", C.c_int), ("slab_stride", C.c_size_t)]
+
+
+class WgradDesc(C.Structure):
+    _fields_ = [("x", C.c_void_p), ("ldx", C.c_int), ("dz", C.c_void_p), ("lddz", C.c_int), ("dw", C.c_void_p), ("db", C.c_void_p),
+                ("B", C.c_int), ("H", C.c_int), ("W", C.c_int), ("Cin", C.c_int), ("Cout", C.c_int), ("accumulate", C.c_int),
+                ("adam", C.c_void_p)]
+
+
+WGRAD_GROUP_MAX = 4
+
+
+def wgrad_group_splits(tiles, steps, cus: int) -> list:
+    n = len(tiles)
+    t, s, r = (C.c_int * n)(*tiles), (C.c_int * n)(*steps), (C.c_int * n)()
+    check(load().gct2_wgrad_group_splits(C.cast(t, C.c_void_p), C.cast(s, C.c_void_p), n, int(cus), C.cast(r, C.c_void_p)), "gct2_wgrad_group_splits")
+    return list(r)
 
 
 _vp, _i, _f, _d, _u64, _sz = C.c_void_p, C.c_int, C.c_float, C.c_double, C.c_uint64, C.c_size_t
@@ -65,6 +81,9 @@
     "gct2_conv4s2_fwd": [_vp, _i, _vp, _i, _vp, _vp, _vp, _i, _i, _i, _i, _i, _i, _i, _vp],
     "gct2_conv4s2_dgrad": [_vp, _i, _vp, _i, _vp, _vp, _i, _vp, _i, _i, _i, _i, _i, _i, _i, _vp, _i, _vp, _i, _vp],
     "gct2_conv4s2_wgrad": [_vp, _i, _vp, _i, _vp, _i, _vp, _vp, _i, _i, _i, _i, _i, _i, _vp, _vp],
+    "gct2_conv4s2_wgrad_group": [_vp, _i, _i, _vp, _vp],
+    "gct2_wgrad_group_splits": [_vp, _vp, _i, _i, _vp],
+    "gct2_ctx_force_wgrad_group_splits": [_vp, _vp, _i],
     "gct2_adam_apply": [_vp, _vp, _sz, _vp],
     "gct2_convT4s2_fwd": [_vp, _i, _vp, _i, _vp, _vp, _vp, _i, _i, _i, _i, _i, _i, _i, _vp],
     "gct2_convT4s2_fwd_head_train": [_vp, _i, _vp, _i, _vp, _vp, _vp, _vp, _vp, _vp, _vp, _i, _vp, _vp, _vp, _i, _i, _i, _i, _i, _i, _i,
@@ -179,7 +198,7 @@
 
 
 PLANNABLE = frozenset(n for n, sig in SIGNATURES.items() if n == "gct2_ctx_set_relu_bits" or (
-    not n.startswith(("gct2_ctx_", "gct2_plan_", "gct2_loss_scale_init")) and n not in ("gct2_abi_version", "gct2_build_flags", "gct2_device_check", "gct2_stream_occupy", "gct2_sumsq_layout", "gct2_loss_scratch", "gct2_dense_steps_scratch", "gct2_dense2_scratch")))
+    not n.startswith(("gct2_ctx_", "gct2_plan_", "gct2_loss_scale_init")) and n not in ("gct2_abi_version", "gct2_build_flags", "gct2_device_check", "gct2_stream_occupy", "gct2_sumsq_layout", "gct2_wgrad_group_splits", "gct2_loss_scratch", "gct2_dense_steps_scratch", "gct2_dense2_scratch")))
 _recording = None
 _FLOAT_STRUCT = struct.Struct("<f")
 _DOUBLE_STRUCT = struct.Struct("<d")
@@ -355,6 +374,14 @@
         call("gct2_ctx_set_bias_queue", self.handle, tensor.data_ptr() if tensor is not None else None,
              tensor.numel() * tensor.element_size() if tensor is not None else 0)
 
+    def set_wgrad_group_splits(self, splits=None) -> None:
+        self.version += 1
+        if splits is None or splits == "balanced":
+            call("gct2_ctx_force_wgrad_group_splits", self.handle, None, 0 if splits is None else -1)
+        else:
+            arr = (C.c_int * len(splits))(*splits)
+            call("gct2_ctx_force_wgrad_group_splits", self.handle, C.cast(arr, C.c_void_p), len(splits))
+
     def set_tuning(self, v: int) -> None:
         self.version += 1
         self.tuning = int(v)
diff --git a/gan-class-transfer2_amd/csrc/capi.hip b/gan-class-transfer2_amd/csrc/capi.hip
--- a/gan-class-transfer2_amd/csrc/capi.hip
+++ b/gan-class-transfer2_amd/csrc/capi.hip
@@ -136,9 +136,14 @@
   return GCT2_OK;
 }
 enum WgradKind { WG_CONV, WG_CONVT, WG_S1 };
-int wgrad_entry(gct2_ctx* ctx, const char* fn, WgradKind kind, int dtype, const void* x, int ldx, const void* dz, int lddz, float* dw, float* db,
-                int B, int H, int W, int Cin, int Cout, int KS, int accumulate, gct2_adam_args* adam, void* stream) {
-  gct2_ctx& c = C(ctx);
+struct WgradCall {
+  WgradParams p; WgradKind kind;
+  const void* dz; int lddz; float* dw; float* db; int Cout, accumulate;
+  size_t nw, dz_pixels;
+  gct2_adam_args* adam;
+};
+int wgrad_check(gct2_ctx& c, const char* fn, WgradKind kind, int dtype, const void* x, int ldx, const void* dz, int lddz, float* dw, float* db,
+                int B, int H, int W, int Cin, int Cout, int KS, int accumulate, gct2_adam_args* adam, WgradCall* out) {
   if (int e = PlaneTaken(c).none(fn)) return e;
   const int up = kind == WG_CONVT ? 2 : 1;
   if (int e = check_conv_args(fn, dtype, x, dz, dw, B, up * H, up * W, Cin, Cout)) return e;
@@ -152,15 +157,26 @@
   p.accumulate = accumulate ? 1 : 0;
   p.ks = kind == WG_S1 ? KS : 0;
   const size_t nw = (size_t)16 * Cin * Cout, dz_pixels = (size_t)B * p.Hs * p.Ws * (kind == WG_CONVT ? 4 : 1);
+  if (adam) if (int e = check_adam_args(adam, dw, nw)) return e;
+  *out = WgradCall{p, kind, dz, lddz, dw, db, Cout, accumulate, nw, dz_pixels, adam};
+  return GCT2_OK;
+}
+int wgrad_finish(gct2_ctx& c, int dtype, const WgradCall& w, const WgradSlabs& sl, void* stream) {
+  if (w.db) if (int e = wgrad_db(c, dtype, w.dz, w.lddz, w.db, w.dz_pixels, w.Cout, w.accumulate, stream)) return e;
+  return w.adam ? adam_after_wgrad(w.adam, w.dw, w.nw, sl, stream) : GCT2_OK;
+}
+int wgrad_entry(gct2_ctx* ctx, const char* fn, WgradKind kind, int dtype, const void* x, int ldx, const void* dz, int lddz, float* dw, float* db,
+                int B, int H, int W, int Cin, int Cout, int KS, int accumulate, gct2_adam_args* adam, void* stream) {
+  gct2_ctx& c = C(ctx);
+  WgradCall w;
+  if (int e = wgrad_check(c, fn, kind, dtype, x, ldx, dz, lddz, dw, db, B, H, W, Cin, Cout, KS, accumulate, adam, &w)) return e;
   WgradSlabs sl{nullptr, 0, 0};
   WgradSlabs* defer = adam ? &sl : nullptr;
-  if (adam) if (int e = check_adam_args(adam, dw, nw)) return e;
-  if (kind == WG_CONV && !c.force_direct && rgb_wgrad_supported(dtype, p)) {
+  if (kind == WG_CONV && !c.force_direct && rgb_wgrad_supported(dtype, w.p)) {
     gct2_log(c, "rgb:wgrad");
-    if (int e = rgb_wgrad(c, dtype, p, S(stream), defer)) return e;
-  } else if (int e = run_wgrad(c, dtype, p, stream, defer)) return e;
-  if (db) if (int e = wgrad_db(c, dtype, dz, lddz, db, dz_pixels, Cout, accumulate, stream)) return e;
-  return adam ? adam_after_wgrad(adam, dw, nw, sl, stream) : GCT2_OK;
+    if (int e = rgb_wgrad(c, dtype, w.p, S(stream), defer)) return e;
+  } else if (int e = run_wgrad(c, dtype, w.p, stream, defer)) return e;
+  return wgrad_finish(c, dtype, w, sl, stream);
 }
 int check_scratch(const char* fn, const gct2_ctx* ctx, const void* buf) {
   if (!ctx) return gct2_fail(GCT2_EINVAL, "%s: null ctx", fn);
@@ -328,6 +344,60 @@
 int gct2_conv4s2_wgrad(gct2_ctx* ctx, int dtype, const void* x, int ldx, const void* dz, int lddz, float* dw, float* db, int B, int H, int W,
                        int Cin, int Cout, int accumulate, gct2_adam_args* adam, void* stream) {
   return wgrad_entry(ctx, "conv4s2_wgrad", WG_CONV, dtype, x, ldx, dz, lddz, dw, db, B, H, W, Cin, Cout, 0, accumulate, adam, stream);
+}
+
+int gct2_conv4s2_wgrad_group(gct2_ctx* ctx, int dtype, int n, const gct2_wgrad_desc* descs, void* stream) {
+  gct2_ctx& c = C(ctx);
+  if (int e = PlaneTaken(c).none("conv4s2_wgrad_group")) return e;
+  if (n < 1 || n > GCT2_WGRAD_GROUP_MAX) return gct2_fail(GCT2_EINVAL, "conv4s2_wgrad_group: n = %d outside [1, %d]", n, GCT2_WGRAD_GROUP_MAX);
+  if (!descs) return gct2_fail(GCT2_EINVAL, "conv4s2_wgrad_group: null descriptor array");
+  WgradCall w[GCT2_WGRAD_GROUP_MAX];
+  WgradParams members[GCT2_WGRAD_GROUP_MAX];
+  WgradSlabs sl[GCT2_WGRAD_GROUP_MAX];
+  WgradSlabs* defer[GCT2_WGRAD_GROUP_MAX];
+  bool fits = !f32_on_mfma(c, dtype);
+  for (int i = 0; i < n; i++) {
+    const gct2_wgrad_desc& d = descs[i];
+    if (int e = wgrad_check(c, "conv4s2_wgrad", WG_CONV, dtype, d.x, d.ldx, d.dz, d.lddz, d.dw, d.db, d.B, d.H, d.W, d.Cin, d.Cout, 0, d.accumulate,
+                            d.adam, &w[i]))
+      return e;
+    members[i] = w[i].p;
+    sl[i] = WgradSlabs{nullptr, 0, 0};
+    defer[i] = d.adam ? &sl[i] : nullptr;
+    if (rgb_wgrad_supported(dtype, w[i].p)) fits = false;
+  }
+  bool done = false;
+  if (fits) if (int e = wgrad_mfma_group(c, dtype, n, members, S(stream), defer, &done)) return e;
+  if (!done) {
+    for (int i = 0; i < n; i++) {
+      const gct2_wgrad_desc& d = descs[i];
+      if (int e = wgrad_entry(ctx, "conv4s2_wgrad", WG_CONV, dtype, d.x, d.ldx, d.dz, d.lddz, d.dw, d.db, d.B, d.H, d.W, d.Cin, d.Cout, 0,
+                              d.accumulate, d.adam, stream))
+        return e;
+    }
+    return GCT2_OK;
+  }
+  for (int i = 0; i < n; i++) if (int e = wgrad_finish(c, dtype, w[i], sl[i], stream)) return e;
+  return GCT2_OK;
+}
+int gct2_wgrad_group_splits(const int* tiles, const int* steps, int n, int cus, int* rsplit) {
+  if (!tiles || !steps || !rsplit) return gct2_fail(GCT2_EINVAL, "wgrad_group_splits: null pointer");
+  if (n < 1 || n > GCT2_WGRAD_GROUP_MAX) return gct2_fail(GCT2_EINVAL, "wgrad_group_splits: n = %d outside [1, %d]", n, GCT2_WGRAD_GROUP_MAX);
+  long long owners = 0;
+  for (int i = 0; i < n; i++) {
+    if (tiles[i] < 1 || steps[i] < 1 || cus < 1) return gct2_fail(GCT2_EINVAL, "wgrad_group_splits: non-positive tiles, steps or cus");
+    owners += tiles[i];
+  }
+  if (owners > cus || !wgrad_group_splits(n, tiles, steps, cus, rsplit))
+    return gct2_fail(GCT2_EINVAL, "wgrad_group_splits: %lld tiles are more than %d work-groups hold in one round", owners, cus);
+  return GCT2_OK;
+}
+int gct2_ctx_force_wgrad_group_splits(gct2_ctx* ctx, const int* rsplit, int n) {
+  if (!ctx) return gct2_fail(GCT2_EINVAL, "ctx_force_wgrad_group_splits: null ctx");
+  if (n < -1 || n > GCT2_WGRAD_GROUP_MAX || (n > 0 && !rsplit)) return gct2_fail(GCT2_EINVAL, "ctx_force_wgrad_group_splits: n = %d outside [-1, %d] or null splits", n, GCT2_WGRAD_GROUP_MAX);
+  ctx->group_splits_n = n;
+  for (int i = 0; i < n; i++) ctx->group_splits[i] = rsplit[i];
+  return GCT2_OK;
 }
 
 int gct2_convT4s2_fwd(gct2_ctx* ctx, int dtype, const void* x, int ldx, const void* w, const float* bias, void* y, int ldy, int B, int H, int W,
diff --git a/gan-class-transfer2_amd/csrc/gct2_common.h b/gan-class-transfer2_amd/csrc/gct2_common.h
--- a/gan-class-transfer2_amd/csrc/gct2_common.h
+++ b/gan-class-transfer2_amd/csrc/gct2_common.h
@@ -24,6 +24,7 @@
   int wgrad_split = 0;
   int no_splitk = 0;
   int force_direct = 0;
+  int group_splits_n = 0, group_splits[GCT2_WGRAD_GROUP_MAX] = {};
   int f32_math = GCT2_F32_MATH_DIRECT;
   unsigned long long* stamps = nullptr; size_t stamps_bytes = 0;
   unsigned char* relu_bits = nullptr; int relu_ldbits = 0; int relu_bits_done = 0;
@@ -323,6 +324,8 @@
 bool wgrad_mfma_supported(int dtype, const WgradParams& p);
 int wgrad_mfma(gct2_ctx& c, int dtype, WgradParams p, hipStream_t s, WgradSlabs* defer);
 int wgrad_reduce(const float* ws, float* dw, size_t n, int nsplit, int accumulate, hipStream_t s);
+bool wgrad_group_splits(int n, const int* tiles, const int* steps, int cus, int* rsplit);
+int wgrad_mfma_group(gct2_ctx& c, int dtype, int n, const WgradParams* members, hipStream_t s, WgradSlabs* const* defer, bool* done);
 
 bool rgb_fwd_supported(int dtype, const TapGemmParams& p);
 bool rgb_fwd_writes_bits(const TapGemmParams& p);
diff --git a/gan-class-transfer2_amd/csrc/plan.hip b/gan-class-transfer2_amd/csrc/plan.hip
--- a/gan-class-transfer2_amd/csrc/plan.hip
+++ b/gan-class-transfer2_amd/csrc/plan.hip
@@ -23,7 +23,7 @@
 #define GCT2_ENTRY(f) {#f, [](const uint64_t* a) -> int { return thunk(&f, a); }, arity(&f)}
 const Entry ENTRIES[] = {
     GCT2_ENTRY(gct2_ctx_set_relu_bits), GCT2_ENTRY(gct2_bias_queue_flush),
-    GCT2_ENTRY(gct2_conv4s2_fwd), GCT2_ENTRY(gct2_conv4s2_dgrad), GCT2_ENTRY(gct2_conv4s2_wgrad),
+    GCT2_ENTRY(gct2_conv4s2_fwd), GCT2_ENTRY(gct2_conv4s2_dgrad), GCT2_ENTRY(gct2_conv4s2_wgrad), GCT2_ENTRY(gct2_conv4s2_wgrad_group),
     GCT2_ENTRY(gct2_convT4s2_fwd), GCT2_ENTRY(gct2_convT4s2_fwd_head_train), GCT2_ENTRY(gct2_convT4s2_dgrad), GCT2_ENTRY(gct2_convT4s2_wgrad),
     GCT2_ENTRY(gct2_adam_apply), GCT2_ENTRY(gct2_adam_keras_multi), GCT2_ENTRY(gct2_ema_update),
     GCT2_ENTRY(gct2_grad_sumsq), GCT2_ENTRY(gct2_adam_keras_clipped), GCT2_ENTRY(gct2_optimizer_apply), GCT2_ENTRY(gct2_loss_scale_begin_schedule),
diff --git a/gan-class-transfer2_amd/csrc/wgrad_mfma.hip b/gan-class-transfer2_amd/csrc/wgrad_mfma.hip
--- a/gan-class-transfer2_amd/csrc/wgrad_mfma.hip
+++ b/gan-class-transfer2_amd/csrc/wgrad_mfma.hip
@@ -214,8 +214,27 @@
                : "memory", "m0");
 }
 
-template <typename T, bool TURNS, bool ALIGNED, bool PIPE = false>
-__global__ __launch_bounds__(512, 2) void wgrad256q_kernel(WgradParams p) {
+struct WgradGroup {
+  WgradParams m[GCT2_WGRAD_GROUP_MAX];
+  int first[GCT2_WGRAD_GROUP_MAX];
+  int n, items, per;
+};
+template <typename T, bool TURNS, bool ALIGNED, bool PIPE = false, typename Args = WgradParams>
+__global__ __launch_bounds__(512, 2) void wgrad256q_kernel(Args args) {
+  constexpr bool GROUPED = std::is_same<Args, WgradGroup>::value;
+  static_assert(!GROUPED || PIPE, "only the aligned, pipelined order is grouped");
+  int item = 0, member = 0;
+  if constexpr (GROUPED) {
+    item = args.per ? (int)(blockIdx.x & 7) * args.per + (int)(blockIdx.x >> 3) : (int)blockIdx.x;
+    if (item >= args.items) return;
+#pragma unroll
+    for (int i = 1; i < GCT2_WGRAD_GROUP_MAX; i++) member += (i < args.n && item >= args.first[i]) ? 1 : 0;
+    item -= args.first[member];
+  }
+  const WgradParams& p = [&]() -> const WgradParams& {
+    if constexpr (GROUPED) return args.m[member];
+    else return args;
+  }();
   static_assert(!PIPE || (TURNS && ALIGNED), "the pipelined order exists for the aligned, turn-taking stage only");
   constexpr int NST = 5;
   constexpr int IMG = 32 * 256;
@@ -234,7 +253,17 @@
   const int tiles_n = (Cs + 255) / 256;
   const int tiles = ((GC + 255) / 256) * tiles_n;
   int tile, split;
-  if (p.rsplit >= 8) {
+  if constexpr (GROUPED) {
+    if (args.per || p.rsplit < 8) {
+      tile = item % tiles;
+      split = item / tiles;
+    } else {
+      const int xcd = item & 7, j = item >> 3;
+      tile = j % tiles;
+      split = (j / tiles) * 8 + xcd;
+    }
+    if (split >= p.rsplit) return;
+  } else if (p.rsplit >= 8) {
     const int xcd = blockIdx.x & 7, j = blockIdx.x >> 3;
     tile = j % tiles;
     split = (j / tiles) * 8 + xcd;
@@ -570,6 +599,7 @@
   GCT2_CLOCK_EXIT(p.clock ? p.stamps : nullptr, 8, wave, lane);
 #endif
 }
+template <typename T> constexpr auto wgrad256q_group_kernel = wgrad256q_kernel<T, true, true, true, WgradGroup>;
 
 __global__ __launch_bounds__(256) void wgrad_reduce_kernel(const float* __restrict__ ws, float* __restrict__ dw, size_t n4, int nsplit,
                                                             int accumulate) {
@@ -633,6 +663,25 @@
   return true;
 }
 
+static bool wgrad_big_tile(int variant, const WgradParams& p) {
+  const int taps = p.ks ? p.ks * p.ks : 16;
+  const int steps_total = (p.B * p.Hs * p.Ws + 63) / 64;
+  const int tiles128 = ((taps * p.Cb + 127) / 128) * ((p.Cs + 127) / 128);
+  const int tiles256 = ((taps * p.Cb + 255) / 256) * ((p.Cs + 255) / 256);
+  const int minsteps = tiles128 < 256 ? 4 : 8;
+  const int blocks256 = tiles256 * std::max(1, std::min((256 + tiles256 - 1) / tiles256, steps_total / minsteps));
+  return !p.ks && (variant == 2 || variant == 4 || variant == 5 || (variant == 0 && tiles128 < 512 && blocks256 >= 192));
+}
+
+static int wgrad_single_split(bool big_tile, int tiles, int steps_total, int forced) {
+  int rsplit = big_tile ? (256 + tiles - 1) / tiles : (tiles >= 512 ? 1 : (768 + tiles - 1) / tiles);
+  if (!big_tile && tiles >= 256 && tiles < 512) rsplit = steps_total >= 32 ? 2 : 1;
+  if (!big_tile && forced) rsplit = 1 << (forced - 1);
+  rsplit = max(1, min(rsplit, steps_total / 4));
+  const int per = (steps_total + rsplit - 1) / rsplit;
+  return (steps_total + per - 1) / per;
+}
+
 int wgrad_mfma(gct2_ctx& c, int dtype, WgradParams p, hipStream_t s, WgradSlabs* defer) {
   if (defer) *defer = WgradSlabs{nullptr, 0, 0};
   const int variant = c.wgrad_variant;
@@ -641,16 +690,9 @@
   const int steps_total = (R + 63) / 64;
   const int tiles128 = ((taps * p.Cb + 127) / 128) * ((p.Cs + 127) / 128);
   const int tiles256 = ((taps * p.Cb + 255) / 256) * ((p.Cs + 255) / 256);
-  const int minsteps = tiles128 < 256 ? 4 : 8;
-  const int blocks256 = tiles256 * std::max(1, std::min((256 + tiles256 - 1) / tiles256, steps_total / minsteps));
-  const bool big_tile = !p.ks && (variant == 2 || variant == 4 || variant == 5 || (variant == 0 && tiles128 < 512 && blocks256 >= 192));
+  const bool big_tile = wgrad_big_tile(variant, p);
   const int tiles = big_tile ? tiles256 : tiles128;
-  int rsplit = big_tile ? (256 + tiles - 1) / tiles : (tiles >= 512 ? 1 : (768 + tiles - 1) / tiles);
-  if (!big_tile && tiles >= 256 && tiles < 512) rsplit = steps_total >= 32 ? 2 : 1;
-  if (!big_tile && c.wgrad_split) rsplit = 1 << (c.wgrad_split - 1);
-  rsplit = max(1, min(rsplit, steps_total / 4));
-  const int per = (steps_total + rsplit - 1) / rsplit;
-  rsplit = (steps_total + per - 1) / per;
+  const int rsplit = wgrad_single_split(big_tile, tiles, steps_total, c.wgrad_split);
   p.rsplit = rsplit;
   p.ws = nullptr;
 #ifdef GCT2_STAMP
@@ -684,6 +726,103 @@
   return gct2_check_launch("wgrad_mfma");
 }
 
+static bool split_allowed(int steps, int r) {
+  if (r == 1) return true;
+  const int per = (steps + r - 1) / r, last = steps - (r - 1) * per;
+  return r <= 128 && last >= 4;
+}
+bool wgrad_group_splits(int n, const int* tiles, const int* steps, int cus, int* rsplit) {
+  int longest = 0;
+  for (int i = 0; i < n; i++) longest = std::max(longest, steps[i]);
+  for (int L = 1; L <= longest; L++) {
+    long long blocks = 0;
+    bool ok = true;
+    for (int i = 0; i < n && ok; i++) {
+      int r = (steps[i] + L - 1) / L;
+      while (r <= 128 && !split_allowed(steps[i], r)) r++;
+      ok = r <= 128 && (steps[i] + r - 1) / r <= L;
+      rsplit[i] = r;
+      blocks += (long long)tiles[i] * r;
+    }
+    if (ok && blocks <= cus) return true;
+  }
+  return false;
+}
+
+int wgrad_mfma_group(gct2_ctx& c, int dtype, int n, const WgradParams* members, hipStream_t s, WgradSlabs* const* defer, bool* done) {
+  *done = false;
+  if (n < 1 || n > GCT2_WGRAD_GROUP_MAX || (c.wgrad_variant != 0 && c.wgrad_variant != 2) || c.force_direct) return GCT2_OK;
+  int tiles[GCT2_WGRAD_GROUP_MAX], steps[GCT2_WGRAD_GROUP_MAX], rsplit[GCT2_WGRAD_GROUP_MAX];
+  for (int i = 0; i < n; i++) {
+    const WgradParams& p = members[i];
+    if (p.ks || !wgrad_mfma_supported(dtype, p) || !wgrad_big_tile(c.wgrad_variant, p)) return GCT2_OK;
+    if (!(p.Ws % 32 == 0 || (32 % p.Ws == 0 && p.Hs % (32 / p.Ws) == 0))) return GCT2_OK;
+    tiles[i] = ((16 * p.Cb + 255) / 256) * ((p.Cs + 255) / 256);
+    steps[i] = (p.B * p.Hs * p.Ws + 63) / 64;
+  }
+  bool one_round = false;
+  if (c.group_splits_n > 0) {
+    if (c.group_splits_n != n) return gct2_fail(GCT2_EINVAL, "conv4s2_wgrad_group: %d forced splits for %d members", c.group_splits_n, n);
+    for (int i = 0; i < n; i++) {
+      const int r = c.group_splits[i];
+      if (r < 1 || r > 128) return gct2_fail(GCT2_EINVAL, "conv4s2_wgrad_group: forced split %d of member %d outside [1, 128]", r, i);
+      const int per = (steps[i] + r - 1) / r;
+      rsplit[i] = (steps[i] + per - 1) / per;
+    }
+  } else if (c.group_splits_n < 0) {
+    int dev = 0, cus = 0;
+    if (hipGetDevice(&dev) != hipSuccess || hipDeviceGetAttribute(&cus, hipDeviceAttributeMultiprocessorCount, dev) != hipSuccess || cus < 8) {
+      (void)hipGetLastError();
+      cus = 256;
+    }
+    if (!wgrad_group_splits(n, tiles, steps, cus, rsplit)) return GCT2_OK;
+    one_round = true;
+  } else {
+    for (int i = 0; i < n; i++) rsplit[i] = wgrad_single_split(true, tiles[i], steps[i], 0);
+  }
+  size_t ws_bytes = 0, used = 0;
+  int live = 0;
+  float* ws = c.wgrad_scratch(&ws_bytes);
+  WgradGroup g{};
+  g.n = n;
+  for (int i = 0; i < n; i++) {
+    WgradParams p = members[i];
+    const size_t nw = (size_t)16 * p.Cb * p.Cs;
+    p.rsplit = rsplit[i];
+    p.ws = nullptr;
+#ifdef GCT2_STAMP
+    p.stamps = c.stamps;
+    p.clock = c.stamps_bytes >= GCT2_CLOCK_BYTES ? 1 : 0;
+#endif
+    if (rsplit[i] > 1) {
+      const size_t bytes = nw * sizeof(float) * rsplit[i];
+      if (!ws || (uintptr_t)ws % 16 || used + bytes > ws_bytes) return GCT2_OK;
+      p.ws = reinterpret_cast<float*>(reinterpret_cast<char*>(ws) + used);
+      used = (used + bytes + 255) / 256 * 256;
+    }
+    g.m[i] = p;
+    g.first[i] = g.items;
+    live += tiles[i] * rsplit[i];
+    g.items += one_round ? tiles[i] * rsplit[i] : (rsplit[i] >= 8 ? tiles[i] * 8 * ((rsplit[i] + 7) / 8) : (tiles[i] * rsplit[i] + 7) / 8 * 8);
+  }
+  g.per = one_round ? (g.items + 7) / 8 : 0;
+  for (int i = 0; i < n; i++) gct2_log(c, "wgrad:256q:rsplit=%d:%s", rsplit[i], g.m[i].ws ? "slabs" : "owner");
+  gct2_log(c, "wgrad_group:n=%d:blocks=%d", n, live);
+  with_dtype16(dtype, [&](auto tag) {
+    using T = typename decltype(tag)::type;
+    hipLaunchKernelGGL((wgrad256q_group_kernel<T>), dim3(one_round ? 8 * g.per : g.items), dim3(512), 0, s, g);
+  });
+  *done = true;
+  for (int i = 0; i < n; i++) {
+    const WgradParams& p = g.m[i];
+    const size_t nw = (size_t)16 * p.Cb * p.Cs;
+    if (defer[i]) *defer[i] = WgradSlabs{nullptr, 0, 0};
+    if (p.ws && defer[i] && !p.accumulate) *defer[i] = WgradSlabs{p.ws, p.rsplit, nw};
+    else if (p.ws) hipLaunchKernelGGL(wgrad_reduce_kernel, dim3((unsigned)((nw / 4 + 255) / 256)), dim3(256), 0, s, p.ws, p.dw, nw / 4, p.rsplit, p.accumulate);
+  }
+  return gct2_check_launch("wgrad_mfma_group");
+}
+
 int wgrad_reduce(const float* ws, float* dw, size_t n, int nsplit, int accumulate, hipStream_t s) {
   if (n / 4 <= 16384 && nsplit >= 64) {
     hipLaunchKernelGGL(wgrad_reduce_wide_kernel, dim3((unsigned)((n / 4 + 15) / 16)), dim3(256), 0, s, ws, dw, n / 4, nsplit, accumulate);
diff --git a/gan-class-transfer2_amd/engine.py b/gan-class-transfer2_amd/engine.py
--- a/gan-class-transfer2_amd/engine.py
+++ b/gan-class-transfer2_amd/engine.py
@@ -291,7 +291,7 @@
         self._side = distinct_stream(self.device, "side", self._caller0)
         self.chain_priority = False
         self._chain_stream = None
-        self.wgrad_workspace = torch.empty(workspace_mb << 18, dtype=torch.float32, device=self.device) if workspace_mb else None
+        self.wgrad_workspace = torch.empty(3 * workspace_mb << 18, dtype=torch.float32, device=self.device) if workspace_mb else None
         self.ctx.set_workspace(self.workspace)
         self.ctx.set_wgrad_workspace(self.wgrad_workspace)
         self.tail_on_chain = True
@@ -350,7 +350,7 @@
         c = self._defer_ctxs.get(layer)
         if c is None:
             c = self._defer_ctxs[layer] = self._new_ctx()
-            self._defer_ws[layer] = torch.empty_like(self.wgrad_workspace)
+            self._defer_ws[layer] = torch.empty(self.wgrad_workspace.numel() // 3, dtype=torch.float32, device=self.device)
             c.set_wgrad_workspace(self._defer_ws[layer])
         c.mirror(self.ctx)
         return c
@@ -770,6 +770,12 @@
             self._ready(f"U{i}", side)
             if not adam_inline:
                 dgrad_u()
+        grouped = [3, 2, 1] if n >= 4 else []
+        descs = None
+        if grouped:
+            descs = b.__dict__.setdefault("wgrad_descs", {}).get(adam_inline)
+            if descs is None:
+                descs = b.wgrad_descs[adam_inline] = (_lib.WgradDesc * len(grouped))()
         for i in reversed(range(n)):
             H, W = b.hw[i]
             if i < n - 1:
@@ -800,10 +806,20 @@
                      t.fd(0), 0, fused("D0"), s)
                 self._ready("D0", main)
                 continue
-            side_waits_main()
-            call("gct2_conv4s2_wgrad", cx, dt, xw, ldxw, dz, lddz, A.gptr(f"D{i}.w"), None, b.B, H, W, t.cx(i), t.fd(i), 0,
-                 fused(f"D{i}"), sw)
-            self._ready(f"D{i}", side)
+            if i in grouped:
+                d = descs[grouped.index(i)]
+                d.x, d.ldx, d.dz, d.lddz, d.dw, d.db = xw, ldxw, dz, lddz, A.gptr(f"D{i}.w"), None
+                d.B, d.H, d.W, d.Cin, d.Cout, d.accumulate, d.adam = b.B, H, W, t.cx(i), t.fd(i), 0, fused(f"D{i}")
+                if i == grouped[-1]:
+                    side_waits_main()
+                    call("gct2_conv4s2_wgrad_group", cx, dt, len(grouped), ctypes.addressof(descs), sw)
+                    for j in grouped:
+                        self._ready(f"D{j}", side)
+            else:
+                side_waits_main()
+                call("gct2_conv4s2_wgrad", cx, dt, xw, ldxw, dz, lddz, A.gptr(f"D{i}.w"), None, b.B, H, W, t.cx(i), t.fd(i), 0,
+                     fused(f"D{i}"), sw)
+                self._ready(f"D{i}", side)
             if not adam_inline:
                 dgrad_d()
         if side is not main:
diff --git a/include/gct2.h b/include/gct2.h
--- a/include/gct2.h
+++ b/include/gct2.h
@@ -61,6 +61,18 @@
                        gct2_adam_args* adam , void* stream);
 int gct2_adam_apply(const gct2_adam_args* adam, float* dw, size_t nw, void* stream);
 
+#define GCT2_WGRAD_GROUP_MAX 4
+typedef struct gct2_wgrad_desc {
+  const void* x; int ldx;
+  const void* dz; int lddz;
+  float* dw; float* db;
+  int B, H, W, Cin, Cout, accumulate;
+  gct2_adam_args* adam;
+} gct2_wgrad_desc;
+int gct2_conv4s2_wgrad_group(gct2_ctx* ctx, int dtype, int n, const gct2_wgrad_desc* descs, void* stream);
+int gct2_wgrad_group_splits(const int* tiles, const int* steps, int n, int cus, int* rsplit);
+int gct2_ctx_force_wgrad_group_splits(gct2_ctx* ctx, const int* rsplit, int n);
+
 int gct2_convT4s2_fwd(gct2_ctx* ctx, int dtype, const void* x, int ldx, const void* w, const float* bias,
                       void* y, int ldy, int B, int H, int W, int Cin, int Cout, int relu,
                       void* stream);
```

After: 25810 images/sec. No clear change (-0.3%).
